# lc700x/desktop2stereo

Hardware: AMD Instinct MI355X
Metric: stereo frames/sec @1080p DepthAnything-v2-ViT-B (higher is better)
Workload: dtype bf16; 1 GPU; DepthAnything-v2-vitb bf16, 1920x1080 uint8 RGB noise frames, batch 1 per GPU, Depth Resolution 518 (model input 294x518), Full-SBS uint8 output 3840x1080, pred; parallelism=frame-sharded dp1, no data-path collective (each rank generates its own frames)

## Files before the change

### desktop2stereo_amd/_lib.py

```python
from __future__ import annotations

import ctypes as C
import os

HERE = os.path.dirname(os.path.abspath(__file__))
LIB_PATH = os.environ.get("D2S_LIB") or os.path.join(HERE, "libd2s_hip.so")

OK = 0
MODE = {"Half-SBS": 0, "Full-SBS": 1, "Half-TAB": 2, "Full-TAB": 3}
FMT_U8_HWC, FMT_F32_CHW, FMT_F32_HWC, FMT_U8_CHW = 0, 1, 2, 3
PREC_FP32, PREC_BF16, PREC_FP8, PREC_BF16X3, PREC_FP8_MLP = 0, 1, 2, 3, 4


class ModelDesc(C.Structure):
    _fields_ = [("hidden", C.c_int32), ("heads", C.c_int32), ("layers", C.c_int32),
                ("out_indices", C.c_int32 * 4), ("neck", C.c_int32 * 4), ("fusion", C.c_int32),
                ("head_hidden", C.c_int32), ("mlp", C.c_int32), ("patch", C.c_int32),
                ("pos_grid", C.c_int32), ("ln_eps", C.c_float), ("precision", C.c_int32), ("temporal", C.c_int32),
                ("max_depth", C.c_float)]


class PostParams(C.Structure):
    _fields_ = [("percentile", C.c_float), ("subsample_cap", C.c_int32), ("gamma", C.c_float),
                ("foreground_scale", C.c_float), ("aa_strength", C.c_float), ("ema_alpha", C.c_float),
                ("metric", C.c_int32)]


RESAMPLE = {"bilinear": 0, "bicubic_aa": 1}


class PreParams(C.Structure):
    _fields_ = [("mean", C.c_float * 3), ("std", C.c_float * 3), ("resample", C.c_int32), ("square", C.c_int32)]


class SbsParams(C.Structure):
    _fields_ = [("ipd_uv", C.c_double), ("depth_ratio", C.c_float), ("convergence", C.c_float),
                ("display_mode", C.c_int32), ("fill_16_9", C.c_int32)]


class DibrParams(C.Structure):
    _fields_ = [("ipd_uv", C.c_double), ("depth_strength", C.c_float), ("convergence", C.c_float), ("roll", C.c_float),
                ("search_radius", C.c_float), ("depth_tolerance", C.c_float), ("blur_radius", C.c_float),
                ("res_w", C.c_float), ("res_h", C.c_float), ("display_mode", C.c_int32),
                ("feather_enabled", C.c_int32), ("feather_width", C.c_float), ("corner_radius", C.c_float),
                ("viewport", C.c_float * 4), ("alpha_mode", C.c_int32), ("struct_size", C.c_uint32)]


class XrScreen(C.Structure):
    _fields_ = [("struct_size", C.c_uint32), ("curve", C.c_int32), ("width", C.c_double), ("height", C.c_double),
                ("distance", C.c_double), ("pan_x", C.c_double), ("pan_y", C.c_double), ("yaw", C.c_double), ("pitch", C.c_double),
                ("roll", C.c_double), ("normal_offset", C.c_double), ("clear", C.c_float * 4)]


class XrEye(C.Structure):
    _fields_ = [("vp", C.c_double * 16), ("width", C.c_int32), ("height", C.c_int32), ("eye", C.c_int32), ("struct_size", C.c_uint32)]


class XrGlow(C.Structure):
    _fields_ = [("struct_size", C.c_uint32), ("mode", C.c_int32), ("range_m", C.c_double), ("inner_edge_fraction", C.c_double)]


class XrFrost(C.Structure):
    _fields_ = [("struct_size", C.c_uint32), ("mode", C.c_int32), ("head", C.c_double * 3), ("intensity", C.c_double), ("alpha", C.c_double),
                ("edge_inset", C.c_double), ("beam_softness", C.c_double), ("beam_thickness", C.c_double), ("lod", C.c_double),
                ("threshold", C.c_double), ("noise_scale", C.c_double), ("blend", C.c_double), ("diffuse", C.c_double), ("time", C.c_double)]


class XrPanorama(C.Structure):
    _fields_ = [("struct_size", C.c_uint32), ("flip_y", C.c_int32), ("height", C.c_int32), ("width", C.c_int32),
                ("yaw_offset", C.c_double), ("exposure", C.c_double), ("ray", (C.c_double * 9) * 2)]


XR_GLOW = {"off": 0, "glow": 1, "glow2": 2}
XR_FROST = {"off": 0, "veil": 1, "frosted": 2}
XR_CURVE = {"flat": 0, "horizontal": 1, "vertical": 2}
DIBR_ALPHA = {"window": 0, "premultiplied": 1, "rgba": 2}
COMPOSITE = {"Anaglyph": 0, "Interleaved": 1, "Interleaved-V": 2, "Depth Map": 3}


class Conv3ProbeParams(C.Structure):
    _fields_ = [("struct_size", C.c_uint32), ("precision", C.c_int32), ("tile", C.c_int32),
                ("batch", C.c_int32), ("C", C.c_int32), ("N", C.c_int32), ("Hs", C.c_int32), ("Ws", C.c_int32),
                ("Hi", C.c_int32), ("Wi", C.c_int32), ("stride", C.c_int32), ("relu_in", C.c_int32), ("act", C.c_int32),
                ("out_f32", C.c_int32), ("map_head", C.c_int32), ("b3", C.c_float), ("max_depth", C.c_float),
                ("reserved", C.c_int32), ("splitk_elems", C.c_int64),
                ("x", C.c_void_p), ("w", C.c_void_p), ("bias", C.c_void_p), ("res", C.c_void_p), ("w3", C.c_void_p),
                ("out", C.c_void_p), ("kernel", C.c_char * 128)]


class RcuProbeParams(C.Structure):
    _fields_ = [("struct_size", C.c_uint32), ("batch", C.c_int32), ("H", C.c_int32), ("W", C.c_int32), ("C", C.c_int32),
                ("reserved", C.c_int32), ("x", C.c_void_p), ("w1", C.c_void_p), ("b1", C.c_void_p), ("w2", C.c_void_p),
                ("b2", C.c_void_p), ("wp", C.c_void_p), ("bp", C.c_void_p), ("out", C.c_void_p), ("kernel", C.c_char * 128)]


class AttentionProbeParams(C.Structure):
    _fields_ = [("struct_size", C.c_uint32), ("precision", C.c_int32), ("B", C.c_int32), ("heads", C.c_int32), ("N", C.c_int32),
                ("out_e4m3", C.c_int32), ("oscale", C.c_float), ("reserved", C.c_int32),
                ("q", C.c_void_p), ("k", C.c_void_p), ("v", C.c_void_p), ("out", C.c_void_p), ("kernel", C.c_char * 128)]


class LinearProbeParams(C.Structure):
    _fields_ = [("struct_size", C.c_uint32), ("site", C.c_int32), ("precision", C.c_int32), ("ln_fold", C.c_int32),
                ("M", C.c_int32), ("N", C.c_int32), ("K", C.c_int32), ("ntok", C.c_int32), ("heads", C.c_int32), ("npad", C.c_int32),
                ("gh", C.c_int32), ("gw", C.c_int32), ("ks", C.c_int32), ("pK", C.c_int32), ("ln_eps", C.c_float),
                ("s_act", C.c_float), ("s_out", C.c_float), ("s_res", C.c_float), ("s_pact", C.c_float), ("tile", C.c_int32),
                ("splitk_elems", C.c_int64),
                ("a", C.c_void_p), ("w", C.c_void_p), ("bias", C.c_void_p), ("scale", C.c_void_p), ("res", C.c_void_p), ("res2", C.c_void_p),
                ("ln_g", C.c_void_p), ("ln_b", C.c_void_p), ("pa", C.c_void_p), ("pw", C.c_void_p), ("pbias", C.c_void_p),
                ("pscale", C.c_void_p), ("x", C.c_void_p), ("out", C.c_void_p), ("out2", C.c_void_p), ("vt", C.c_void_p),
                ("stats", C.c_void_p), ("stats_slots", C.c_int32), ("reserved", C.c_int32),
                ("kernel", C.c_char * 128), ("kernel2", C.c_char * 128)]


class TemporalProbeParams(C.Structure):
    _fields_ = [("struct_size", C.c_uint32), ("op", C.c_int32), ("precision", C.c_int32), ("rows", C.c_int32), ("sites", C.c_int32),
                ("C", C.c_int32), ("groups", C.c_int32), ("slots", C.c_int32), ("eps", C.c_float), ("qscale", C.c_float),
                ("bx3_out", C.c_int32), ("rows_per_img", C.c_int32), ("img_rows", C.c_int32), ("row_off", C.c_int32), ("n", C.c_int64),
                ("x", C.c_void_p), ("out", C.c_void_p), ("gamma", C.c_void_p), ("beta", C.c_void_p), ("ptab", C.c_void_p),
                ("x_elems", C.c_uint64), ("out_elems", C.c_uint64), ("gamma_elems", C.c_uint64), ("beta_elems", C.c_uint64),
                ("ptab_elems", C.c_uint64), ("ring", C.c_void_p * 32), ("ring_elems", C.c_uint64 * 32),
                ("head", C.c_int32 * 32), ("Tw", C.c_int32 * 32), ("store_slot", C.c_int32 * 32),
                ("slot0", C.c_int32 * 32), ("nslots", C.c_int32 * 32), ("kernel", C.c_char * 128)]


class WarpPlanResult(C.Structure):
    _fields_ = [("struct_size", C.c_uint32), ("gather", C.c_int32), ("direct", C.c_int32), ("nc", C.c_int32), ("ntx", C.c_int32),
                ("wpc", C.c_int32), ("rpw", C.c_int32), ("out_h", C.c_int32), ("out_w", C.c_int32), ("grid", C.c_uint32),
                ("waves", C.c_int64), ("kernel", C.c_char * 64)]


class PostPlanResult(C.Structure):
    _fields_ = [("struct_size", C.c_uint32), ("form", C.c_int32), ("launches", C.c_int32), ("k", C.c_int32), ("r", C.c_int32),
                ("step", C.c_int32), ("m", C.c_int32), ("tail", C.c_int32), ("lds_bytes", C.c_uint32 * 3), ("kernel", (C.c_char * 32) * 3)]


POST_FORM = {0: "fused", 1: "tile", 2: "rows"}


class XrPlanResult(C.Structure):
    _fields_ = [("struct_size", C.c_uint32), ("kind", C.c_int32), ("rows_per_eye", C.c_int32), ("setup_launches", C.c_int32),
                ("grid", C.c_uint32 * 3), ("lds_dynamic_bytes", C.c_uint32), ("lds_static_bytes", C.c_uint32), ("reserved", C.c_uint32),
                ("workspace_bytes", C.c_uint64), ("out_elems", C.c_uint64), ("offsets", C.c_uint64 * 2)]


XR_ENTRY = {"eyes": 0, "glow": 1, "glow_curved": 2}
XR_KIND = {0: "plain", 1: "glow", 2: "glow_curved", 3: "frost", 4: "frost_curved"}


class ForwardPlanResult(C.Structure):
    _fields_ = [("struct_size", C.c_uint32), ("f8", C.c_int32), ("f8a", C.c_int32), ("x3", C.c_int32), ("lnf", C.c_int32),
                ("pp_fold", C.c_int32), ("tap_fold", C.c_int32), ("use_side", C.c_int32), ("ln_slots", C.c_int32 * 2),
                ("site", C.c_int32 * 11), ("tap_side", C.c_int32 * 4), ("head1_ups", C.c_int32), ("head2_fused", C.c_int32),
                ("head2_ups", C.c_int32), ("bn", C.c_int32), ("tm_fold", C.c_int32), ("tm_cache_store", C.c_int32),
                ("tm_slots", (C.c_int32 * 3) * 4), ("tm_folded", (C.c_int32 * 3) * 4), ("gh", C.c_int32), ("gw", C.c_int32),
                ("P", C.c_int32), ("N", C.c_int32), ("Npad", C.c_int32), ("fH", C.c_int32 * 4), ("fW", C.c_int32 * 4),
                ("tm_C", C.c_int32 * 4), ("tm_sites", C.c_int32 * 4), ("ln_launches", C.c_int32), ("rcu_fused", C.c_int32),
                ("splitk_elems", C.c_uint64), ("scr_elems", C.c_uint64)]


PLAN_FLAGS = {"calibrating": 1, "profiling": 2, "window_filled": 4, "calibrated": 8}
PLAN_SITES = ("patch", "qkv0", "qkv", "proj", "fc1", "fc2", "fc2_last", "neck0", "neck1", "neck2", "neck3")


class PrepatchProbeParams(C.Structure):
    _fields_ = [("struct_size", C.c_uint32), ("precision", C.c_int32), ("fmt", C.c_int32), ("batch", C.c_int32), ("H", C.c_int32),
                ("W", C.c_int32), ("decim_stride", C.c_int32), ("h", C.c_int32), ("w", C.c_int32), ("p", C.c_int32), ("Kp", C.c_int32),
                ("N", C.c_int32), ("D", C.c_int32), ("reserved", C.c_int32), ("pre", C.POINTER(PreParams)), ("frames", C.c_void_p),
                ("A", C.c_void_p), ("cls", C.c_void_p), ("pos", C.c_void_p), ("resid", C.c_void_p),
                ("frames_elems", C.c_uint64), ("A_elems", C.c_uint64), ("cls_elems", C.c_uint64), ("pos_elems", C.c_uint64),
                ("resid_elems", C.c_uint64), ("kernel", C.c_char * 64)]


TEMPORAL_OPS = {"groupnorm": 0, "temporal_attn": 1, "cache_store": 2, "geglu": 3, "cast_f32": 4, "layernorm": 5}

LINEAR_SITES = {"patch": 0, "qkv": 1, "proj": 2, "fc1": 3, "fc2": 4, "neck_proj": 5, "neck_resize": 6, "tm_proj_in": 7,
# ... 165 lines not shown
```

### desktop2stereo_amd/csrc/conv3.hip

```cpp
#include "conv3_tile.h"
#include <algorithm>

namespace d2s {

static_assert(sizeof(GemmA) + sizeof(GemmEpi) + 8 >= KERNARG_WARM_BYTES, "KERNARG_WARM reads past the kernarg segment");


template <int N_> __device__ __forceinline__ void c3_wait_vm() { asm volatile("s_waitcnt vmcnt(%0) lgkmcnt(0)" ::"n"(N_) : "memory"); }

template <int PST> __device__ __forceinline__ int c3_lane_pixel(int fr) {
    if constexpr ((PST & 1) == 0) return fr;
    else return fr < 4 ? 2 * fr : (fr < 12 ? 2 * (fr - 4) + 1 : 2 * (fr - 8));
}
template <int PST> __device__ __forceinline__ int c3_chunk_slot(int c) {
    if constexpr ((PST & 1) == 0) return c;
    else return (c & ~3) | ((c & 1) << 1) | ((c >> 1) & 1);
}

template <int CPP, int PST, int BN, int WM, int WN, int NS, int HG = 3 >
__global__ void __launch_bounds__(64 * WM * WN)
conv3_halo2_kernel(GemmA a, const bf16_t* __restrict__ W, int M, int N, int Kpad, GemmEpi e, int xn) {
    KERNARG_WARM(kaw_)
    KERNARG_WARM_END(kaw_)
    constexpr int TW = 16, TH = 8, HWD = TW + 2, HPX = (TH + 2) * HWD;
// ... 849 lines not shown
            for (int i = 0; i < FM; ++i)
#pragma unroll
                for (int jn = 0; jn < FN; ++jn) mma_chunk(acc[i][jn], fb[kt & 1][jn], fa[kt & 1][i], bf16_t());
            __builtin_amdgcn_sched_barrier(0);
            __builtin_amdgcn_s_barrier();
            if constexpr (kt < NKT - 1) {
                issue_w((gb + kt + PD) & (NS - 1), (kt + PD) % NKT);
                if constexpr (kt == HKT) load_halo(tl);
                read_frags(std::integral_constant<int, kt + 1>{}, fa[(kt + 1) & 1], fb[(kt + 1) & 1]);
                if constexpr (kt + 2 < NKT) {
                    if constexpr (kt >= HKT && kt <= HKT + PD - 2) asm volatile("s_waitcnt vmcnt(%0)" ::"n"(NLD + PD - 2) : "memory");
                    else asm volatile("s_waitcnt vmcnt(%0)" ::"n"(PD - 2) : "memory");
                }
            }
            __builtin_amdgcn_sched_barrier(0);
            __builtin_amdgcn_s_barrier();
#ifdef D2S_C3_TIMING
            if constexpr (kt == 0) { C3_ACC(4, wall_clock64() - t_a) }
#endif
        });
        if (!grp) __builtin_amdgcn_s_barrier();
        C3_T(t_b)
        C3_ACC(0, t_b - t_a)
        int b, ty0, tx0;
        tiles.org(t, b, ty0, tx0);
        bool ok[FM];
        long mo[FM];
        uint2 rr[FM][FN];
#pragma unroll
        for (int i = 0; i < FM; ++i) {
            const int y = ty0 + frow[i], x = tx0 + fcol[i];
            ok[i] = y < a.Ho && x < a.Wo;
            mo[i] = ok[i] ? ((long)(b * a.Ho + y) * a.Wo + x) * e.ldc + wave_n * 64 + fg * 4 : (long)(wave_n * 64 + fg * 4);
        }
        auto load_res = [&]() {
            const bf16_t* rp = (const bf16_t*)e.res1;
#pragma unroll
            for (int i = 0; i < FM; ++i)
#pragma unroll
                for (int jn = 0; jn < FN; ++jn) rr[i][jn] = *(const uint2*)(rp + mo[i] + jn * 16);
        };
        float cb[FN][4];
#pragma unroll
        for (int jn = 0; jn < FN; ++jn) {
            if (e.bias) load4(e.bias + wave_n * 64 + jn * 16 + fg * 4, cb[jn]);
            else cb[jn][0] = cb[jn][1] = cb[jn][2] = cb[jn][3] = 0.f;
        }
        if (e.res1) load_res();
        C3_T(t_c)
        C3_ACC(1, t_c - t_b)
        __builtin_amdgcn_s_waitcnt(0xc07f);
        __builtin_amdgcn_s_barrier();
        if (tn >= 0) store_halo();
        C3_T(t_d)
        C3_ACC(2, t_d - t_c)
#pragma unroll
        for (int i = 0; i < FM; ++i)
#pragma unroll
            for (int jn = 0; jn < FN; ++jn) {
                float v[4] = {acc[i][jn][0] + cb[jn][0], acc[i][jn][1] + cb[jn][1], acc[i][jn][2] + cb[jn][2], acc[i][jn][3] + cb[jn][3]};
                if (e.act == ACT_RELU) { v[0] = fmaxf(v[0], 0.f); v[1] = fmaxf(v[1], 0.f); v[2] = fmaxf(v[2], 0.f); v[3] = fmaxf(v[3], 0.f); }
                if (e.res1) {
                    const uint2 r = rr[i][jn];
                    v[0] += __uint_as_float(r.x << 16); v[1] += __uint_as_float(r.x & 0xffff0000u);
                    v[2] += __uint_as_float(r.y << 16); v[3] += __uint_as_float(r.y & 0xffff0000u);
                }
                if (ok[i]) *(uint2*)((bf16_t*)e.out + mo[i] + jn * 16) = make_uint2(pk_bf16(v[0], v[1]), pk_bf16(v[2], v[3]));
            }
        C3_ACC(6, wall_clock64() - t_d)
        C3_ACC(3, 1)
        gb = (gb + NKT) & (NS - 1); t = tn;
    }
    c3_wait_vm<0>();
    C3_ACC(5, wall_clock64() - t_begin)
}


struct RcuArgs {
    const bf16_t* x;
    bf16_t* out;
    const bf16_t *w1, *w2, *wp;
    const float *b1, *b2, *bp;
    int H, W, nimg, Kpad, KpadP;
};
constexpr int RCU_TH = 4, RCU_TW = 8;
typedef short s16x4 __attribute__((ext_vector_type(4)));
__device__ __forceinline__ uint2 rcu_pack4(const float v[4], bool relu) {
    uint2 t = make_uint2(pk_bf16(v[0], v[1]), pk_bf16(v[2], v[3]));
    if (relu) t = __builtin_bit_cast(uint2, __builtin_elementwise_max(__builtin_bit_cast(s16x4, t), (s16x4){0, 0, 0, 0}));
    return t;
}
typedef unsigned int u32x2 __attribute__((ext_vector_type(2)));
__device__ __forceinline__ void rcu_lds_write_b64(const u32x4* chunk, int half, uint2 v) {
    const unsigned addr = (unsigned)(unsigned long)((__attribute__((address_space(3))) const char*)chunk) + (unsigned)half * 8u;
    const u32x2 d = {v.x, v.y};
    asm volatile("ds_write_b64 %0, %1" ::"v"(addr), "v"(d) : "memory");
}
template <int PROJ>
__global__ void __launch_bounds__(512)
conv3_rcu_kernel(RcuArgs r) {
    constexpr int TH = RCU_TH, TW = RCU_TW, CPP = 16, PST = 17, NW = 8;
    constexpr int W0 = TW + 4, P0 = (TH + 4) * W0;
    constexpr int W1 = TW + 2, P1 = (TH + 2) * W1;
    constexpr int NKT = 18, NG = 2 * NKT + (PROJ ? 2 : 0);
    constexpr int WST = 128 * 8;
    constexpr int NS = 7, PD = NS - 1, BI = 128 / (8 * NW);
    static_assert(P1 <= 64 && TH * TW == 32 && BI == 2 && NG > PD, "fragment counts below are for a 4 x 8 tile");
    __shared__ __attribute__((aligned(16))) u32x4 lds[NS * WST + P0 * PST + P1 * PST];
    D2S_POISON_LDS(lds, NS * WST + P0 * PST + P1 * PST)
    u32x4* const h0 = lds + NS * WST;
    u32x4* const h1 = h0 + P0 * PST;
    u32x4* const h2 = h0;

    const int tid = threadIdx.x, lane = tid & 63;
    const int wid = __builtin_amdgcn_readfirstlane(tid >> 6);
    const int fr = lane & 15, fg = lane >> 4;
    GemmA a = {};
    a.ptr = r.x; a.Hi = a.Ho = r.H; a.Wi = a.Wo = r.W; a.C = 128; a.relu = 1;
    const C3Tiles<TH, TW> tiles(a);
    int b, ty0, tx0;
    tiles.org(blockIdx.x, b, ty0, tx0);

    const int n0 = wid * 16 + fg * 4;
    float c1[4], c2[4], cp[4] = {0.f, 0.f, 0.f, 0.f};
    load4(r.b1 + n0, c1); load4(r.b2 + n0, c2);
    if constexpr (PROJ) load4(r.bp + n0, cp);

    const unsigned wbytes = 256u * (unsigned)r.Kpad * 2u, pbytes = 256u * (unsigned)r.KpadP * 2u;
    const __amdgpu_buffer_rsrc_t rs1 = __builtin_amdgcn_make_buffer_rsrc(uniform_ptr(r.w1), 0, wbytes, 0x00020000);
    const __amdgpu_buffer_rsrc_t rs2 = __builtin_amdgcn_make_buffer_rsrc(uniform_ptr(r.w2), 0, wbytes, 0x00020000);
    const __amdgpu_buffer_rsrc_t rsP = __builtin_amdgcn_make_buffer_rsrc(uniform_ptr(PROJ ? r.wp : r.w2), 0, PROJ ? pbytes : wbytes, 0x00020000);
    unsigned voW[BI], voP[BI];
#pragma unroll
    for (int i = 0; i < BI; ++i) {
        const int row = (i * NW + wid) * 8 + (lane >> 3);
        const unsigned ch = (unsigned)(((lane & 7) ^ ((row >> 1) & 7)) * 16);
        voW[i] = (unsigned)(row * r.Kpad * 2) + ch;
        voP[i] = (unsigned)(row * r.KpadP * 2) + ch;
    }
    auto issue = [&](int g, int slot) {
        u32x4* st_ = lds + slot * WST;
        if (g < NKT) {
#pragma unroll
            for (int i = 0; i < BI; ++i) lds_dma16(rs1, st_ + (i * NW + wid) * 64, voW[i], g * 128);
        } else if (!PROJ || g < 2 * NKT) {
#pragma unroll
            for (int i = 0; i < BI; ++i) lds_dma16(rs2, st_ + (i * NW + wid) * 64, voW[i], (g - NKT) * 128);
        } else {
#pragma unroll
            for (int i = 0; i < BI; ++i) lds_dma16(rsP, st_ + (i * NW + wid) * 64, voP[i], (g - 2 * NKT) * 128);
        }
    };
#pragma unroll
    for (int t = 0; t < PD; ++t) issue(t, t);

    conv_halo_fill<bf16_t, 64 * NW, 3>(a, b, ty0 - 1, tx0 - 1, W0, P0, CPP, tid, h0,
        [&](int p, int c) { return p * PST + c; },
        [&](u32x4 v) { return relu_frag(v, relu_floor_bf16(a), bf16_t()); });
#pragma unroll
    for (int q = 0; q < 4; ++q) asm volatile("" : "+v"(c1[q]), "+v"(c2[q]), "+v"(cp[q]));

    int g = 0, slot = 0, islot = PD;
    auto ring_step = [&]() -> const u32x4* {
        const int rem = NG - 1 - g;
        if (rem >= PD - 1) c3_wait_vm<(PD - 1) * BI>();
        else if (rem == 4) c3_wait_vm<4 * BI>();
        else if (rem == 3) c3_wait_vm<3 * BI>();
        else if (rem == 2) c3_wait_vm<2 * BI>();
        else if (rem == 1) c3_wait_vm<1 * BI>();
        else c3_wait_vm<0>();
        __builtin_amdgcn_s_barrier();
        if (g + PD < NG) issue(g + PD, islot);
        const u32x4* B_l = lds + slot * WST;
        ++g;
        slot = slot + 1 == NS ? 0 : slot + 1;
        islot = islot + 1 == NS ? 0 : islot + 1;
        return B_l;
    };
    static_assert(PD == 6, "ring_step spells out the waits of the last PD - 1 tiles");
    int wo[2];
    {
        const int row = wid * 16 + fr;
#pragma unroll
        for (int ks = 0; ks < 2; ++ks) wo[ks] = row * 8 + ((ks * 4 + fg) ^ ((row >> 1) & 7));
    }

    {
        const u32x4* hb[4];
#pragma unroll
        for (int f = 0; f < 4; ++f) {
            const int p = f * 16 + fr < P1 ? f * 16 + fr : P1 - 1;
            hb[f] = h0 + ((p / W1) * W0 + p % W1) * PST + fg;
        }
        f32x4 acc[4];
#pragma unroll
        for (int f = 0; f < 4; ++f) acc[f] = (f32x4){0.f, 0.f, 0.f, 0.f};
#pragma unroll 1
        for (int kt = 0; kt < NKT; ++kt) {
            const int tap = kt >> 1, ky = (tap * 11) >> 5, kx = tap - 3 * ky;
            const int toff = (ky * W0 + kx) * PST + (kt & 1) * 8;
            const u32x4* B_l = ring_step();
            u32x4 fb[2], fa[2][4];
#pragma unroll
            for (int ks = 0; ks < 2; ++ks) {
                fb[ks] = B_l[wo[ks]];
#pragma unroll
                for (int f = 0; f < 4; ++f) fa[ks][f] = hb[f][toff + ks * 4];
            }
            __builtin_amdgcn_sched_barrier(0);
#pragma unroll
            for (int ks = 0; ks < 2; ++ks)
#pragma unroll
                for (int f = 0; f < 4; ++f) mma_chunk(acc[f], fb[ks], fa[ks][f], bf16_t());
        }
#pragma unroll
        for (int f = 0; f < 4; ++f) {
            const int p = f * 16 + fr;
            const int py = p / W1, px = p - py * W1;
            const int iy = ty0 - 1 + py, ix = tx0 - 1 + px;
            const float v[4] = {acc[f][0] + c1[0], acc[f][1] + c1[1], acc[f][2] + c1[2], acc[f][3] + c1[3]};
            uint2 t = rcu_pack4(v, true);
            if (!(iy >= 0 && iy < r.H && ix >= 0 && ix < r.W)) t = make_uint2(0u, 0u);
            if (p < P1) rcu_lds_write_b64(h1 + p * PST + 2 * wid + (fg >> 1), fg & 1, t);
        }
    }

    const int oy0 = fr >> 3, ox = fr & 7;
    uint2 rcu[2];
    {
        const u32x4* hb[2];
#pragma unroll
        for (int f = 0; f < 2; ++f) hb[f] = h1 + ((2 * f + oy0) * W1 + ox) * PST + fg;
        f32x4 acc[2];
#pragma unroll
        for (int f = 0; f < 2; ++f) acc[f] = (f32x4){0.f, 0.f, 0.f, 0.f};
#pragma unroll 1
        for (int kt = 0; kt < NKT; ++kt) {
            const int tap = kt >> 1, ky = (tap * 11) >> 5, kx = tap - 3 * ky;
            const int toff = (ky * W1 + kx) * PST + (kt & 1) * 8;
            const u32x4* B_l = ring_step();
            u32x4 fb[2], fa[2][2];
#pragma unroll
            for (int ks = 0; ks < 2; ++ks) {
                fb[ks] = B_l[wo[ks]];
#pragma unroll
                for (int f = 0; f < 2; ++f) fa[ks][f] = hb[f][toff + ks * 4];
            }
            __builtin_amdgcn_sched_barrier(0);
#pragma unroll
            for (int ks = 0; ks < 2; ++ks)
#pragma unroll
                for (int f = 0; f < 2; ++f) mma_chunk(acc[f], fb[ks], fa[ks][f], bf16_t());
        }
        float xr[2][4];
#pragma unroll
        for (int f = 0; f < 2; ++f) {
            const int y = ty0 + 2 * f + oy0, x = tx0 + ox;
            const bool ok = y < r.H && x < r.W;
            load4(r.x + ((long)(b * r.H + (ok ? y : 0)) * r.W + (ok ? x : 0)) * 128 + n0, xr[f]);
        }
#pragma unroll
        for (int f = 0; f < 2; ++f) {
            float v[4] = {acc[f][0] + c2[0], acc[f][1] + c2[1], acc[f][2] + c2[2], acc[f][3] + c2[3]};
            v[0] += xr[f][0]; v[1] += xr[f][1]; v[2] += xr[f][2]; v[3] += xr[f][3];
            rcu[f] = rcu_pack4(v, false);
        }
    }
    if constexpr (!PROJ) {
#pragma unroll
        for (int f = 0; f < 2; ++f) {
            const int y = ty0 + 2 * f + oy0, x = tx0 + ox;
            if (y < r.H && x < r.W) *(uint2*)(r.out + ((long)(b * r.H + y) * r.W + x) * 128 + n0) = rcu[f];
        }
    } else {
#pragma unroll
        for (int f = 0; f < 2; ++f) rcu_lds_write_b64(h2 + (f * 16 + fr) * PST + 2 * wid + (fg >> 1), fg & 1, rcu[f]);
        f32x4 acc[2];
#pragma unroll
        for (int f = 0; f < 2; ++f) acc[f] = (f32x4){0.f, 0.f, 0.f, 0.f};
#pragma unroll 1
        for (int kt = 0; kt < 2; ++kt) {
            const u32x4* B_l = ring_step();
#pragma unroll
            for (int ks = 0; ks < 2; ++ks) {
                const u32x4 fb = B_l[wo[ks]];
#pragma unroll
                for (int f = 0; f < 2; ++f) mma_chunk(acc[f], fb, h2[(f * 16 + fr) * PST + fg + kt * 8 + ks * 4], bf16_t());
            }
        }
#pragma unroll
        for (int f = 0; f < 2; ++f) {
            const int y = ty0 + 2 * f + oy0, x = tx0 + ox;
            const float v[4] = {acc[f][0] + cp[0], acc[f][1] + cp[1], acc[f][2] + cp[2], acc[f][3] + cp[3]};
            if (y < r.H && x < r.W) *(uint2*)(r.out + ((long)(b * r.H + y) * r.W + x) * 128 + n0) = rcu_pack4(v, false);
        }
    }
}

#define C3_INSTANCES(P, H, R)                                                                                                    \
    R(C3_RCU, conv3_rcu_kernel<0>)                                                                                               \
    R(C3_RCU_PROJ, conv3_rcu_kernel<1>)                                                                                          \
    P(C3_HEAD_UPS, conv3_head_ups_kernel)                                                                                        \
    P(C3_HEAD_1, conv3_head_kernel<1>)                                                                                           \
    P(C3_HEAD_0, conv3_head_kernel<0>)                                                                                           \
    P(C3_C128_UPS, conv3_c128_ups_kernel)                                                                                        \
    P(C3_WIDE_8_32, conv3_wide_kernel<8,32>)                                                                                     \
    P(C3_WIDE_16_16, conv3_wide_kernel<16,16>)                                                                                   \
    H(C3_H2_MID, 16,17,64,4,2,10,6)                                             \
    H(C3_H2_C128_N128, 16,17,128,2,4,2)                     \
    H(C3_H2_C128_N64, 16,17,64,4,2,3)                                                                                            \
    H(C3_H2_C128_N32, 16,17,32,4,1,3)                                                                                            \
    H(C3_H2_C64_N128, 8,10,128,2,4,3)                                                                                            \
    H(C3_H2_C64_N64, 8,10,64,4,2,3)                                                                                              \
    H(C3_H2_C64_N32, 8,10,32,4,1,3)
#define C3_ID(ID, ...) ID,
enum { C3_INSTANCES(C3_ID, C3_ID, C3_ID) };
#undef C3_ID
#define C3_BLOCK(CPP, PST, BN, WM, WN, ...) 64 * WM * WN
#define C3_P(ID, ...) {#__VA_ARGS__, 512},
#define C3_H(ID, ...) {"conv3_halo2_kernel<" #__VA_ARGS__ ">", C3_BLOCK(__VA_ARGS__)},
static const struct { const char* name; int block; } c3_inst[] = { C3_INSTANCES(C3_P, C3_H, C3_P) };
#undef C3_P
#undef C3_H
#undef C3_BLOCK
static void c3_plan(GemmPlan& p, int inst, unsigned grid, int xn, const GemmA& a) {
    p.family = GEMM_CONV3; p.inst = inst; p.name = c3_inst[inst].name; p.grid = grid; p.block = c3_inst[inst].block; p.xn = xn; p.ups = a.ups;
}


static bool c3_head_persistent_ok(const GemmA& a, int N, const GemmEpi& e, long t16) {
    static EnvInt headp_min{"D2S_HEADP_MIN", 2048};
    return e.map == MAP_HEAD && a.C == 64 && N <= 32 && t16 >= headp_min.get();
}
static bool c3_c128_ups_ok(const GemmA& a, int N, const GemmEpi& e, int nimg, long t8) {
    static EnvInt c128_min{"D2S_HEAD1P_MIN", 2048};
    return a.ups && a.C == 128 && N == 64 && e.map == MAP_ROWS && !a.relu && a.usy <= 0.5f && a.usx <= 0.5f && a.Hs >= 2 && a.Ws >= 2 &&
           (e.out_type == OUT_T || e.out_type == OUT_BF16) && !e.scale && !e.res1 && !e.res2 && e.act == ACT_NONE && !e.deq && !e.out2 && !(e.ldc & 7) &&
           c128_min.get() > 0 && t8 >= c128_min.get() && t8 < (1L << 30) && (long)nimg * a.Hs * a.Ws * a.C * 2 < (1L << 31);
}
static bool c3_wide_ok(const GemmA& a, int N, int Kpad, const GemmEpi& e, long t256, int ncu) {
    static EnvInt no_wide{"D2S_NO_WIDE", 0};
    return !no_wide.get() && !a.ups && e.map == MAP_ROWS && a.C == 128 && N == 128 && (long)gemm_npad(N) * Kpad * 2 < (1L << 31) &&
           (e.out_type == OUT_T || e.out_type == OUT_BF16) && !e.scale && !e.res2 && !e.res1_mod && (e.act == ACT_NONE || e.act == ACT_RELU) &&
           t256 >= 384 && t256 < (1L << 30) && (ncu & ~7) >= 8;
}
static bool c3_mid_ok(const GemmA& a, int N, int Kpad, const GemmEpi& e, long t8, int ncu) {
    return a.C == 128 && e.map == MAP_ROWS && N % 64 == 0 && (long)gemm_npad(N) * Kpad * 2 < (1L << 31) &&
           t8 * (N / 64) <= ncu && t8 * (N / 64) * 2 > ncu;
}

bool plan_conv3_halo2(const GemmA& a, int M, int N, int K, int Kpad, const GemmEpi& e, GemmPlan& p) {
    static EnvInt off{"D2S_NO_HALO2", 0};
    if (off.get()) return false;
    if (a.mode != A_CONV3 || a.stride != 1 || a.Hi != a.Ho || a.Wi != a.Wo || (a.C != 64 && a.C != 128) || K != 9 * a.C) return false;
    if (!(e.map == MAP_ROWS || e.map == MAP_HEAD) || e.rows_per_img || e.ln_stats || e.stats_out || e.deq || e.ksplit > 1) return false;
    if (e.map == MAP_HEAD && N > 32) return false;
    if (N != 32 && N != 64 && (N & 127)) return false;
    const int nimg = M / (a.Ho * a.Wo);
    if ((long)nimg * a.Ho * a.Wo != M) return false;
    const int ncu = device_cu_count();
    const long per16 = (long)cdiv(a.Ho, 16) * cdiv(a.Wo, 16), per8x32 = (long)cdiv(a.Ho, 8) * cdiv(a.Wo, 32);
    const long t16 = nimg * per16, t8 = (long)nimg * cdiv(a.Ho, 8) * cdiv(a.Wo, 16);
    const long t256 = nimg * std::min(per8x32, per16);
    if (c3_head_persistent_ok(a, N, e, t16)) {
        static EnvInt no_headups{"D2S_NO_HEADUPS", 0};
        if (a.ups && (no_headups.get() || a.usy > 0.6f || a.usx > 0.6f || a.relu)) return false;
        static EnvInt ups_v1{"D2S_HEADUPS_V1", 0};
        const bool ups_fits = (long)nimg * a.Hs * a.Ws * a.C * 2 < (1L << 31) && (long)a.Ws * a.C * 2 <= 65536;
        c3_plan(p, a.ups ? (!ups_v1.get() && ups_fits ? C3_HEAD_UPS : C3_HEAD_1) : C3_HEAD_0, std::min(ncu, (int)t16), (int)t16, a);
        return true;
    }
    if (c3_c128_ups_ok(a, N, e, nimg, t8)) {
        c3_plan(p, C3_C128_UPS, std::min(ncu & ~7, (int)t8), (int)t8, a);
        return true;
    }
    if (c3_wide_ok(a, N, Kpad, e, t256, ncu)) {
        c3_plan(p, per8x32 <= per16 ? C3_WIDE_8_32 : C3_WIDE_16_16, ncu & ~7, (int)t256, a);
        return true;
    }
    unsigned grid = 0;
    if (c3_mid_ok(a, N, Kpad, e, t8, ncu)) {
        const int xn = pick_xn((int)t8, N / 64, 64, Kpad, 2, grid);
        c3_plan(p, C3_H2_MID, grid, xn, a);
        return true;
    }
    const int bn = N <= 32 ? 32 : (N <= 64 ? 64 : 128);
    if (t8 * cdiv(N, bn) < 384) return false;
    if ((long)gemm_npad(N) * Kpad * 2 >= (1L << 31)) return false;
    const int xn = pick_xn((int)t8, cdiv(N, bn), bn, Kpad, 2, grid);
    if (a.C == 128) c3_plan(p, bn == 128 ? C3_H2_C128_N128 : (bn == 64 ? C3_H2_C128_N64 : C3_H2_C128_N32), grid, xn, a);
    else c3_plan(p, bn == 128 ? C3_H2_C64_N128 : (bn == 64 ? C3_H2_C64_N64 : C3_H2_C64_N32), grid, xn, a);
    return true;
}

void launch_conv3_halo2(const GemmPlan& p, const GemmA& a, const void* W, int M, int N, int Kpad, const GemmEpi& e, hipStream_t st) {
    const bf16_t* w = (const bf16_t*)W;
    const dim3 grid(p.grid), block(p.block);
    switch (p.inst) {
#define C3_P(ID, ...) case ID: hipLaunchKernelGGL((__VA_ARGS__), grid, block, 0, st, a, w, N, Kpad, e, p.xn); break;
#define C3_H(ID, ...) case ID: hipLaunchKernelGGL((conv3_halo2_kernel<__VA_ARGS__>), grid, block, 0, st, a, w, M, N, Kpad, e, p.xn); break;
#define C3_R(ID, ...) case ID: break;
        C3_INSTANCES(C3_P, C3_H, C3_R)
#undef C3_P
#undef C3_H
#undef C3_R
    }
}

bool c3_rcu_ok(bool plain_bf16, int C, int nimg, int H, int W) {
    return plain_bf16 && C == 128 && nimg > 0 && H > 0 && W > 0 && (long)nimg * H * W * 128 < (1L << 31) &&
           (long)nimg * cdiv(H, RCU_TH) * cdiv(W, RCU_TW) <= device_cu_count();
}
bool plan_conv3_rcu(bool plain_bf16, int C, int nimg, int H, int W, bool proj, GemmPlan& p) {
    if (!c3_rcu_ok(plain_bf16, C, nimg, H, W)) return false;
    p = GemmPlan{};
    const int inst = proj ? C3_RCU_PROJ : C3_RCU;
    p.family = GEMM_CONV3; p.inst = inst; p.name = c3_inst[inst].name; p.block = c3_inst[inst].block;
    p.grid = (unsigned)(nimg * cdiv(H, RCU_TH) * cdiv(W, RCU_TW)); p.ksplit = 1;
    return true;
}
void launch_conv3_rcu(const GemmPlan& p, const RcuOp& o, hipStream_t st) {
    const RcuArgs r = {(const bf16_t*)o.x, (bf16_t*)o.out, (const bf16_t*)o.w1, (const bf16_t*)o.w2, (const bf16_t*)o.wp, o.b1, o.b2, o.bp,
                       o.H, o.W, o.nimg, o.Kpad, o.KpadP};
    const dim3 grid(p.grid), block(p.block);
    switch (p.inst) {
#define C3_N(ID, ...)
#define C3_R(ID, ...) case ID: hipLaunchKernelGGL((__VA_ARGS__), grid, block, 0, st, r); break;
        C3_INSTANCES(C3_N, C3_N, C3_R)
#undef C3_N
#undef C3_R
    }
    kernel_note() = KernelNote{p.name, 0, 1, NOTE_TAIL_NONE};
}

}

#ifdef D2S_C3U_TIMING
extern "C" int d2s_c3u_timing(unsigned long long* out, int clear) {
    if (out) D2S_HIP(hipMemcpyFromSymbol(out, HIP_SYMBOL(d2s::c3u_timing), sizeof(unsigned long long) * 256 * 9));
    if (clear) { static unsigned long long z[256 * 9]; D2S_HIP(hipMemcpyToSymbol(HIP_SYMBOL(d2s::c3u_timing), z, sizeof(z))); }
    return D2S_OK;
}
#endif
#ifdef D2S_C3_TIMING
extern "C" int d2s_c3_timing(unsigned long long* out, int clear) {
    if (out) D2S_HIP(hipMemcpyFromSymbol(out, HIP_SYMBOL(d2s::c3_timing), sizeof(unsigned long long) * 256 * 8));
    if (clear) { static unsigned long long z[256 * 8]; D2S_HIP(hipMemcpyToSymbol(HIP_SYMBOL(d2s::c3_timing), z, sizeof(z))); }
    return D2S_OK;
}
#endif
```

### desktop2stereo_amd/csrc/core.cpp

```cpp
#include "common.h"

#include <atomic>
#include <cstdlib>

namespace d2s {

static thread_local std::string g_err;

void set_error(const std::string& msg) { g_err = msg; }

int hip_fail(hipError_t err, const char* what, const char* file, int line) {
    g_err = std::string("HIP error ") + hipGetErrorName(err) + " (" + hipGetErrorString(err) + ") in " + what +
            " at " + file + ":" + std::to_string(line);
    return D2S_E_HIP;
}

int env_int(const char* name, int dflt) {
    const char* v = getenv(name);
    return v ? atoi(v) : dflt;
}

static std::atomic<int> g_env_gen{1};
int env_generation() { return g_env_gen.load(std::memory_order_relaxed); }
int EnvInt::get() {
    const uint32_t g = (uint32_t)env_generation();
    const uint64_t c = cached.load(std::memory_order_relaxed);
    if ((uint32_t)(c >> 32) == g) return (int)(uint32_t)c;
    const int val = env_int(name, dflt);
    cached.store(((uint64_t)g << 32) | (uint32_t)val, std::memory_order_relaxed);
    return val;
}

int device_cu_count() {
    static const int n = [] { hipDeviceProp_t p; int d = 0; (void)hipGetDevice(&d); return hipGetDeviceProperties(&p, d) == hipSuccess ? p.multiProcessorCount : 256; }();
    return n;
}

}

extern "C" int d2s_debug_lds_poison(void) {
#ifdef D2S_LDS_POISON
    return 1;
#else
    return 0;
#endif
}
extern "C" int d2s_debug_reload_env(void) { return d2s::g_env_gen.fetch_add(1) + 1; }
extern "C" const char* d2s_last_error(void) { return d2s::g_err.c_str(); }
extern "C" int d2s_version(void) { return 127; }
```

### desktop2stereo_amd/csrc/engine.hip

```cpp
#include <map>
#include <string>
#include <vector>
#include <cmath>
#include <cstring>

#include "gemm.h"
#include "forward_plan.h"
#include "dibr_xr.h"
#include "vit_ops.h"

using namespace d2s;

namespace {

struct HostT { std::vector<float> data; std::vector<int64_t> shape; };

struct Layer {
    float *ln1g, *ln1b, *ln2g, *ln2b, *ls1, *ls2;
    LinearForms qkv, proj, fc1, fc2;
    LinearForms& lin(int i) { LinearForms* const a[4] = {&qkv, &proj, &fc1, &fc2}; return *a[i]; }
};

}

// ... 170 lines not shown
int pack_convT(d2s_engine* e, const std::string& wname, const std::string& bname, int C, int ks, DevLinear& out) {
    const std::string err = "weight " + wname + ": wrong shape";
    const float *p = host_f32(e, wname, (size_t)C * C * ks * ks, err), *bt = host_f32(e, bname, C, err);
    if (!p || !bt) return D2S_E_MISSING;
    int N = ks * ks * C;
    std::vector<float> bias(N);
    for (int n = 0; n < N; ++n) bias[n] = bt[n % C];
    return upload_linear(e, prepare_linear(e->wprec, N, C, [&](int n, int k) { return p[convT_weight_index(n, k, C, ks)]; }, bias.data()), out);
}

void cubic_coeffs(float t, float c[4]) {
    const float A = -0.75f;
    auto c1 = [&](float x) { return ((A + 2.f) * x - (A + 3.f)) * x * x + 1.f; };
    auto c2 = [&](float x) { return ((A * x - 5.f * A) * x + 8.f * A) * x - 4.f * A; };
    c[0] = c2(t + 1.f); c[1] = c1(t); c[2] = c1(1.f - t); c[3] = c2(2.f - t);
}

void interp_pos(const float* pos, int grid, int D, int gh, int gw, std::vector<float>& out, double offset = 0.0) {
    out.assign((size_t)(1 + gh * gw) * D, 0.f);
    std::memcpy(out.data(), pos, D * sizeof(float));
    if (gh == grid && gw == grid) { std::memcpy(out.data() + D, pos + D, (size_t)grid * grid * D * sizeof(float)); return; }
    float sy = (float)grid / (float)gh, sx = (float)grid / (float)gw;
    if (offset != 0.0) {
        sy = (float)(1.0 / (((double)gh + offset) / (double)grid)); sx = (float)(1.0 / (((double)gw + offset) / (double)grid));
    }
    for (int oy = 0; oy < gh; ++oy) {
        float fy = sy * ((float)oy + 0.5f) - 0.5f;
        float iyf = floorf(fy);
        float cy[4]; cubic_coeffs(fy - iyf, cy);
        int iy = (int)iyf;
        for (int ox = 0; ox < gw; ++ox) {
            float fx = sx * ((float)ox + 0.5f) - 0.5f;
            float ixf = floorf(fx);
            float cx[4]; cubic_coeffs(fx - ixf, cx);
            int ix = (int)ixf;
            float* o = out.data() + (size_t)(1 + oy * gw + ox) * D;
            for (int d = 0; d < D; ++d) {
                float acc = 0.f;
                for (int a = 0; a < 4; ++a) {
                    int yy = std::min(std::max(iy - 1 + a, 0), grid - 1);
                    float row = 0.f;
                    for (int b = 0; b < 4; ++b) {
                        int xx = std::min(std::max(ix - 1 + b, 0), grid - 1);
                        row += pos[(size_t)(1 + yy * grid + xx) * D + d] * cx[b];
                    }
                    acc += row * cy[a];
                }
                o[d] = acc;
            }
        }
    }
}

FrameState frame_state(const d2s_engine* e) {
    return FrameState{e->calib, e->fp8_ready, e->taps, e->prof_on, e->overlap && e->side != nullptr, e->no_lnfuse, e->tm_fold, e->tap_ln[0] != nullptr};
}

struct LnPair { void* buf; float* stats; };
LnPair tap_ln_pair(const d2s_engine* e, const ForwardPlan& pl, int i) {
    return i >= 0 && i < 4 && pl.tap_private[i] ? LnPair{e->tap_ln[i], e->tap_stats[i]} : LnPair{e->lnbuf, e->lnstats};
}

int slots_check(int got, int planned, const char* site) {
    if (got == planned) return D2S_OK;
    set_error(std::string("forward: ") + site + " left " + std::to_string(got) + " LayerNorm statistics slots, the frame's plan says " + std::to_string(planned));
    return D2S_E_STATE;
}

int linear(d2s_engine* e, const GemmA& a, const DevLinear& w, int M, const GemmEpi& ep, hipStream_t st, hipEvent_t stop = nullptr) {
    float* ws = (e->side && st == e->side) ? e->splitk_ws_side : e->splitk_ws;
    PROF(a.mode == A_CONV3 ? PC_CONV : PC_GEMM, 2.0 * M * w.N * w.K, 0, launch_linear(w, a, M, ep, ws, e->g.splitk_elems, 0, st, stop));
    return D2S_OK;
}

int conv3(d2s_engine* e, const void* in, int B, int Hi, int Wi, int C, int stride, int relu_in, const DevLinear& w,
          void* out, int act, const void* res1, const void* res2, hipStream_t st) {
    int Ho = (Hi + 2 - 3) / stride + 1, Wo = (Wi + 2 - 3) / stride + 1;
    GemmA a = convA(in, Hi, Wi, C, Ho, Wo, stride, relu_in);
    GemmEpi ep = rowsE(out, OUT_T, w.N, w.bias);
    ep.act = act; ep.res1 = res1; ep.res2 = res2;
    return linear(e, a, w, B * Ho * Wo, ep, st);
}

int rcu(d2s_engine* e, const void* x, int B, int H, int W, const DevLinear& c1, const DevLinear& c2, const DevLinear* proj, void* out, hipStream_t st) {
    GemmPlan p;
    if (!plan_conv3_rcu(true, e->d.fusion, B, H, W, proj != nullptr, p) || c1.Kpad != c2.Kpad || !c1.bias || !c2.bias || (proj && !proj->bias)) {
        set_error("forward: the frame's plan fuses a residual unit that conv3_rcu_kernel does not take");
        return D2S_E_STATE;
    }
    const RcuOp o = {x, out, B, H, W, c1.w, c2.w, proj ? proj->w : nullptr, c1.bias, c2.bias, proj ? proj->bias : nullptr, c1.Kpad, proj ? proj->Kpad : 0};
    const double macs = (double)c1.N * c1.K + (double)c2.N * c2.K + (proj ? (double)proj->N * proj->K : 0.0);
    PROF(PC_CONV, 2.0 * B * H * W * macs, 0, (launch_conv3_rcu(p, o, st), D2S_OK));
    return D2S_OK;
}

void window_rows(const d2s_engine::TSlot& sl, bool fold, void* ring, AttnRow& attn, CacheRow& store) {
    const bool in_attn = fold && sl.filled;
    attn = AttnRow{ring, (int16_t)sl.head, (int16_t)(sl.filled ? 32 : 1), in_attn ? sl.head : -1};
    store = CacheRow{ring, sl.filled ? sl.head : 0, sl.filled ? (in_attn ? 0 : 1) : 31};
}

int run_temporal(d2s_engine* e, const ForwardPlan& pl, int m, const void* x, void* out, int B, hipStream_t st, const void* add = nullptr) {
    d2s_engine::TMod& t = e->tm[m];
    const int C = t.C, S = B * t.sites, prec = e->prec;
    const int* ids = e->row_ids;
    const bool fold = pl.tm_fold;
    auto residual = [&](int j, const void* A, const DevLinear& W, const char* site) -> int {
        int slots = -1;
        const LinearOp o = op_tm_residual(e->tm_hs, C, A, W.bias, j > 0, e->tm_a, e->tm_stats, fold ? &slots : nullptr);
        RC(linear(e, o.a, W, S, o.ep, st));
        return fold ? slots_check(slots, pl.tm[m].slots[j], site) : D2S_OK;
    };
    auto consumer = [&](GemmEpi& ep, int j, const float* csum) { epi_ln_consumer(ep, e->tm_stats, pl.tm[m].slots[j], csum, 1e-5f, C); };
    void* gn_out = fold ? e->tm_out : e->tm_a;
    PROF(PC_ELT, 0, 0, launch_groupnorm(prec, x, t.gn_g, t.gn_b, gn_out, t.sites, C, 32, 1e-6f, st, B));
    RC(residual(0, gn_out, t.proj_in, "a temporal module's proj_in"));
    for (int a = 0; a < 2; ++a) {
        const bool folded = pl.tm[m].folded[a];
        if (!folded) PROF(PC_LN, 0, 0, launch_layernorm(prec, e->tm_hs, t.ln_g[a], t.ln_b[a], e->tm_a, S, C, 1e-5f, 0, 0, 0, st));
        {
            const DevLinear& W = t.kvq[a].form(false, folded);
            GemmEpi ep = rowsE(e->tm_kv, OUT_T, 3 * C, W.bias);
            if (folded) consumer(ep, a, W.csum);
            RC(linear(e, plainA(e->tm_a, C), W, S, ep, st));
        }
        AttnRows attn = {};
        CacheRows store = {};
        double win_rows = 0;
        bool store_due = false;
        for (int r = 0; r < B; ++r) {
            window_rows(e->tm_slot[ids[r]], fold, (char*)t.cache[a] + (size_t)ids[r] * t.ring_bytes, attn.r[r], store.r[r]);
            win_rows += attn.r[r].Tw;
            store_due |= store.r[r].nslots > 0;
        }
        PROF(PC_ATTN, 4.0 * t.sites * win_rows * C, 0, launch_temporal_attn(prec, e->tm_kv, t.ptab[a], e->tm_out, t.sites, C, 31, B, attn, st));
        RC(residual(a + 1, e->tm_out, t.to_out[a], "a temporal module's to_out"));
        if (store_due) PROF(PC_ELT, 0, 0, launch_cache_store(prec, e->tm_kv, t.sites, C, B, store, st));
    }
    {
        const bool folded = pl.tm[m].folded[2];
        if (!folded) PROF(PC_LN, 0, 0, launch_layernorm(prec, e->tm_hs, t.ffn_g, t.ffn_b, e->tm_a, S, C, 1e-5f, 0, 0, 0, st));
        const DevLinear& W = t.ff1.form(false, folded);
        GemmEpi ep = rowsE(folded ? e->tm_g : e->tm_u, OUT_T, (folded ? 4 : 8) * C, W.bias);
        if (folded) { ep.act = ACT_GEGLU; consumer(ep, 2, W.csum); }
        RC(linear(e, plainA(e->tm_a, C), W, S, ep, st));
        if (!folded) PROF(PC_ELT, 0, 0, launch_geglu(prec, e->tm_u, e->tm_g, S, 4 * C, st));
    }
    {
        GemmEpi ep = epi_residual(e->tm_hs, C, t.ff2.bias, nullptr);
        if (fold) epi_ln_producer(ep, e->tm_a, nullptr, nullptr);
        RC(linear(e, plainA(e->tm_g, 4 * C), t.ff2, S, ep, st));
    }
    const void* a_out = e->tm_a;
    if (!fold) {
        if (prec == D2S_PREC_BF16) PROF(PC_ELT, 0, 0, launch_cast_f32(prec, e->tm_hs, e->tm_a, (long)S * C, st));
        else a_out = e->tm_hs;
    }
    {
        GemmEpi ep = rowsE(out, OUT_T, C, t.proj_out.bias);
        ep.res1 = x; ep.res2 = add;
        RC(linear(e, plainA(a_out, C), t.proj_out, S, ep, st));
    }
    return D2S_OK;
}

int neck_proj(d2s_engine* e, const ForwardPlan& pl, int i, int B, hipStream_t st) {
    const d2s_model_desc& d = e->d;
    const int D = d.hidden, Mp = B * e->g.P, c = d.neck[i];
    const DevLinear& W = e->re[i].proj.form(false, pl.tap_folded);
    GemmEpi ep = rowsE(e->rproj[i], OUT_T, c, W.bias);
    if (!pl.tap_folded) return linear(e, plainA(e->tapbuf[i], D), W, Mp, ep, st);
    const LnPair ln = tap_ln_pair(e, pl, i);
    epi_ln_consumer(ep, ln.stats, pl.slots_fc2, W.csum, d.ln_eps, D);
    const int skip = epi_tap_fold_rows(ep, B, e->g.N, e->g.P);
    return linear(e, plainA((const bf16_t*)ln.buf + (size_t)skip * D, D), W, skip ? Mp : B * e->g.N, ep, st);
}

int neck_rest(d2s_engine* e, const ForwardPlan& pl, int i, int B, hipStream_t st) {
    const d2s_model_desc& d = e->d;
    const int F = d.fusion, gh = e->g.gh, gw = e->g.gw, Mp = B * e->g.P, c = d.neck[i];
    const void* src = e->rproj[i];
    int Hs = gh, Ws = gw;
    if (i < 2) {
        int ks = i == 0 ? 4 : 2;
        RC(linear(e, plainA(e->rproj[i], c), e->re[i].resize, Mp, epi_convT(e->rres[i], c, e->re[i].resize.bias, gh, gw, ks), st));
        src = e->rres[i]; Hs = gh * ks; Ws = gw * ks;
    } else if (i == 3) {
        RC(conv3(e, e->rproj[i], B, gh, gw, c, 2, 0, e->re[i].resize, e->rres[i], ACT_NONE, nullptr, nullptr, st));
        src = e->rres[i]; Hs = (gh - 1) / 2 + 1; Ws = (gw - 1) / 2 + 1;
    }
    if (d.temporal && i == 2) { RC(run_temporal(e, pl, 0, src, e->rres[2], B, st)); src = e->rres[2]; }
    if (d.temporal && i == 3) { RC(run_temporal(e, pl, 1, src, e->scr[0], B, st)); src = e->scr[0]; }
    RC(conv3(e, src, B, Hs, Ws, c, 1, 0, e->re[i].conv, e->feat[i], ACT_NONE, nullptr, nullptr, st));
    if (i < 3) {
        const int idx = 3 - i;
        if (pl.rcu1_fused[i]) RC(rcu(e, e->feat[i], B, Hs, Ws, e->fu[idx].r1c1, e->fu[idx].r1c2, nullptr, e->r1[i], st));
        else {
            RC(conv3(e, e->feat[i], B, Hs, Ws, F, 1, 1, e->fu[idx].r1c1, e->r1tmp, ACT_NONE, nullptr, nullptr, st));
            RC(conv3(e, e->r1tmp, B, Hs, Ws, F, 1, 1, e->fu[idx].r1c2, e->r1[i], ACT_NONE, e->feat[i], nullptr, st));
        }
    }
    return D2S_OK;
}

int forward(d2s_engine* e, const float* x, float* depth, int B, hipStream_t st) {
    const d2s_model_desc& d = e->d;
    const int D = d.hidden, N = e->g.N, P = e->g.P, M = B * N, Mp = B * P, prec = e->prec;
    const int F = d.fusion;
    ForwardPlan pl;
    RC(plan_forward(d, e->g, e->h, e->w, B, frame_state(e), pl));
    if (x) PROF(PC_ELT, 0, 0, launch_patchify(prec, x, e->patchA, B, e->h, e->w, d.patch, e->patch.Kpad, e->cls, e->pos, e->resid, N, D, st));
    {
        RC(linear(e, plainA(e->patchA, e->patch.Kpad), e->patch, Mp, epi_patch_embed(e->resid, D, e->patch.bias, e->pos, P, N), st));
    }
    if (e->taps) D2S_HIP(hipMemcpyAsync(e->tap_hidden, e->resid, (size_t)N * D * 4, hipMemcpyDeviceToDevice, st));
    int tap_i = 0;
    const bool f8 = pl.f8, f8a = pl.f8a, x3 = pl.x3;
    int pending_ln = -1;
    bool fork_in_launch = false;
    int ln_tap = -1;
    for (int l = 0; l < d.layers; ++l) {
        const Layer& ly = e->L[l];
        const float* sa = f8 ? &e->act_scale[(size_t)l * NSITE] : nullptr;
        float* am = e->calib ? e->amax + (size_t)l * NSITE : nullptr;
        const bool ln1_folded = pl.ln1_folded && l > 0;
        if (!ln1_folded) PROF(PC_LN, 0, 0, launch_layernorm(prec, e->resid, ly.ln1g, ly.ln1b, e->lnbuf, M, D, d.ln_eps, 0, 0, 0, st, f8a ? 1.0f / sa[0] : 0.f, x3));
        if (am) RC(launch_amax(prec, e->lnbuf, (long)M * D, am + 0, st));
        {
            const DevLinear& W = ly.qkv.form(f8a, ln1_folded);
            GemmEpi ep = epi_qkv(e->qkv, qkv_out_type(f8, x3), D, W.bias, e->vt, N, e->g.Npad, d.heads);
            const LnPair ln = tap_ln_pair(e, pl, ln1_folded ? ln_tap : -1);
            if (ln1_folded) epi_ln_consumer(ep, ln.stats, pl.slots_fc2, W.csum, d.ln_eps, D);
            RC(linear(e, splitA(ln.buf, D, x3), W, M, ep, st));
            ln_tap = -1;
        }
        PROF(PC_ATTN, 4.0 * B * d.heads * (double)N * N * 64, 0,
             launch_attention(x3 ? D2S_PREC_BF16X3 : prec, e->qkv, e->vt, e->attn, B, N, e->g.Npad, d.heads, st, f8a ? 1.0f / sa[1] : 0.f, e->attn_prescaled));
        if (am) RC(launch_amax(prec, e->attn, (long)M * D, am + 1, st));
        {
            if (pending_ln >= 0) { D2S_HIP(hipStreamWaitEvent(st, e->ev_ln[pending_ln], 0)); pending_ln = -1; }
            const DevLinear& W = ly.proj.form(f8a, false);
            int slots = -1;
            const LinearOp o = op_residual(e->resid, D, e->attn, D, x3, W.bias, ly.ls1, e->lnbuf, e->lnstats, pl.lnf ? &slots : nullptr, f8 ? 1.0f / sa[4] : 0.f);
            RC(linear(e, o.a, W, M, o.ep, st));
            if (pl.lnf) RC(slots_check(slots, pl.slots_proj, "proj"));
        }
        const bool ln2_folded = pl.ln2_folded;
        if (!ln2_folded) PROF(PC_LN, 0, 0, launch_layernorm(prec, e->resid, ly.ln2g, ly.ln2b, e->lnbuf, M, D, d.ln_eps, 0, 0, 0, st, f8 ? 1.0f / sa[2] : 0.f, x3));
        if (am) RC(launch_amax(D2S_PREC_FP32, e->resid, (long)M * D, am + 4, st));
        if (am) RC(launch_amax(prec, e->lnbuf, (long)M * D, am + 2, st));
        {
            const DevLinear& W = ly.fc1.form(f8, ln2_folded);
            GemmEpi ep = epi_fc1(e->mlp, fc1_out_type(x3), d.mlp, W.bias);
            if (ln2_folded) epi_ln_consumer(ep, e->lnstats, pl.slots_proj, W.csum, d.ln_eps, D);
            if (f8) ep.out_qscale = 1.0f / sa[3];
            RC(linear(e, splitA(e->lnbuf, D, x3), W, M, ep, st));
        }
        if (am) RC(launch_amax(prec, e->mlp, (long)M * d.mlp, am + 3, st));
        {
            const DevLinear& W = ly.fc2.form(f8, false);
            const bool stats = l + 1 < d.layers ? pl.fc2_stats : pl.fc2_stats_last;
            const bool tap_layer = tap_i < 4 && l + 1 == d.out_indices[tap_i];
            int slots = -1;
            const LnPair ln = tap_ln_pair(e, pl, tap_layer ? tap_i : -1);
            const LinearOp o = op_residual(e->resid, D, e->mlp, d.mlp, x3, W.bias, ly.ls2, ln.buf, ln.stats, stats ? &slots : nullptr, f8 ? 1.0f / sa[5] : 0.f);
            fork_in_launch = tap_layer && pl.tap_side[tap_i] && pl.tap_folded && e->side_sync;
            RC(linear(e, o.a, W, M, o.ep, st, fork_in_launch ? e->ev_tap[tap_i] : nullptr));
            if (tap_layer) ln_tap = tap_i;
            if (stats) RC(slots_check(slots, pl.slots_fc2, "FC2"));
        }
        if (am) RC(launch_amax(D2S_PREC_FP32, e->resid, (long)M * D, am + 5, st));
        if (e->taps) D2S_HIP(hipMemcpyAsync(e->tap_hidden + (size_t)(l + 1) * N * D, e->resid, (size_t)N * D * 4, hipMemcpyDeviceToDevice, st));
        if (tap_i < 4 && l + 1 == d.out_indices[tap_i]) {
            if (!pl.tap_folded) PROF(PC_LN, 0, 0, launch_layernorm(prec, e->resid, e->lnfg, e->lnfb, e->tapbuf[tap_i], Mp, D, d.ln_eps, P, N, 1, st));
            if (pl.tap_side[tap_i]) {
                if (!fork_in_launch) D2S_HIP(hipEventRecord(e->ev_tap[tap_i], st));
                D2S_HIP(hipStreamWaitEvent(e->side, e->ev_tap[tap_i], 0));
                RC(neck_proj(e, pl, tap_i, B, e->side));
                if (pl.tap_folded && !pl.tap_private[tap_i]) { D2S_HIP(hipEventRecord(e->ev_ln[tap_i], e->side)); pending_ln = tap_i; }
                RC(neck_rest(e, pl, tap_i, B, e->side));
            } else {
                RC(neck_proj(e, pl, tap_i, B, st));
            }
            ++tap_i;
        }
    }
    for (int i = 0; i < 4; ++i)
        if (!pl.tap_side[i]) RC(neck_rest(e, pl, i, B, st));
    if (pl.use_side) {
        D2S_HIP(hipEventRecord(e->ev_side, e->side));
        D2S_HIP(hipStreamWaitEvent(st, e->ev_side, 0));
    }
    void *X = e->scr[0], *Y = e->scr[1], *Z = e->scr[2];
    void* fused = nullptr;
    int Hc = 0, Wc = 0;
    for (int idx = 0; idx < 4; ++idx) {
        int mi = 3 - idx;
        void* m = e->feat[mi];
        Hc = e->g.fH[mi]; Wc = e->g.fW[mi];
        const void* hcur = idx == 0 ? m : fused;
        if (pl.rcu_fused[idx]) RC(rcu(e, hcur, B, Hc, Wc, e->fu[idx].r2c1, e->fu[idx].r2c2, &e->fu[idx].proj, X, st));
        else {
            RC(conv3(e, hcur, B, Hc, Wc, F, 1, 1, e->fu[idx].r2c1, X, ACT_NONE, nullptr, nullptr, st));
            RC(conv3(e, X, B, Hc, Wc, F, 1, 1, e->fu[idx].r2c2, Z, ACT_NONE, hcur, nullptr, st));
        }
        int Ho, Wo;
        if (idx < 3) { Ho = e->g.fH[mi - 1]; Wo = e->g.fW[mi - 1]; } else { Ho = Hc * 2; Wo = Wc * 2; }
        void* pout = e->scr[3 + (idx & 1)];
        const void* next_r1 = idx < 3 ? e->r1[2 - idx] : nullptr;
        if (!pl.rcu_fused[idx]) RC(linear(e, plainA(Z, F), e->fu[idx].proj, B * Hc * Wc, rowsE(X, OUT_T, F, e->fu[idx].proj.bias), st));
        if (d.temporal && idx < 2) {
            PROF(PC_ELT, 0, 0, launch_bilinear_nhwc(prec, X, pout, B, Hc, Wc, Ho, Wo, F, st));
            void* alt = e->scr[3 + ((idx + 1) & 1)];
            RC(run_temporal(e, pl, 2 + idx, pout, alt, B, st, next_r1));
            pout = alt;
        } else {
            if (!(idx == 3 && pl.head1_ups)) PROF(PC_ELT, 0, 0, launch_bilinear_nhwc(prec, X, pout, B, Hc, Wc, Ho, Wo, F, st, next_r1));
        }
        fused = pout; Hc = Ho; Wc = Wo;
    }
    void* c1out = X;
    void* up2 = Y;
    if (pl.head1_ups) {
        c1out = Y; up2 = X;
        const LinearOp o = op_head1_ups(X, e->g.fH[0], e->g.fW[0], F, c1out, e->head1.bias);
        PROF(PC_CONV, 2.0 * B * Hc * Wc * e->head1.N * e->head1.K, 0, launch_gemm(e->wprec, 0, o.a, e->head1.w, B * Hc * Wc, e->head1.N, e->head1.K, e->head1.Kpad, o.ep, st));
    } else {
        RC(conv3(e, fused, B, Hc, Wc, F, 1, 0, e->head1, c1out, ACT_NONE, nullptr, nullptr, st));
    }
    {
        const int Mh = B * e->h * e->w, Nh = d.head_hidden;
        if (!pl.head2_ups) PROF(PC_ELT, 0, 0, launch_bilinear_nhwc(prec, c1out, up2, B, Hc, Wc, e->h, e->w, F / 2, st));
        if (pl.head2_fused) {
            const LinearOp o = op_head_tail(pl.head2_ups ? c1out : up2, pl.head2_ups, Hc, Wc, e->h, e->w, F / 2, depth, e->head2.bias, e->w3, e->b3, d.max_depth);
            PROF(PC_CONV, 2.0 * Mh * Nh * e->head2.K, 0, launch_gemm(e->wprec, head_tile(pl.bn), o.a, e->head2.w, Mh, Nh, e->head2.K, e->head2.Kpad, o.ep, st));
        } else {
            RC(conv3(e, up2, B, e->h, e->w, F / 2, 1, 0, e->head2, Z, ACT_RELU, nullptr, nullptr, st));
            PROF(PC_ELT, 0, 0, launch_head_final(prec, Z, e->w3, e->b3, d.max_depth, depth, (long)B * e->h * e->w, d.head_hidden, st));
        }
    }
    if (d.temporal) {
        for (int r = 0; r < B; ++r) {
            d2s_engine::TSlot& sl = e->tm_slot[e->row_ids[r]];
            if (sl.filled) sl.head = (sl.head + 1) % 31;
            sl.filled = 1;
        }
    }
    e->last_batch = B;
    return D2S_OK;
}

int check_desc(const d2s_model_desc* desc) {
    D2S_REQUIRE(desc->hidden > 0 && desc->heads > 0 && desc->hidden == desc->heads * 64, "head_dim must be 64");
    D2S_REQUIRE(desc->layers > 0 && desc->patch > 0 && desc->pos_grid > 0 && desc->fusion % 8 == 0, "bad model desc");
    D2S_REQUIRE(desc->precision == D2S_PREC_FP32 || desc->precision == D2S_PREC_BF16 || desc->precision == D2S_PREC_FP8 ||
                desc->precision == D2S_PREC_BF16X3 || desc->precision == D2S_PREC_FP8_MLP, "bad precision");
    for (int i = 0; i < 4; ++i) D2S_REQUIRE(desc->neck[i] % 8 == 0 && desc->out_indices[i] >= 1 && desc->out_indices[i] <= desc->layers, "bad neck / out_indices");
    D2S_REQUIRE(desc->head_hidden % 4 == 0 && desc->mlp % 8 == 0, "bad head_hidden / mlp");
    D2S_REQUIRE(desc->max_depth >= 0.f && !(desc->temporal && desc->max_depth > 0.f),
                "max_depth must be >= 0, and 0 for a Video-Depth-Anything engine (its head ends in ReLU, dpt_temporal.py:136)");
    return D2S_OK;
}
int check_shape(const d2s_model_desc& d, int h, int w, int max_batch) {
    D2S_REQUIRE(h > 0 && w > 0 && h % d.patch == 0 && w % d.patch == 0 && max_batch >= 1, "h, w must be patch multiples");
    D2S_REQUIRE(!d.temporal || max_batch <= D2S_MAX_STREAMS, "a Video-Depth-Anything engine has at most D2S_MAX_STREAMS (32) stream slots: max_batch too large");
    for (int c : {d.neck[2], d.neck[3], d.fusion})
        D2S_REQUIRE(!d.temporal || (c % 32 == 0 && c <= 1024), "temporal module channels must be a multiple of 32 (GroupNorm) and <= 1024");
    return D2S_OK;
}

}

extern "C" int d2s_engine_create(const d2s_model_desc* desc, int device_id, d2s_engine** out) {
    D2S_REQUIRE(desc && out, "null pointer");
    RC(check_desc(desc));
    D2S_ON_DEVICE(device_id);
    d2s_engine* e = new d2s_engine();
    e->d = *desc; e->device = device_id;
    const PrecRules pr = prec_rules(desc->precision);
    e->fp8 = pr.e4m3;
    e->no_lnfuse = env_int("D2S_NO_LNFUSE", 0) != 0;
    e->lnf = pr.ln_folds(D2S_LIN_FC1) && !pr.e4m3 && !e->no_lnfuse;
    e->prec = pr.act;
    e->wprec = pr.w;
    e->attn_prescaled = e->prec == D2S_PREC_BF16;
    e->taps = env_int("D2S_TAPS", 0) != 0;
    *out = e;
    return D2S_OK;
}

extern "C" int d2s_engine_set_weight(d2s_engine* e, const char* name, const float* host, const int64_t* shape, int ndim) {
    D2S_REQUIRE(e && name && host && shape && ndim >= 1 && ndim <= 4, "bad argument");
    if (e->finalized) { set_error("d2s_engine_set_weight after finalize"); return D2S_E_STATE; }
    HostT t;
    size_t n = 1;
    for (int i = 0; i < ndim; ++i) { D2S_REQUIRE(shape[i] > 0, "bad shape"); n *= (size_t)shape[i]; t.shape.push_back(shape[i]); }
    t.data.assign(host, host + n);
    e->host[name] = std::move(t);
    return D2S_OK;
}

extern "C" int d2s_engine_finalize(d2s_engine* e, int h, int w, int max_batch) {
    D2S_REQUIRE(e, "null engine");
    if (e->finalized) { set_error("engine already finalized"); return D2S_E_STATE; }
    const d2s_model_desc& d = e->d;
    RC(check_shape(d, h, w, max_batch));
    D2S_ON_DEVICE(e->device);
    const int D = d.hidden, F = d.fusion;
// ... 198 lines not shown
    D2S_ON_DEVICE(e->device);
    if (e->side) (void)hipStreamSynchronize(e->side);
    for (int i = 0; i < 4; ++i) if (e->ev_tap[i]) (void)hipEventDestroy(e->ev_tap[i]);
    for (int i = 0; i < 4; ++i) if (e->ev_ln[i]) (void)hipEventDestroy(e->ev_ln[i]);
    if (e->ev_side) (void)hipEventDestroy(e->ev_side);
    if (e->side) (void)hipStreamDestroy(e->side);
    for (void* p : e->allocs) (void)hipFree(p);
    delete e;
    return D2S_OK;
}

extern "C" int d2s_engine_memory(const d2s_engine* e, uint64_t* bytes) {
    D2S_REQUIRE(e && bytes, "null pointer");
    *bytes = e->bytes;
    return D2S_OK;
}

namespace {
int resolve_streams(d2s_engine* e, int batch, const int* stream_ids) {
    if (!e->d.temporal) {
        D2S_REQUIRE(!stream_ids, "stream_ids on an engine that is not a Video-Depth-Anything engine: its batch rows are not streams");
        return D2S_OK;
    }
    uint32_t seen = 0;
    for (int r = 0; r < batch; ++r) {
        const int id = stream_ids ? stream_ids[r] : r;
        if (id < 0 || id >= e->maxB) { set_error("stream id " + std::to_string(id) + " out of range: the engine has " + std::to_string(e->maxB) + " stream slot(s)"); return D2S_E_INVALID; }
        if (seen >> id & 1u) { set_error("stream id " + std::to_string(id) + " named twice in one call"); return D2S_E_INVALID; }
        seen |= 1u << id;
    }
    for (int r = 0; r < batch; ++r) e->row_ids[r] = stream_ids ? stream_ids[r] : r;
    return D2S_OK;
}
}

extern "C" int d2s_model_forward_streams(d2s_engine* e, const float* x, float* depth, int batch, const int* stream_ids, void* stream) {
    D2S_REQUIRE(e && x && depth, "null pointer");
    if (!e->finalized) { set_error("d2s_model_forward before d2s_engine_finalize"); return D2S_E_STATE; }
    D2S_REQUIRE(batch >= 1 && batch <= e->maxB, "batch exceeds max_batch");
    RC(resolve_streams(e, batch, stream_ids));
    D2S_ON_DEVICE(e->device);
    return forward(e, x, depth, batch, (hipStream_t)stream);
}

extern "C" int d2s_model_forward(d2s_engine* e, const float* x, float* depth, int batch, void* stream) {
    return d2s_model_forward_streams(e, x, depth, batch, nullptr, stream);
}

extern "C" int d2s_forward_plan(const d2s_model_desc* desc, int h, int w, int batch, int flags, d2s_forward_plan_result* res) {
    D2S_REQUIRE(desc && res, "null pointer");
    D2S_REQUIRE(res->struct_size == sizeof(d2s_forward_plan_result), "d2s_forward_plan_result.struct_size must be sizeof(d2s_forward_plan_result)");
    RC(check_desc(desc));
    RC(check_shape(*desc, h, w, batch));
    const d2s_model_desc& d = *desc;
    const PrecRules pr = prec_rules(d.precision);
    FrameState s = {};
    s.calib = (flags & D2S_PLAN_CALIBRATING) != 0; s.fp8_ready = (flags & D2S_PLAN_CALIBRATED) != 0; s.prof = (flags & D2S_PLAN_PROFILING) != 0;
    s.taps = env_int("D2S_TAPS", 0) != 0; s.side = env_int("D2S_NO_OVERLAP", 0) == 0; s.no_lnfuse = env_int("D2S_NO_LNFUSE", 0) != 0;
    s.tm_fold = d.temporal && pr.ln_folds(D2S_LIN_TM_KVQ) && env_int("D2S_VDA_FUSE", 1) != 0;
    D2S_REQUIRE(!s.calib || (pr.e4m3 && !d.temporal), "D2S_PLAN_CALIBRATING: not a D2S_PREC_FP8 engine (or a Video-Depth-Anything engine)");
    const EngineGeom g = engine_geom(d, h, w, batch);
    ForwardPlan pl;
    RC(plan_forward(d, g, h, w, batch, s, pl));
    d2s_forward_plan_result r = {};
    r.struct_size = sizeof(r);
    r.f8 = pl.f8; r.f8a = pl.f8a; r.x3 = pl.x3; r.lnf = pl.lnf; r.pp_fold = pl.pp_fold; r.tap_fold = pl.tap_fold; r.use_side = pl.use_side;
    r.ln_slots[0] = pl.slots_proj; r.ln_slots[1] = pl.slots_fc2;
    const int e4a = pl.f8a ? D2S_PLAN_E4M3 : 0, e4 = pl.f8 ? D2S_PLAN_E4M3 : 0;
    r.site[D2S_PLAN_SITE_QKV0] = e4a;
    r.site[D2S_PLAN_SITE_QKV] = e4a | (pl.ln1_folded ? D2S_PLAN_FOLDED : 0);
    r.site[D2S_PLAN_SITE_PROJ] = e4a | (pl.lnf ? D2S_PLAN_STATS : 0);
    r.site[D2S_PLAN_SITE_FC1] = e4 | (pl.ln2_folded ? D2S_PLAN_FOLDED : 0);
    r.site[D2S_PLAN_SITE_FC2] = e4 | (pl.fc2_stats ? D2S_PLAN_STATS : 0);
    r.site[D2S_PLAN_SITE_FC2_LAST] = e4 | (pl.fc2_stats_last ? D2S_PLAN_STATS : 0);
    for (int i = 0; i < 4; ++i) { r.site[D2S_PLAN_SITE_NECK0 + i] = pl.tap_folded ? D2S_PLAN_FOLDED : 0; r.tap_side[i] = pl.tap_side[i]; }
    r.head1_ups = pl.head1_ups; r.head2_fused = pl.head2_fused; r.head2_ups = pl.head2_ups; r.bn = pl.bn;
    r.tm_fold = s.tm_fold;
    r.tm_cache_store = d.temporal && !(s.tm_fold && (flags & D2S_PLAN_WINDOW_FILLED));
    for (int m = 0; m < 4; ++m)
        for (int j = 0; j < 3; ++j) { r.tm_slots[m][j] = pl.tm[m].slots[j]; r.tm_folded[m][j] = pl.tm[m].folded[j]; }
    r.gh = g.gh; r.gw = g.gw; r.P = g.P; r.N = g.N; r.Npad = g.Npad;
    for (int i = 0; i < 4; ++i) { r.fH[i] = g.fH[i]; r.fW[i] = g.fW[i]; r.tm_C[i] = d.temporal ? g.tmC[i] : 0; r.tm_sites[i] = d.temporal ? g.tmS[i] : 0; }
    r.ln_launches = pl.ln_launches;
    for (int i = 0; i < 4; ++i) r.rcu_fused |= (pl.rcu_fused[i] ? 1 << i : 0) | (pl.rcu1_fused[i] ? 256 << i : 0);
    r.splitk_elems = g.splitk_elems; r.scr_elems = g.scr_elems;
    *res = r;
    return D2S_OK;
}

extern "C" int d2s_engine_calibrate(d2s_engine* e, const float* x, int batch, void* stream) {
    D2S_REQUIRE(e && x, "null pointer");
    if (!e->finalized) { set_error("d2s_engine_calibrate before d2s_engine_finalize"); return D2S_E_STATE; }
    D2S_REQUIRE(e->fp8, "d2s_engine_calibrate: not a D2S_PREC_FP8 engine");
    D2S_REQUIRE(batch >= 1 && batch <= e->maxB && !e->d.temporal, "bad batch (or a Video-Depth-Anything engine)");
    D2S_ON_DEVICE(e->device);
    hipStream_t st = (hipStream_t)stream;
    const int L = e->d.layers;
    D2S_HIP(hipMemsetAsync(e->amax, 0, (size_t)L * NSITE * sizeof(float), st));
    const bool prof = e->prof_on;
    e->prof_on = false;
    e->calib = true;
    int rc = forward(e, x, e->depth_small, batch, st);
    e->calib = false;
    e->prof_on = prof;
    if (rc != D2S_OK) return rc;
    static const float headroom = getenv("D2S_FP8_HEADROOM") ? std::max(1.0f, (float)atof(getenv("D2S_FP8_HEADROOM"))) : 1.0f;
    std::vector<float> am((size_t)L * NSITE);
    D2S_HIP(hipMemcpyAsync(am.data(), e->amax, am.size() * sizeof(float), hipMemcpyDeviceToHost, st));
    D2S_HIP(hipStreamSynchronize(st));
    for (int l = 0; l < L; ++l) {
        Layer& ly = e->L[l];
        for (int s = 0; s < NSITE; ++s) {
            float a = am[(size_t)l * NSITE + s];
            if (!(a > 0.f) || !std::isfinite(a)) { set_error("d2s_engine_calibrate: degenerate activation range"); return D2S_E_INVALID; }
            e->act_scale[(size_t)l * NSITE + s] = a * headroom / FP8_MAX;
        }
        for (int i = 0; i < 4; ++i)
            for (int folded = 0; folded < 2; ++folded) {
                const DevLinear& W = ly.lin(i).form(true, folded);
                const CalibSite cs = CALIB_SITE[i][folded];
                if (!W.w || l + cs.dlayer < 0) continue;
                const std::vector<float> dq = deq_scales(e->act_scale[(size_t)(l + cs.dlayer) * NSITE + cs.site], W.sw);
                D2S_HIP(hipMemcpy(W.deq, dq.data(), dq.size() * sizeof(float), hipMemcpyHostToDevice));
            }
    }
    e->fp8_ready = true;
    return D2S_OK;
}

extern "C" int d2s_engine_reset_stream(d2s_engine* e) {
    D2S_REQUIRE(e, "null engine");
    e->ema_init = 0;
    for (auto& sl : e->tm_slot) sl = d2s_engine::TSlot();
    for (auto& i : e->ema_slot_init) i = 0;
    return D2S_OK;
}

extern "C" int d2s_engine_reset_stream_at(d2s_engine* e, int stream_id) {
    D2S_REQUIRE(e, "null engine");
    const int slots = e->d.temporal ? (int)e->tm_slot.size() : 1;
    if (stream_id < 0 || stream_id >= slots) {
        set_error("d2s_engine_reset_stream_at: stream " + std::to_string(stream_id) + " does not exist (the engine has " + std::to_string(slots) + " slot(s))");
        return D2S_E_INVALID;
    }
    if (!e->d.temporal) { e->ema_init = 0; return D2S_OK; }
    e->tm_slot[stream_id] = d2s_engine::TSlot();
    e->ema_slot_init[stream_id] = 0;
    return D2S_OK;
}

extern "C" int d2s_pipeline(d2s_engine* e, const uint8_t* frames, int batch, int H, int W, int depth_resolution,
                            const d2s_pre_params* pre, const d2s_post_params* pp, const d2s_sbs_params* sp, int use_ema,
                            void* out, int out_fmt, float* depth_full, void* stream) {
    return d2s_pipeline_streams(e, frames, batch, nullptr, H, W, depth_resolution, pre, pp, sp, use_ema, out, out_fmt, depth_full, stream);
}

namespace d2s {
int dibr_warp_any(const uint8_t* rgb, const float* depth, int dh, int dw, int batch, int H, int W, const d2s_dibr_params* p,
                  void* out, int out_fmt, void* stream, bool check_only);
int dibr_composite_any(const uint8_t* rgb, const float* depth, int dh, int dw, int batch, int H, int W, const d2s_dibr_params* p,
                       int composite, void* out, int out_fmt, void* stream, bool check_only);
int dibr_warp_crop_any(const uint8_t* rgb, const float* depth, int dh, int dw, int batch, int H, int W, const d2s_dibr_params* p,
                       const double* crop, void* out, int out_fmt, void* stream, bool check_only);
}

namespace {
int pipeline_check(d2s_engine* e, int batch, const int* stream_ids, int H, int W, int depth_resolution, const d2s_pre_params* pre, int* stride_out) {
// ... 258 lines not shown
```

### desktop2stereo_amd/csrc/forward_plan.h

```cpp
#pragma once
#include <algorithm>
#include "linear_site.h"

namespace d2s {

struct EngineGeom {
    int gh, gw, P, N, Npad;
    int fH[4], fW[4];
    size_t splitk_elems;
    size_t scr_elems;
    int tmC[4], tmS[4];
};
static inline EngineGeom engine_geom(const d2s_model_desc& d, int h, int w, int max_batch) {
    EngineGeom g = {};
    const int F = d.fusion;
    g.gh = h / d.patch; g.gw = w / d.patch; g.P = g.gh * g.gw; g.N = g.P + 1; g.Npad = (g.N + 63) / 64 * 64;
    g.fH[0] = g.gh * 4; g.fW[0] = g.gw * 4; g.fH[1] = g.gh * 2; g.fW[1] = g.gw * 2; g.fH[2] = g.gh; g.fW[2] = g.gw;
    g.fH[3] = (g.gh - 1) / 2 + 1; g.fW[3] = (g.gw - 1) / 2 + 1;
    g.splitk_elems = (size_t)max_batch * 16 * g.fH[2] * g.fW[2] * std::max(F, d.neck[3]);
    g.scr_elems = std::max({(size_t)64 * g.gh * g.gw * F, (size_t)h * w * (F / 2), (size_t)h * w * d.head_hidden}) * max_batch;
    const int tC[4] = {d.neck[2], d.neck[3], F, F}, tM[4] = {2, 3, 2, 1};
    for (int m = 0; m < 4; ++m) { g.tmC[m] = tC[m]; g.tmS[m] = g.fH[tM[m]] * g.fW[tM[m]]; }
    return g;
}

static inline GemmA plainA(const void* p, long lda) { GemmA a = {}; a.ptr = p; a.mode = A_PLAIN; a.lda = lda; return a; }
static inline GemmA splitA(const void* p, long lda, bool split) { GemmA a = plainA(p, lda); a.bx3 = split ? 1 : 0; return a; }
static inline GemmA convA(const void* p, int Hi, int Wi, int C, int Ho, int Wo, int stride, int relu) {
    GemmA a = {}; a.ptr = p; a.mode = A_CONV3; a.Hi = Hi; a.Wi = Wi; a.C = C; a.Ho = Ho; a.Wo = Wo; a.stride = stride; a.relu = relu; return a;
}
struct LinearOp { GemmA a; GemmEpi ep; };

static inline LinearOp op_residual(float* resid, int D, const void* A, int K, bool x3, const float* bias, const float* ls, void* lnbuf,
                                   float* lnstats, int* slots, float out2_qscale) {
    LinearOp o = {splitA(A, K, x3), epi_residual(resid, D, bias, ls)};
    if (slots) epi_ln_producer(o.ep, lnbuf, lnstats, slots, x3, out2_qscale);
    return o;
}
static inline LinearOp op_tm_residual(float* hs, int C, const void* A, const float* bias, bool residual, void* copy, float* stats, int* slots) {
    LinearOp o = {plainA(A, C), residual ? epi_residual(hs, C, bias, nullptr) : rowsE(hs, OUT_F32, C, bias)};
    if (slots) epi_ln_producer(o.ep, copy, stats, slots);
    return o;
}
static inline GemmA upsA(const void* src, int Hs, int Ws, int C, int Ho, int Wo) {
    GemmA a = convA(src, Ho, Wo, C, Ho, Wo, 1, 0);
    a.ups = 1; a.Hs = Hs; a.Ws = Ws; a.usy = linear_scale(Hs, Ho, true); a.usx = linear_scale(Ws, Wo, true);
    return a;
}
static inline LinearOp op_head1_ups(const void* src, int Hs, int Ws, int F, void* out, const float* bias) {
    return {upsA(src, Hs, Ws, F, 2 * Hs, 2 * Ws), rowsE(out, OUT_T, F / 2, bias)};
}
static inline LinearOp op_head_tail(const void* in, bool ups, int Hs, int Ws, int h, int w, int C, float* depth, const float* bias, const float* w3,
                                    float b3, float max_depth) {
    LinearOp o = {ups ? upsA(in, Hs, Ws, C, h, w) : convA(in, h, w, C, h, w, 1, 0), rowsE(depth, OUT_F32, 1, bias)};
    o.ep.map = MAP_HEAD; o.ep.scale = w3; o.ep.head_b3 = b3; o.ep.head_max_depth = max_depth;
    return o;
}

static inline void* plan_addr() { static float word[4]; return word; }
static inline DevLinear linear_shape(int gprec, int N, int K) {
    DevLinear L;
    L.w = plan_addr(); L.bias = (const float*)plan_addr(); L.deq = gprec == D2S_PREC_FP8_OPERANDS ? (float*)plan_addr() : nullptr;
    L.N = N; L.K = K; L.Kpad = gemm_kpad(K, gprec); L.prec = gprec;
    return L;
}

struct FrameState {
    bool calib;
    bool fp8_ready;
    bool taps;
    bool prof;
    bool side;
    bool no_lnfuse;
    bool tm_fold;
    bool tap_private;
};
constexpr int LN_SLOTS_MAX = 16;
struct ForwardPlan {
    bool use_side;
    bool f8, f8a, x3;
    bool pp_fold, lnf, tap_fold;
    int slots_proj, slots_fc2;
    bool ln1_folded;
    bool ln2_folded;
    bool fc2_stats, fc2_stats_last;
    bool tap_folded;
    bool tap_side[4];
    bool tap_private[4];
    bool head1_ups;
    bool head2_fused, head2_ups;
    int bn;
    bool rcu_fused[4];
    bool rcu1_fused[4];
    bool tm_fold;
    struct { int slots[3]; bool folded[3]; } tm[4];
    int ln_launches;
};

static inline int plan_forward(const d2s_model_desc& d, const EngineGeom& g, int h, int w, int B, const FrameState& s, ForwardPlan& pl) {
    pl = ForwardPlan{};
    const PrecRules pr = prec_rules(d.precision);
    if (pr.e4m3 && !s.fp8_ready && !s.calib) {
        set_error("D2S_PREC_FP8 engine: activation scales are not set, call d2s_engine_calibrate first");
        return D2S_E_STATE;
    }
    const int D = d.hidden, F = d.fusion, M = B * g.N;
    float* const ws = (float*)plan_addr();
    pl.use_side = s.side && !s.prof;
    pl.f8 = pr.e4m3 && !s.calib;
    pl.f8a = pl.f8 && pr.e4m3_attn;
    pl.x3 = pr.w == D2S_PREC_BF16X3;
    static EnvInt lnf_pp{"D2S_LNF_PP", 1};
    const int pp_min = gemm_pp_min_tiles();
    const bool forms_lnf = pr.ln_folds(D2S_LIN_FC1) && !pr.e4m3 && !s.no_lnfuse;
    pl.pp_fold = lnf_pp.get() && forms_lnf && pr.w == D2S_PREC_BF16 && !s.calib && !s.taps && D % 256 == 0 && D <= 1024 && pp_min > 0 &&
                 (long)cdiv(M, 256) * (D / 256) >= pp_min;
    pl.lnf = (pr.ln_folds(D2S_LIN_FC1) && !s.no_lnfuse && !s.calib && B <= (pl.x3 ? 8 : 3)) || pl.pp_fold;
    pl.tap_fold = pl.lnf && pr.ln_folds(D2S_LIN_NECK_PROJ) && (B == 1 || pl.pp_fold);
    pl.fc2_stats = pl.lnf && pr.ln_folds(D2S_LIN_FC2);
    pl.fc2_stats_last = pl.fc2_stats && pl.tap_fold;
    GemmPlan gp;
    int slots = 0;
    const float qs = pl.f8 ? 1.f : 0.f;
    if (pl.lnf) {
        const LinearOp o = op_residual(ws, D, ws, D, pl.x3, ws, ws, ws, ws, &slots, qs);
        if (plan_linear(linear_shape(pl.f8a ? D2S_PREC_FP8_OPERANDS : pr.w, D, D), o.a, M, o.ep, ws, g.splitk_elems, gp)) { set_error(gp.error); return D2S_E_INVALID; }
        pl.slots_proj = gp.stats_slots;
    }
    if (pl.fc2_stats && (d.layers > 1 || pl.fc2_stats_last)) {
        const LinearOp o = op_residual(ws, D, ws, d.mlp, pl.x3, ws, ws, ws, ws, &slots, qs);
        if (plan_linear(linear_shape(pl.f8 ? D2S_PREC_FP8_OPERANDS : pr.w, D, d.mlp), o.a, M, o.ep, ws, g.splitk_elems, gp)) { set_error(gp.error); return D2S_E_INVALID; }
        pl.slots_fc2 = gp.stats_slots;
    }
    pl.ln2_folded = pl.lnf && pl.slots_proj <= LN_SLOTS_MAX;
    pl.ln1_folded = pl.fc2_stats && pr.ln_folds(D2S_LIN_QKV) && pl.slots_fc2 <= LN_SLOTS_MAX;
    pl.tap_folded = pl.tap_fold && pl.slots_fc2 <= LN_SLOTS_MAX;
    for (int i = 0; i < 4; ++i) pl.tap_side[i] = pl.use_side && (i < 3 || d.temporal);
    for (int i = 0; i < 4; ++i) pl.tap_private[i] = pl.tap_side[i] && pl.tap_folded && s.tap_private;
    pl.ln_launches = 1 + (d.layers - 1) * !pl.ln1_folded + d.layers * !pl.ln2_folded + 4 * !pl.tap_folded;
    {
        static EnvInt rcu_fuse{"D2S_RCU_FUSE", 1};
        const bool plain_bf16 = rcu_fuse.get() && pr.precision == D2S_PREC_BF16 && !s.calib;
        for (int i = 0; i < 4; ++i) {
            const bool ok = c3_rcu_ok(plain_bf16, F, B, g.fH[i], g.fW[i]);
            pl.rcu_fused[3 - i] = ok;
            pl.rcu1_fused[i] = ok && i < 3;
        }
    }
    pl.tm_fold = d.temporal && s.tm_fold;
    for (int m = 0; m < 4 && d.temporal; ++m) {
        const int C = g.tmC[m], S = B * g.tmS[m];
        for (int j = 0; j < 3; ++j) {
            if (pl.tm_fold) {
                const LinearOp o = op_tm_residual(ws, C, ws, ws, j > 0, ws, ws, &slots);
                if (plan_linear(linear_shape(pr.w, C, C), o.a, S, o.ep, ws, g.splitk_elems, gp)) { set_error(gp.error); return D2S_E_INVALID; }
                pl.tm[m].slots[j] = gp.stats_slots;
            }
            pl.tm[m].folded[j] = pl.tm_fold && pl.tm[m].slots[j] >= 1 && pl.tm[m].slots[j] <= LN_SLOTS_MAX;
            pl.ln_launches += !pl.tm[m].folded[j];
        }
    }
    {
        const DevLinear h1 = linear_shape(pr.w, F / 2, 9 * F);
        const LinearOp o = op_head1_ups(ws, g.fH[0], g.fW[0], F, ws, ws);
        pl.head1_ups = conv3_upsample_ok(pr.w, 0, o.a, B * 4 * g.fH[0] * g.fW[0], h1.N, h1.K, h1.Kpad, o.ep);
    }
    {
        const int Mh = B * h * w, Nh = d.head_hidden;
        pl.bn = Nh <= 32 ? 32 : 64;
        pl.head2_fused = Nh <= 64 && (long)cdiv(Mh, 256) * cdiv(Nh, pl.bn) >= 224;
        const DevLinear h2 = linear_shape(pr.w, Nh, 9 * (F / 2));
        const LinearOp o = op_head_tail(ws, true, 2 * g.fH[0], 2 * g.fW[0], h, w, F / 2, ws, ws, ws, 0.f, d.max_depth);
        pl.head2_ups = pl.head2_fused && conv3_upsample_ok(pr.w, head_tile(pl.bn), o.a, Mh, Nh, h2.K, h2.Kpad, o.ep);
    }
    return D2S_OK;
}

}
```

### desktop2stereo_amd/csrc/gemm.h

```cpp
#pragma once
#include "common.h"
#include <hip/hip_ext.h>
#include <cstring>

namespace d2s {

enum { A_PLAIN = 0, A_CONV3 = 1 };
enum { ACT_NONE = 0, ACT_GELU = 1, ACT_RELU = 2,
       ACT_GEGLU = 3 };
enum { MAP_ROWS = 0, MAP_SHUFFLE = 1, MAP_QKV = 2, MAP_HEAD = 3 };
enum { OUT_T = 0, OUT_F32 = 1, OUT_BF16 = 2, OUT_BX3 = 3 };

constexpr int D2S_PREC_FP8_OPERANDS = D2S_PREC_FP8;

struct GemmA {
    const void* ptr;
    int mode;
    long lda;
    int Hi, Wi, C;
    int Ho, Wo, stride;
    int relu;
    int buf;
    int bx3;
    int ups, Hs, Ws;
    float usy, usx;
};

constexpr int GEMM_PART_CTR_WORDS = 256;
struct GemmEpi {
    void* out;
    int out_type;
    long ldc;
    const float* bias;
    const float* scale;
    int act;
    const void* res1;
    const void* res2;
    int rows_per_img, img_rows, row_off;
    int res1_mod, res1_off;
    int map, gh, gw, ks, cout;
    void* vt; int ntok, npad, qk_cols, heads;
    float* part; size_t part_elems; int ksplit;
    float head_b3;
    float head_max_depth;
    const float* deq;
    float out_qscale;
    void* out2; float* stats_out; int* stats_slots;
    float out2_qscale;
    int out2_bx3;
    const float* ln_stats; int ln_slots; const float* ln_csum; float ln_eps; int ln_dim;
    int ln_M;
};

int launch_gemm(int precision, int tile, const GemmA& a, const void* W, int M, int N, int K, int Kpad,
                const GemmEpi& e, hipStream_t st, hipEvent_t stop = nullptr);
#define D2S_LAUNCH_STOP(stop, kernel, grid, block, st, ...)                                                            \
    do {                                                                                                               \
        if (stop) hipExtLaunchKernelGGL(kernel, grid, block, 0, st, nullptr, stop, 0, __VA_ARGS__);                    \
        else hipLaunchKernelGGL(kernel, grid, block, 0, st, __VA_ARGS__);                                              \
    } while (0)

bool conv3_upsample_ok(int precision, int tile, const GemmA& a, int M, int N, int K, int Kpad, const GemmEpi& e);

int gemm_pp_min_tiles();

enum { GEMM_GLDS = 0, GEMM_HALO = 1, GEMM_CONV3 = 2, GEMM_PP = 3, GEMM_SK = 4 };
enum { NOTE_TAIL_NONE = 0, NOTE_TAIL_INKERNEL = 1, NOTE_TAIL_TWO_LAUNCH = 2, NOTE_TAIL_ROWSPLIT = 3 };
struct GemmPlan {
    int family, inst;
    const char* name;
    int tile;
    unsigned grid, gridy;
    int block;
    unsigned grid2;
    int xn;
    int buf;
    int ksplit, tail;
    int stats_slots;
    int ups;
    int kps, tw, ink, lxn, skew_us;
    const char* error;
};
int plan_gemm(int precision, int tile, const GemmA& a, int M, int N, int K, int Kpad, const GemmEpi& e, GemmPlan& p);

bool plan_conv3_halo2(const GemmA& a, int M, int N, int K, int Kpad, const GemmEpi& e, GemmPlan& p);
void launch_conv3_halo2(const GemmPlan& p, const GemmA& a, const void* W, int M, int N, int Kpad, const GemmEpi& e, hipStream_t st);
struct RcuOp {
    const void* x; void* out;
    int nimg, H, W;
    const void *w1, *w2, *wp;
    const float *b1, *b2, *bp;
    int Kpad, KpadP;
};
bool c3_rcu_ok(bool plain_bf16, int C, int nimg, int H, int W);
bool plan_conv3_rcu(bool plain_bf16, int C, int nimg, int H, int W, bool proj, GemmPlan& p);
void launch_conv3_rcu(const GemmPlan& p, const RcuOp& o, hipStream_t st);
bool pp_supported(int precision, const GemmA& a, int M, int N, int K, int Kpad, const GemmEpi& e);
int plan_gemm_pp(int precision, const GemmA& a, int M, int N, int K, int Kpad, const GemmEpi& e, GemmPlan& p);
int launch_gemm_pp(const GemmPlan& p, int precision, const GemmA& a, const void* W, int M, int N, int K, int Kpad, const GemmEpi& e, hipStream_t st,
                   hipEvent_t stop = nullptr);
bool sk_supported(int precision, const GemmA& a, int M, int N, int K, int Kpad, const GemmEpi& e);
void plan_gemm_sk(const GemmA& a, int M, int N, int K, GemmPlan& p);
void launch_gemm_sk(const GemmPlan& p, const GemmA& a, const void* W, int M, int N, int Kpad, const GemmEpi& e, hipStream_t st);

struct KernelNote { const char* name; int tile; int ksplit; int tail; };
KernelNote& kernel_note();

static inline int head_tile(int bn) { return bn == 32 ? 912832 : 9256648; }

static inline size_t conv3_weight_index(int n, int k, int Ci) { const int tap = k / Ci, ci = k % Ci; return ((size_t)n * Ci + ci) * 9 + tap; }

static inline size_t elem_size(int precision) { return precision == D2S_PREC_BF16 ? 2 : (precision == D2S_PREC_FP8_OPERANDS ? 1 : 4); }
static inline void bx3_pack_elem(uint8_t* row, int k, float v) {
    const bf16_t hi = f2bf(v), lo = f2bf(v - bf2f(hi));
    uint8_t* u = row + (size_t)(k >> 3) * 32 + (k & 7) * 2;
    memcpy(u, &hi, 2); memcpy(u + 16, &lo, 2);
}
static inline int gemm_bk(int precision) { return 128 / (int)elem_size(precision); }
static inline int gemm_kpad(int K, int precision) { int bk = 2 * gemm_bk(precision); return (K + bk - 1) / bk * bk; }
static inline int gemm_npad(int N) { return (N + 255) / 256 * 256; }

}
```

### desktop2stereo_amd/csrc/gemm.hip

```cpp
#include "gemm_epi.h"
#include "linear_site.h"
#include <cstdio>
#include <deque>
#include <vector>

namespace d2s {

__device__ u32x4 d2s_zero_page[4];

#ifdef D2S_GLDS_TIMING
__device__ unsigned long long glds_timing[4096 * 8];
#define GL_STAMP(SLOT) { if (threadIdx.x == 0 && blockIdx.y == 0 && blockIdx.x < 4096) glds_timing[blockIdx.x * 8 + (SLOT)] = wall_clock64(); }
#else
#define GL_STAMP(SLOT) {}
#endif

__device__ __forceinline__ u32x4 relu_frag(u32x4 v, int, fp8_t) { return v; }
__device__ __forceinline__ u32x4 relu_frag(u32x4 v, int, bx3_t) { return v; }
__device__ __forceinline__ u32x4 relu_frag(u32x4 v, int floor_bits, float) {
    f32x4 x = __builtin_bit_cast(f32x4, v);
    float f = floor_bits == 0 ? 0.f : -3.0e38f;
    x = __builtin_elementwise_max(x, (f32x4){f, f, f, f});
    return __builtin_bit_cast(u32x4, x);
}

template <int N> __device__ __forceinline__ void wait_vmcnt() { asm volatile("s_waitcnt vmcnt(%0)" ::"n"(N) : "memory"); }

template <int CPR> __device__ __forceinline__ int swz_row(int r) { return CPR == 8 ? ((r >> 1) & 7) : (CPR == 4 ? ((r >> 1) & 3) : (r & 15)); }

static_assert(sizeof(GemmA) + sizeof(GemmEpi) + 8 >= KERNARG_WARM_BYTES, "KERNARG_WARM reads past the kernarg segment");
template <typename T, int BM, int BN, int WM, int WN, int NS, int CPR, int STG = 0>
__global__ void __launch_bounds__(64 * WM * WN)
gemm_glds_kernel(const T* __restrict__ W, const void* a_ptr, long a_lda, int M, int N, int K, int Kpad, int xn, GemmA a, GemmEpi e) {
    static_assert(STG == 0 || STG == 2 || (STG == 1 && NS == 2), "the register-staged variant uses two LDS stages");
    constexpr bool LEAN = STG == 2;
    constexpr bool BX3 = std::is_same<T, bx3_t>::value;
    static_assert(!BX3 || CPR == 8, "bf16x3 units are laid out for 128-byte K tiles");
    constexpr int CE = Prec<T>::CE;
    constexpr int BK = CPR * CE;
    constexpr int RPI = 64 / CPR;
    constexpr int NW = WM * WN;
    constexpr int AI = BM / (RPI * NW), BI = BN / (RPI * NW);
    constexpr int LPT = AI + BI;
    constexpr int FM = BM / WM / 16, FN = BN / WN / 16;
    constexpr int PD = NS - 1;
    constexpr int STAGE = (BM + BN) * CPR;
    __shared__ __attribute__((aligned(16))) u32x4 lds[NS * STAGE];
    KERNARG_WARM(kaw_)
    if constexpr (STG != 2) { KERNARG_WARM_END(kaw_) }
    D2S_POISON_LDS(lds, NS * STAGE)

    const int tid = threadIdx.x, lane = tid & 63;
    const int wid = __builtin_amdgcn_readfirstlane(tid >> 6);
    const int wave_m = wid / WN, wave_n = wid % WN;
    int tm_, tn_;
    GL_STAMP(0)
    if (!tile_of_block(blockIdx.x, (M + BM - 1) / BM, (N + BN - 1) / BN, xn, tm_, tn_)) return;
    const int bm0 = tm_ * BM, bn0 = tn_ * BN;
    static_assert((RPI * NW) % 16 == 0, "row swizzle must be invariant across a thread's instructions");
    static_assert(BM % (RPI * NW) == 0 && BN % (RPI * NW) == 0 && BM % (16 * WM) == 0 && BN % (16 * WN) == 0, "tile must split evenly over the waves");
    const int lrow = wid * RPI + lane / CPR;
    const int src_chunk = (lane % CPR) ^ swz_row<CPR>(lrow);
    const T* zero = (const T*)d2s_zero_page;

    const T* arow[AI];
    int aiy[AI], aix[AI];
    bool aok[AI];
    if constexpr (!LEAN)
#pragma unroll
    for (int i = 0; i < AI; ++i) {
        int m = bm0 + i * NW * RPI + lrow;
        aok[i] = m < M;
        int mm = aok[i] ? m : 0;
        if (a.mode == A_PLAIN) { arow[i] = (const T*)a.ptr + (long)mm * a.lda; aiy[i] = aix[i] = 0; }
        else {
            int ox = mm % a.Wo, oy = (mm / a.Wo) % a.Ho, b = mm / (a.Wo * a.Ho);
            aiy[i] = oy * a.stride - 1; aix[i] = ox * a.stride - 1;
            arow[i] = (const T*)a.ptr + (long)b * a.Hi * a.Wi * a.C;
        }
    }
    const T* wrow = W + (long)(bn0 + lrow) * Kpad + src_chunk * CE;
    const float inv_c = a.mode == A_CONV3 ? 1.0f / (float)a.C : 0.f;
    constexpr int ES = (int)sizeof(T);
    const __amdgpu_buffer_rsrc_t rsA = __builtin_amdgcn_make_buffer_rsrc(uniform_ptr(a_ptr), 0, (unsigned)((long)M * a_lda * ES), 0x00020000);
// ... 761 lines not shown
    e.out = Cout; e.out_type = OUT_F32; e.ldc = N; e.bias = bias;
    static EnvInt sk_force{"D2S_SPLITK_FORCE", 0};
    if (sk_force.get() > 1) {
        const size_t pe = (size_t)sk_force.get() * M * N;
        int rc = alloc_splitk_ws(dP, pe, st);
        if (rc != D2S_OK) return rc;
        e.part = (float*)dP.p; e.part_elems = pe;
    }
    int rc = D2S_OK;
    for (int i = 0; i < iters && rc == D2S_OK; ++i) rc = launch_gemm(precision, tile, a, dW.p, M, N, Kp, Kp, e, st);
    hipError_t err = hipStreamSynchronize(st);
    if (rc != D2S_OK) return rc;
    D2S_HIP(err);
    return D2S_OK;
}

extern "C" int d2s_conv3_probe(d2s_conv3_probe_params* p, void* stream) {
    D2S_REQUIRE(p && p->struct_size == sizeof(d2s_conv3_probe_params), "d2s_conv3_probe_params.struct_size must be sizeof(d2s_conv3_probe_params)");
    p->kernel[0] = 0;
    const int prec = p->precision, B = p->batch, C = p->C, N = p->N;
    D2S_REQUIRE(prec == D2S_PREC_BF16 || prec == D2S_PREC_FP32 || prec == D2S_PREC_BF16X3, "bad precision (bf16, fp32 or bf16x3)");
    D2S_REQUIRE(p->x && p->w && p->out && B > 0 && C > 0 && N > 0 && p->Hs > 0 && p->Ws > 0 && p->Hi > 0 && p->Wi > 0, "bad argument");
    D2S_REQUIRE(p->stride == 1 || p->stride == 2, "stride must be 1 or 2");
    const bool ups = p->Hs != p->Hi || p->Ws != p->Wi;
    D2S_REQUIRE(!ups || p->stride == 1, "a folded up-sample needs stride 1");
    D2S_REQUIRE(!p->map_head || (p->w3 && !p->res && p->act == 0 && p->stride == 1), "map_head: w3 needed; no residual, no act, stride 1");
    hipStream_t st = (hipStream_t)stream;
    const int Ho = (p->Hi + 2 - 3) / p->stride + 1, Wo = (p->Wi + 2 - 3) / p->stride + 1;
    const long M = (long)B * Ho * Wo, nsrc = (long)B * p->Hs * p->Ws;
    D2S_REQUIRE(M < (1L << 31) && nsrc * C < (1L << 31), "too large");
    const int K = 9 * C, Kp = gemm_kpad(K, prec);
    const bool bf = prec == D2S_PREC_BF16;
    const bool out_t = !p->out_f32 && !p->map_head;
    ProbeBuf dW, dX, dR, dP;
    {
        std::vector<float> w;
        int rc = fetch_f32(w, p->w, (size_t)N * C * 9);
        if (rc == D2S_OK) {
            const LinearImage im = prepare_linear(prec, N, K, [&](int n, int k) { return w[conv3_weight_index(n, k, C)]; }, nullptr);
            rc = upload(dW, im.w.data(), im.w.size());
        }
        if (rc != D2S_OK) return rc;
    }
    const void* x = p->x;
    if (bf) {
        D2S_HIP(hipMalloc(&dX.p, (size_t)nsrc * C * 2));
        hipLaunchKernelGGL(cast_pad_kernel, dim3(cdiv(nsrc * C, 256)), dim3(256), 0, st, p->x, dX.p, (int)nsrc, C, (int)nsrc, C, D2S_PREC_BF16);
        x = dX.p;
    }
    const void* res = p->res;
    if (res && bf && out_t) {
        D2S_HIP(hipMalloc(&dR.p, (size_t)M * N * 2));
        hipLaunchKernelGGL(cast_pad_kernel, dim3(cdiv(M * N, 256)), dim3(256), 0, st, p->res, dR.p, (int)M, N, (int)M, N, D2S_PREC_BF16);
        res = dR.p;
    }
    D2S_HIP(hipExtGetLastError());
    GemmA a = {};
    a.ptr = x; a.mode = A_CONV3; a.Hi = p->Hi; a.Wi = p->Wi; a.C = C; a.Ho = Ho; a.Wo = Wo; a.stride = p->stride; a.relu = p->relu_in;
    if (ups) { a.ups = 1; a.Hs = p->Hs; a.Ws = p->Ws; a.usy = linear_scale(p->Hs, p->Hi, true); a.usx = linear_scale(p->Ws, p->Wi, true); }
    GemmEpi e = {};
    e.out = p->out; e.out_type = out_t ? OUT_T : OUT_F32; e.ldc = N; e.bias = p->bias;
    e.act = p->act ? ACT_RELU : ACT_NONE; e.res1 = res;
    if (p->map_head) { e.ldc = 1; e.map = MAP_HEAD; e.scale = p->w3; e.head_b3 = p->b3; e.head_max_depth = p->max_depth; }
    const int tile = p->tile ? p->tile : (p->map_head ? head_tile(N <= 32 ? 32 : 64) : 0);
    if (p->splitk_elems > 0) {
        int rc = alloc_splitk_ws(dP, (size_t)p->splitk_elems, st);
        if (rc != D2S_OK) return rc;
        e.part = (float*)dP.p; e.part_elems = (size_t)p->splitk_elems;
    }
    if (ups && !conv3_upsample_ok(prec, tile, a, (int)M, N, K, Kp, e)) {
        set_error("d2s_conv3_probe: conv3_upsample_ok refuses to fold this up-sample");
        return D2S_E_UNSUPPORTED;
    }
    kernel_note() = KernelNote{nullptr, 0, 1};
    int rc = launch_gemm(prec, tile, a, dW.p, (int)M, N, K, Kp, e, st);
    hipError_t err = hipStreamSynchronize(st);
    if (rc != D2S_OK) return rc;
    D2S_HIP(err);
    snprintf(p->kernel, sizeof(p->kernel), "%s", noted_kernel().c_str());
    return D2S_OK;
}

extern "C" int d2s_rcu_probe(d2s_rcu_probe_params* p, void* stream) {
    D2S_REQUIRE(p && p->struct_size == sizeof(d2s_rcu_probe_params), "d2s_rcu_probe_params.struct_size must be sizeof(d2s_rcu_probe_params)");
    p->kernel[0] = 0;
    const int B = p->batch, H = p->H, W = p->W, C = p->C;
    D2S_REQUIRE(p->x && p->w1 && p->b1 && p->w2 && p->b2 && p->out && B > 0 && H > 0 && W > 0 && C > 0 && C % 8 == 0, "bad argument");
    D2S_REQUIRE(!p->wp == !p->bp, "the projection needs its weight and its bias");
    hipStream_t st = (hipStream_t)stream;
    const long npx = (long)B * H * W;
    D2S_REQUIRE(npx * C < (1L << 31), "too large");
    GemmPlan plan;
    if (!plan_conv3_rcu(true, C, B, H, W, p->wp != nullptr, plan)) {
        set_error("d2s_rcu_probe: c3_rcu_ok refuses this map (C = 128 and tiles x images <= CU count)");
        return D2S_E_UNSUPPORTED;
    }
    ProbeBuf dW[3], dX;
    int Kpad[3] = {0, 0, 0};
    for (int i = 0; i < 3; ++i) {
        const float* src = i == 0 ? p->w1 : (i == 1 ? p->w2 : p->wp);
        if (!src) continue;
        const int K = i < 2 ? 9 * C : C;
        std::vector<float> w;
        int rc = fetch_f32(w, src, (size_t)C * K);
        if (rc != D2S_OK) return rc;
        const LinearImage im = i < 2 ? prepare_linear(D2S_PREC_BF16, C, K, [&](int n, int k) { return w[conv3_weight_index(n, k, C)]; }, nullptr)
                                     : prepare_linear(D2S_PREC_BF16, C, K, [&](int n, int k) { return w[(size_t)n * K + k]; }, nullptr);
        rc = upload(dW[i], im.w.data(), im.w.size());
        if (rc != D2S_OK) return rc;
        Kpad[i] = im.Kpad;
    }
    D2S_HIP(hipMalloc(&dX.p, (size_t)npx * C * 2));
    hipLaunchKernelGGL(cast_pad_kernel, dim3(cdiv(npx * C, 256)), dim3(256), 0, st, p->x, dX.p, (int)npx, C, (int)npx, C, D2S_PREC_BF16);
    D2S_HIP(hipExtGetLastError());
    const RcuOp o = {dX.p, p->out, B, H, W, dW[0].p, dW[1].p, dW[2].p, p->b1, p->b2, p->bp, Kpad[0], Kpad[2]};
    kernel_note() = KernelNote{nullptr, 0, 1, NOTE_TAIL_NONE};
    launch_conv3_rcu(plan, o, st);
    D2S_HIP(hipStreamSynchronize(st));
    snprintf(p->kernel, sizeof(p->kernel), "%s", noted_kernel().c_str());
    return D2S_OK;
}

namespace d2s {
namespace {
enum { ACT_F32 = 0, ACT_BF16 = 1, ACT_BX3 = 2, ACT_E4M3 = 3 };
size_t act_bytes(int fmt) { return fmt == ACT_BF16 ? 2 : (fmt == ACT_E4M3 ? 1 : 4); }

int act_operand(ProbeBuf& buf, const float* x, int M, int K, int lda, int fmt, float qscale) {
    std::vector<float> h;
    int rc = fetch_f32(h, x, (size_t)M * K);
    if (rc != D2S_OK) return rc;
    std::vector<uint8_t> o((size_t)M * lda * act_bytes(fmt), 0);
    for (int m = 0; m < M; ++m)
        for (int k = 0; k < K; ++k) {
            const float v = h[(size_t)m * K + k];
            const size_t i = (size_t)m * lda + k;
            if (fmt == ACT_BF16) ((bf16_t*)o.data())[i] = f2bf(v);
            else if (fmt == ACT_E4M3) o[i] = f2e4m3(v * qscale);
            else if (fmt == ACT_BX3) bx3_pack_elem(o.data() + (size_t)m * lda * 4, k, v);
            else ((float*)o.data())[i] = v;
        }
    return upload(buf, o.data(), o.size());
}

}
}

extern "C" int d2s_linear_probe(d2s_linear_probe_params* p, void* stream) {
    D2S_REQUIRE(p && p->struct_size == sizeof(d2s_linear_probe_params), "d2s_linear_probe_params.struct_size must be sizeof(d2s_linear_probe_params)");
    p->kernel[0] = 0; p->kernel2[0] = 0; p->stats_slots = 0;
    const int prec = p->precision, site = p->site, M = p->M, N = p->N, K = p->K;
    D2S_REQUIRE(prec == D2S_PREC_FP32 || prec == D2S_PREC_BF16 || prec == D2S_PREC_BF16X3 || prec == D2S_PREC_FP8 || prec == D2S_PREC_FP8_MLP, "bad precision");
    D2S_REQUIRE(site >= D2S_LIN_PATCH && site <= D2S_LIN_TM_PROJ_OUT, "bad site");
    D2S_REQUIRE(M > 0 && N > 0 && K > 0 && p->w, "bad argument");
    hipStream_t st = (hipStream_t)stream;
    const PrecRules pr = prec_rules(prec);
    const int wprec = pr.w, aprec = pr.act;
    const bool x3 = wprec == D2S_PREC_BF16X3, f8 = pr.e4m3;
    const bool enc = site == D2S_LIN_QKV || site == D2S_LIN_PROJ || site == D2S_LIN_FC1 || site == D2S_LIN_FC2;
    const bool e8 = pr.e4m3_site(site);
    const bool fold = p->ln_fold != 0;
    const bool consumer = fold && (site == D2S_LIN_QKV || site == D2S_LIN_FC1 || site == D2S_LIN_NECK_PROJ || site == D2S_LIN_TM_KVQ || site == D2S_LIN_TM_FF1);
    const bool producer = fold && !consumer;
    D2S_REQUIRE(!producer || site == D2S_LIN_PROJ || site == D2S_LIN_FC2 || site == D2S_LIN_TM_PROJ_IN || site == D2S_LIN_TM_TO_OUT || site == D2S_LIN_TM_FF2,
                "ln_fold: not a LayerNorm consumer or producer site");
    D2S_REQUIRE(!fold || (pr.ln_folds(site) && (enc || !f8)), "ln_fold: the engine does not fold LayerNorm there in this precision");
    const bool per_frame = site == D2S_LIN_QKV || site == D2S_LIN_PATCH || site == D2S_LIN_NECK_PROJ;
    const int P = p->ntok - 1;
    D2S_REQUIRE(!per_frame || (p->ntok > 1 && M % (site == D2S_LIN_PATCH ? P : p->ntok) == 0), "M must be a multiple of the rows per frame");
    const int B = per_frame ? M / (site == D2S_LIN_PATCH ? P : p->ntok) : 1;
    D2S_REQUIRE(site != D2S_LIN_QKV || (p->vt && p->heads > 0 && N == 3 * K && K == 64 * p->heads && p->npad >= p->ntok), "QKV: N = 3 K, K = 64 heads, vt, npad >= ntok");
    D2S_REQUIRE(site != D2S_LIN_NECK_RESIZE || (p->ks > 0 && p->gh > 0 && p->gw > 0 && N == p->ks * p->ks * K && M % (p->gh * p->gw) == 0), "NECK_RESIZE: N = ks^2 K, M = B gh gw");
    D2S_REQUIRE(site != D2S_LIN_TM_FF1 || !consumer || N % 8 == 0, "GEGLU: N must be a multiple of 8");
    D2S_REQUIRE(!x3 || (site != D2S_LIN_QKV && site != D2S_LIN_FC1) || (N % 8 == 0 && K % 8 == 0), "bf16x3 unit-format outputs: whole units (N % 8 == 0)");
    D2S_REQUIRE(!consumer || (p->pa && p->pw && p->pK > 0 && p->ln_g && p->ln_b && p->x && p->out2 && p->stats), "ln_fold consumer: pa, pw, ln_g, ln_b, x, out2, stats");
    D2S_REQUIRE(!producer || (p->out2 && (site == D2S_LIN_TM_FF2 || p->stats)), "ln_fold producer: out2, stats");
    const bool x_out = site == D2S_LIN_PATCH || site == D2S_LIN_PROJ || site == D2S_LIN_FC2 || site == D2S_LIN_TM_PROJ_IN || site == D2S_LIN_TM_TO_OUT || site == D2S_LIN_TM_FF2;
    D2S_REQUIRE(x_out ? p->x != nullptr : p->out != nullptr, "x (residual-stream sites) / out needed");
    ProbeBuf ws;
    if (p->splitk_elems > 0) { int rc = alloc_splitk_ws(ws, (size_t)p->splitk_elems, st); if (rc != D2S_OK) return rc; }
    std::deque<ProbeBuf> mem;
    auto put = [&](LinearImage im, DevLinear& L, float s_a) {
        auto alloc = [&](void** d, const void* h, size_t bytes) { mem.emplace_back(); int rc = upload(mem.back(), h, bytes); *d = mem.back().p; return rc; };
        const bool folded = !im.csum.empty();
        return upload_linear(alloc, std::move(im), L, folded, nullptr, &s_a);
    };
    auto launch = [&](const GemmA& a, const DevLinear& L, int rows, const GemmEpi& ep, char* name) -> int {
        kernel_note() = KernelNote{nullptr, 0, 1, NOTE_TAIL_NONE};
        const int rc = launch_linear(L, a, rows, ep, (float*)ws.p, ws.p ? (size_t)p->splitk_elems : 0, p->tile, st);
        if (rc == D2S_OK) snprintf(name, 128, "%s", noted_kernel().c_str());
        return rc;
    };
    const int ofmt = x3 ? ACT_BX3 : ((consumer ? e8 : f8) ? ACT_E4M3 : ACT_BF16);
    const float o2q = ofmt == ACT_E4M3 ? 1.0f / p->s_res : 0.f;
    int slots = 0;
    ProbeBuf dPa;
    DevLinear Lp;
    if (consumer) {
// ... 99 lines not shown
```

### desktop2stereo_amd/csrc/gemm_epi.h

```cpp
#pragma once
#include "gemm.h"
#include <type_traits>

namespace d2s {

typedef __attribute__((ext_vector_type(8))) __bf16 bf16x8;
typedef __attribute__((ext_vector_type(4))) float f32x4;
typedef __attribute__((ext_vector_type(4))) unsigned int u32x4;

typedef __attribute__((ext_vector_type(4))) unsigned int u32x4_lds_;
__device__ __forceinline__ void lds_dma16(__amdgpu_buffer_rsrc_t rs, void* lds_dst, unsigned voffset, int soffset) {
    __builtin_amdgcn_raw_ptr_buffer_load_lds(rs, (__attribute__((address_space(3))) void*)lds_dst, 16, voffset, soffset, 0, 0);
}
__device__ __forceinline__ void* uniform_ptr(const void* p) {
    const unsigned long long a = (unsigned long long)p;
    const unsigned lo = __builtin_amdgcn_readfirstlane((unsigned)a), hi32 = __builtin_amdgcn_readfirstlane((unsigned)(a >> 32));
    return (void*)(((unsigned long long)hi32 << 32) | lo);
}

template <typename T> struct Prec;
template <> struct Prec<bx3_t>  { static constexpr int CE = 4; };
template <> struct Prec<bf16_t> { static constexpr int CE = 8; };
template <> struct Prec<float>  { static constexpr int CE = 4; };
template <> struct Prec<fp8_t>  { static constexpr int CE = 16; };

__device__ __forceinline__ void mma_chunk(f32x4& acc, const u32x4& w, const u32x4& a, bf16_t) {
    acc = __builtin_amdgcn_mfma_f32_16x16x32_bf16(*(const bf16x8*)&w, *(const bf16x8*)&a, acc, 0, 0, 0);
}
__device__ __forceinline__ void mma_chunk(f32x4& acc, const u32x4& w, const u32x4& a, float) {
    const float* wf = (const float*)&w;
    const float* af = (const float*)&a;
#pragma unroll
    for (int t = 0; t < 4; ++t) acc = __builtin_amdgcn_mfma_f32_16x16x4f32(wf[t], af[t], acc, 0, 0, 0);
}

#define BX3_UNIT(fg) ((0x2130 >> (4 * (fg))) & 3)
__device__ __forceinline__ void mma_bx3(f32x4& acc, const u32x4& w_hi, const u32x4& w_lo, const u32x4& a_hi, const u32x4& a_lo) {
    acc = __builtin_amdgcn_mfma_f32_16x16x32_bf16(*(const bf16x8*)&w_lo, *(const bf16x8*)&a_hi, acc, 0, 0, 0);
    acc = __builtin_amdgcn_mfma_f32_16x16x32_bf16(*(const bf16x8*)&w_hi, *(const bf16x8*)&a_lo, acc, 0, 0, 0);
    acc = __builtin_amdgcn_mfma_f32_16x16x32_bf16(*(const bf16x8*)&w_hi, *(const bf16x8*)&a_hi, acc, 0, 0, 0);
}

__device__ __forceinline__ void mma_chunk(f32x4& acc, const u32x4& w, const u32x4& a, fp8_t) {
    const long* wl = (const long*)&w;
    const long* al = (const long*)&a;
    acc = __builtin_amdgcn_mfma_f32_16x16x32_fp8_fp8(wl[0], al[0], acc, 0, 0, 0);
    acc = __builtin_amdgcn_mfma_f32_16x16x32_fp8_fp8(wl[1], al[1], acc, 0, 0, 0);
}

typedef float f32x2v __attribute__((ext_vector_type(2)));
__device__ __forceinline__ f32x2v gelu_erf2(f32x2v x) {
    const f32x2v ax = __builtin_elementwise_abs(x);
    const f32x2v den = ax * (0.3275911f * 0.70710678118654752f) + 1.0f;
    const f32x2v t = {__builtin_amdgcn_rcpf(den[0]), __builtin_amdgcn_rcpf(den[1])};
    const f32x2v hp = t * (t * (t * (t * (t * (0.5f * 1.061405429f) + (0.5f * -1.453152027f)) + (0.5f * 1.421413741f)) + (0.5f * -0.284496736f)) + (0.5f * 0.254829592f));
    const f32x2v arg = (ax * ax) * (-0.5f * 1.4426950408889634f);
    const f32x2v ex = {__builtin_amdgcn_exp2f(arg[0]), __builtin_amdgcn_exp2f(arg[1])};
    const f32x2v relu = {fmaxf(x[0], 0.f), fmaxf(x[1], 0.f)};
    return relu - (ax * hp) * ex;
}

__device__ __forceinline__ void load4(const float* p, float v[4]) { float4 t = *(const float4*)p; v[0] = t.x; v[1] = t.y; v[2] = t.z; v[3] = t.w; }
__device__ __forceinline__ void load4(const bf16_t* p, float v[4]) {
    uint2 t = *(const uint2*)p;
    v[0] = __uint_as_float(t.x << 16); v[1] = __uint_as_float(t.x & 0xffff0000u);
    v[2] = __uint_as_float(t.y << 16); v[3] = __uint_as_float(t.y & 0xffff0000u);
}
__device__ __forceinline__ void store4(float* p, const float v[4]) { *(float4*)p = make_float4(v[0], v[1], v[2], v[3]); }
typedef __bf16 bf16x2_t __attribute__((ext_vector_type(2)));
typedef float f32x2_t __attribute__((ext_vector_type(2)));
__device__ __forceinline__ uint32_t pk_bf16(float a, float b) {
    f32x2_t v = {a, b};
    return __builtin_bit_cast(uint32_t, __builtin_convertvector(v, bf16x2_t));
}
__device__ __forceinline__ uint32_t lerp_pair_bf16(uint32_t v00, uint32_t v01, uint32_t v10, uint32_t v11, float w0x_, float w1x_, float w0y_, float w1y_) {
    typedef float f2_ __attribute__((ext_vector_type(2)));
    const f2_ w0x = {w0x_, w0x_}, w1x = {w1x_, w1x_}, w0y = {w0y_, w0y_}, w1y = {w1y_, w1y_};
    const f2_ a00 = {__uint_as_float(v00 << 16), __uint_as_float(v00 & 0xffff0000u)}, a01 = {__uint_as_float(v01 << 16), __uint_as_float(v01 & 0xffff0000u)};
    const f2_ a10 = {__uint_as_float(v10 << 16), __uint_as_float(v10 & 0xffff0000u)}, a11 = {__uint_as_float(v11 << 16), __uint_as_float(v11 & 0xffff0000u)};
    const f2_ top = __builtin_elementwise_fma(w1x, a01, w0x * a00);
    const f2_ bot = __builtin_elementwise_fma(w1x, a11, w0x * a10);
    const f2_ o = __builtin_elementwise_fma(w1y, bot, w0y * top);
    return pk_bf16(o[0], o[1]);
}
__device__ __forceinline__ u32x4 lerp_chunk(const u32x4& v00, const u32x4& v01, const u32x4& v10, const u32x4& v11, const Tap& tx, const Tap& ty, bf16_t) {
    u32x4 r;
#pragma unroll
    for (int q = 0; q < 4; ++q) r[q] = lerp_pair_bf16(v00[q], v01[q], v10[q], v11[q], tx.w0, tx.w1, ty.w0, ty.w1);
    return r;
}
__device__ __forceinline__ u32x4 lerp_chunk(const u32x4& v00, const u32x4& v01, const u32x4& v10, const u32x4& v11, const Tap& tx, const Tap& ty, float) {
    u32x4 r;
#pragma unroll
    for (int q = 0; q < 4; ++q)
        r[q] = __float_as_uint(bilerp1(tx, ty, __uint_as_float(v00[q]), __uint_as_float(v01[q]), __uint_as_float(v10[q]), __uint_as_float(v11[q])));
    return r;
}
template <typename T>
__device__ __forceinline__ u32x4 ups_chunk(const T* src_img , const GemmA& a, int iy, int ix, int c_elem) {
    const Tap ty = linear_tap(iy, a.usy, a.Hs, true), tx = linear_tap(ix, a.usx, a.Ws, true);
    const T* r0 = src_img + (long)ty.i0 * a.Ws * a.C + c_elem;
    const T* r1 = src_img + (long)ty.i1 * a.Ws * a.C + c_elem;
    const u32x4 v00 = *(const u32x4*)(r0 + tx.i0 * a.C), v01 = *(const u32x4*)(r0 + tx.i1 * a.C);
    const u32x4 v10 = *(const u32x4*)(r1 + tx.i0 * a.C), v11 = *(const u32x4*)(r1 + tx.i1 * a.C);
    return lerp_chunk(v00, v01, v10, v11, tx, ty, T());
}

typedef short s16x8 __attribute__((ext_vector_type(8)));
__device__ __forceinline__ u32x4 relu_frag(u32x4 v, int floor_bits, bf16_t) {
    s16x8 x = __builtin_bit_cast(s16x8, v);
    short f = (short)floor_bits;
    x = __builtin_elementwise_max(x, (s16x8){f, f, f, f, f, f, f, f});
    return __builtin_bit_cast(u32x4, x);
}
__device__ __forceinline__ int relu_floor_bf16(const GemmA& a) { return a.relu ? 0 : (short)0x8000; }

template <typename T, int NT, int GRP, typename SlotF, typename FinF>
__device__ __forceinline__ void conv_halo_fill(const GemmA& a, int b, int ty0, int tx0, int hwd, int npx, int cpp, int tid, u32x4* halo, SlotF slot, FinF fin) {
    constexpr int CE = 16 / (int)sizeof(T);
    const T* img = (const T*)a.ptr + (long)b * (a.ups ? (long)a.Hs * a.Ws : (long)a.Hi * a.Wi) * a.C;
    const int total = npx * cpp;
    for (int base = tid; base < total; base += NT * GRP) {
        int pp[GRP], cc[GRP], iy[GRP], ix[GRP];
        bool in[GRP], st[GRP];
#pragma unroll
        for (int g = 0; g < GRP; ++g) {
            const int idx = base + g * NT;
            st[g] = idx < total;
            const int i2 = st[g] ? idx : 0;
            pp[g] = i2 / cpp; cc[g] = i2 - pp[g] * cpp;
            const int hy = pp[g] / hwd, hx = pp[g] - hy * hwd;
            iy[g] = ty0 + hy - 1; ix[g] = tx0 + hx - 1;
            in[g] = st[g] && iy[g] >= 0 && iy[g] < a.Hi && ix[g] >= 0 && ix[g] < a.Wi;
            if (!in[g]) { iy[g] = 0; ix[g] = 0; }
        }
        u32x4 r[GRP];
        if (a.ups) {
            Tap ty[GRP], tx[GRP];
            u32x4 v[GRP][4];
#pragma unroll
            for (int g = 0; g < GRP; ++g) {
                ty[g] = linear_tap(iy[g], a.usy, a.Hs, true); tx[g] = linear_tap(ix[g], a.usx, a.Ws, true);
                const T* r0 = img + (long)ty[g].i0 * a.Ws * a.C + cc[g] * CE;
                const T* r1 = img + (long)ty[g].i1 * a.Ws * a.C + cc[g] * CE;
                v[g][0] = *(const u32x4*)(r0 + tx[g].i0 * a.C); v[g][1] = *(const u32x4*)(r0 + tx[g].i1 * a.C);
                v[g][2] = *(const u32x4*)(r1 + tx[g].i0 * a.C); v[g][3] = *(const u32x4*)(r1 + tx[g].i1 * a.C);
            }
#pragma unroll
            for (int g = 0; g < GRP; ++g) r[g] = lerp_chunk(v[g][0], v[g][1], v[g][2], v[g][3], tx[g], ty[g], T());
        } else {
#pragma unroll
            for (int g = 0; g < GRP; ++g) r[g] = *(const u32x4*)(img + ((long)iy[g] * a.Wi + ix[g]) * a.C + cc[g] * CE);
        }
#pragma unroll
        for (int g = 0; g < GRP; ++g)
            if (st[g]) halo[slot(pp[g], cc[g])] = fin(in[g] ? r[g] : (u32x4){0u, 0u, 0u, 0u});
    }
}

__device__ __forceinline__ void store4(bf16_t* p, const float v[4]) {
    uint2 t;
    t.x = pk_bf16(v[0], v[1]);
    t.y = pk_bf16(v[2], v[3]);
    *(uint2*)p = t;
}
__device__ __forceinline__ void bx3_split4(const f32x4& x, uint2& hi, uint2& lo) {
    hi.x = pk_bf16(x[0], x[1]); hi.y = pk_bf16(x[2], x[3]);
    const float r0 = x[0] - __uint_as_float(hi.x << 16), r1 = x[1] - __uint_as_float(hi.x & 0xffff0000u);
    const float r2 = x[2] - __uint_as_float(hi.y << 16), r3 = x[3] - __uint_as_float(hi.y & 0xffff0000u);
    lo.x = pk_bf16(r0, r1); lo.y = pk_bf16(r2, r3);
}

__device__ __forceinline__ uint32_t pk_fp8x4(float a, float b, float c, float d) {
    a = fminf(fmaxf(a, -FP8_MAX), FP8_MAX); b = fminf(fmaxf(b, -FP8_MAX), FP8_MAX);
    c = fminf(fmaxf(c, -FP8_MAX), FP8_MAX); d = fminf(fmaxf(d, -FP8_MAX), FP8_MAX);
    int r = __builtin_amdgcn_cvt_pk_fp8_f32(a, b, 0, false);
    return (uint32_t)__builtin_amdgcn_cvt_pk_fp8_f32(c, d, r, true);
}
// ... 205 lines not shown
```

### desktop2stereo_amd/ops.py

```python
from __future__ import annotations

import ctypes as C
from typing import Dict, Optional, Sequence, Tuple

import numpy as np
import torch

from . import _lib
from ._lib import (FMT_F32_CHW, FMT_F32_HWC, FMT_U8_CHW, FMT_U8_HWC, MODE, PREC_BF16, PREC_FP32,
                   ModelDesc, PostParams, PreParams, SbsParams, check)
from .config import IMAGENET_MEAN, IMAGENET_STD, ModelConfig, PipelineParams, engine_shape


class _on:

    def __init__(self, device: torch.device):
        self.device = device
        self.guard = torch.cuda.device(device)

    def __enter__(self) -> C.c_void_p:
        self.guard.__enter__()
        return C.c_void_p(torch.cuda.current_stream(self.device).cuda_stream)

    def __exit__(self, *exc):
# ... 569 lines not shown
        f = frames.contiguous() if batched else frames.contiguous().unsqueeze(0)
        if f.shape[0] != B or (size is not None and tuple(f.shape[1:3]) != (H, W)):
            raise ValueError(f"dibr_composite: frames {tuple(f.shape)} do not match depth {tuple(d.shape)} / size {size}")
        H, W = f.shape[1:3]
        _same_device(f, d, "dibr_composite")
    elif mode != "Depth Map":
        raise ValueError(f"dibr_composite: {mode} needs the frames")
    lib = _lib.load()
    oh, ow = C.c_int(), C.c_int()
    check(lib.d2s_dibr_composite_shape(H, W, C.byref(dp), _lib.COMPOSITE[mode], C.byref(oh), C.byref(ow)), "d2s_dibr_composite_shape")
    shape, dtype, fmt = _dibr_out_spec(B, oh.value, ow.value, dp, out_u8)
    out = torch.empty(shape, dtype=dtype, device=d.device)
    with _on(d.device) as st:
        check(lib.d2s_dibr_composite_depth(_ptr(f) if f is not None else None, _ptr(d), dh, dw, B, H, W, C.byref(dp), _lib.COMPOSITE[mode],
                                           _ptr(out), fmt, st), "d2s_dibr_composite_depth")
    return out if batched else out[0]


_JPEG_WS: Dict[Tuple[int, int], torch.Tensor] = {}


def jpeg_bound(H: int, W: int) -> Tuple[int, int]:
    ob, wb = C.c_int64(), C.c_int64()
    check(_lib.load().d2s_jpeg_bound(H, W, C.byref(ob), C.byref(wb)), "d2s_jpeg_bound")
    return ob.value, wb.value


def jpeg_encode(frames: torch.Tensor, quality: int = 90, out_stride: Optional[int] = None,
                workspace: Optional[torch.Tensor] = None) -> Tuple[torch.Tensor, torch.Tensor]:
    _need_cuda(frames, "frames")
    if frames.shape[-1] != 3 or frames.dim() not in (3, 4) or frames.dtype not in (torch.uint8, torch.float32):
        raise ValueError("jpeg_encode: frames must be uint8/float32 [B,H,W,3] or [H,W,3]")
    f = (frames if frames.dim() == 4 else frames.unsqueeze(0)).contiguous()
    B, H, W, _ = f.shape
    safe, ws_frame = jpeg_bound(H, W)
    stride = int(out_stride) if out_stride else (safe // 2 + safe // 32 + 1024)
    if workspace is not None:
        if workspace.dtype != torch.uint8 or not workspace.is_cuda or workspace.numel() < ws_frame * B + 256:
            raise ValueError(f"jpeg_encode: workspace must be a uint8 device tensor of >= {ws_frame * B + 256} bytes")
        ws = workspace
    else:
        key = (f.device.index or 0, torch.cuda.current_stream(f.device).cuda_stream)
        ws = _JPEG_WS.get(key)
        if ws is None or ws.numel() < ws_frame * B + 256:
            ws = _JPEG_WS[key] = torch.empty(ws_frame * B + 256, dtype=torch.uint8, device=f.device)
    pad = (-ws.data_ptr()) % 256
    out = torch.empty((B, stride), dtype=torch.uint8, device=f.device)
    sizes = torch.empty((B,), dtype=torch.int32, device=f.device)
    _same_device(f, ws, "jpeg_encode workspace")
    with _on(f.device) as st:
        check(_lib.load().d2s_jpeg_encode(_ptr(f), FMT_U8_HWC if f.dtype == torch.uint8 else FMT_F32_HWC, B, H, W, int(quality),
                                          _ptr(out), stride, _ptr(sizes), C.c_void_p(ws.data_ptr() + pad), ws_frame * B, st),
              "d2s_jpeg_encode")
    return out, sizes


def model_desc(cfg: ModelConfig, precision: str = "bf16", temporal: bool = False, max_depth: float = 0.0) -> ModelDesc:
    if precision not in ("bf16", "fp32", "fp8", "bf16x3", "fp8_mlp"):
        raise ValueError("precision must be 'bf16', 'fp32', 'fp8', 'fp8_mlp' or 'bf16x3'")
    prec = {"bf16": PREC_BF16, "fp32": PREC_FP32, "fp8": _lib.PREC_FP8, "bf16x3": _lib.PREC_BF16X3, "fp8_mlp": _lib.PREC_FP8_MLP}[precision]
    return ModelDesc(cfg.hidden, cfg.heads, cfg.layers, (C.c_int32 * 4)(*cfg.out_indices), (C.c_int32 * 4)(*cfg.neck),
                     cfg.fusion, cfg.head_hidden, cfg.mlp, cfg.patch, cfg.pos_grid, cfg.ln_eps, prec, int(bool(temporal)), float(max_depth))


def forward_plan(cfg: ModelConfig, h: int, w: int, batch: int = 1, precision: str = "bf16", *, temporal: bool = False, max_depth: float = 0.0,
                 calibrating: bool = False, calibrated: bool = True, profiling: bool = False, window_filled: bool = False) -> dict:
    desc = model_desc(cfg, precision, temporal, max_depth)
    F = _lib.PLAN_FLAGS
    flags = (F["calibrating"] * bool(calibrating) | F["profiling"] * bool(profiling) | F["window_filled"] * bool(window_filled) |
             F["calibrated"] * bool(calibrated))
    r = _lib.ForwardPlanResult()
    r.struct_size = C.sizeof(_lib.ForwardPlanResult)
    check(_lib.load().d2s_forward_plan(C.byref(desc), int(h), int(w), int(batch), int(flags), C.byref(r)), "d2s_forward_plan")
    out = {k: bool(getattr(r, k)) for k in ("f8", "f8a", "x3", "lnf", "pp_fold", "tap_fold", "use_side", "head1_ups", "head2_fused",
                                            "head2_ups", "tm_fold", "tm_cache_store")}
    out.update({k: int(getattr(r, k)) for k in ("bn", "gh", "gw", "P", "N", "Npad", "ln_launches", "splitk_elems", "scr_elems")})
    out.update({k: list(getattr(r, k)) for k in ("ln_slots", "fH", "fW", "tm_C", "tm_sites")})
    out["sites"] = {n: {"folded": bool(v & 1), "stats": bool(v & 2), "e4m3": bool(v & 4)} for n, v in zip(_lib.PLAN_SITES, r.site)}
    out["tap_side"] = [bool(v) for v in r.tap_side]
    out["tm_slots"] = [list(m) for m in r.tm_slots]
    out["tm_folded"] = [[bool(v) for v in m] for m in r.tm_folded]
    out["rcu_fused"] = [bool(r.rcu_fused >> i & 1) for i in range(4)]
    out["rcu1_fused"] = [bool(r.rcu_fused >> (8 + i) & 1) for i in range(3)]
    return out


class Engine:

    def __init__(self, cfg: ModelConfig, weights: Dict[str, np.ndarray], h: int, w: int, max_batch: int = 1,
                 precision: str = "bf16", device: int = 0, temporal: bool = False, max_depth: float = 0.0):
        if not torch.cuda.is_available():
            raise _lib.D2SError("no ROCm device: the HIP engine cannot run (and there is no fallback)")
        self.lib = _lib.load()
        self.cfg, self.h, self.w, self.max_batch = cfg, h, w, max_batch
        self.precision = precision
        self.device = torch.device("cuda", device)
        desc = model_desc(cfg, precision, temporal, max_depth)
        self._h = C.c_void_p()
        with _on(self.device):
            check(self.lib.d2s_engine_create(C.byref(desc), device, C.byref(self._h)), "d2s_engine_create")
            for name, arr in weights.items():
                a = np.ascontiguousarray(arr, dtype=np.float32)
                shape = (C.c_int64 * a.ndim)(*a.shape)
                check(self.lib.d2s_engine_set_weight(self._h, name.encode(), a.ctypes.data_as(C.c_void_p), shape, a.ndim),
                      f"d2s_engine_set_weight({name})")
            check(self.lib.d2s_engine_finalize(self._h, h, w, max_batch), "d2s_engine_finalize")

    def _mine(self, t: torch.Tensor, what: str):
        _need_cuda(t, what)
        if t.device != self.device:
            raise _lib.D2SError(f"{what} is on {t.device}, the engine lives on {self.device}")

    def memory_bytes(self) -> int:
        b = C.c_uint64()
        check(self.lib.d2s_engine_memory(self._h, C.byref(b)))
        return b.value

    @staticmethod
    def _stream_ids(streams, B: int):
        if streams is None:
            return None
        ids = [int(s) for s in streams]
        if len(ids) != B:
            raise ValueError(f"streams names {len(ids)} slots for a batch of {B} frames")
        return (C.c_int * B)(*ids)

    def __call__(self, x: torch.Tensor, streams=None) -> torch.Tensor:
        self._mine(x, "pixel_values")
        x = x.to(torch.float32).contiguous()
        if x.dim() == 3:
            x = x.unsqueeze(0)
        B = x.shape[0]
        if tuple(x.shape[1:]) != (3, self.h, self.w):
            raise ValueError(f"engine was built for [B,3,{self.h},{self.w}], got {tuple(x.shape)}")
        out = torch.empty((B, self.h, self.w), dtype=torch.float32, device=x.device)
        with _on(self.device) as st:
            check(self.lib.d2s_model_forward_streams(self._h, _ptr(x), _ptr(out), B, self._stream_ids(streams, B), st), "d2s_model_forward")
        return out

    def calibrate(self, x: torch.Tensor):
        self._mine(x, "calibration inputs")
        x = x.to(torch.float32).contiguous()
        if x.dim() == 3:
            x = x.unsqueeze(0)
        if tuple(x.shape[1:]) != (3, self.h, self.w):
            raise ValueError(f"engine was built for [B,3,{self.h},{self.w}], got {tuple(x.shape)}")
        with _on(self.device) as st:
            check(self.lib.d2s_engine_calibrate(self._h, _ptr(x), x.shape[0], st), "d2s_engine_calibrate")

    def tap(self, name: str) -> torch.Tensor:
        rows, cols = C.c_int(), C.c_int()
        n = max(self.cfg.hidden * (self.h // 14 * (self.w // 14) + 1), 16 * (self.h // 14) * (self.w // 14) * self.cfg.fusion)
        buf = torch.empty(n, dtype=torch.float32, device=self.device)
        with _on(self.device) as st:
            check(self.lib.d2s_engine_tap(self._h, name.encode(), _ptr(buf), n, C.byref(rows), C.byref(cols), st), "d2s_engine_tap")
        return buf[: rows.value * cols.value].view(rows.value, cols.value)

    def profile(self, enable: bool):
        check(self.lib.d2s_engine_profile(self._h, int(enable)), "d2s_engine_profile")

    def profile_read(self) -> Dict[str, dict]:
        n = 16
        ms, fl, by = (C.c_double * n)(), (C.c_double * n)(), (C.c_double * n)()
        cnt = (C.c_int64 * n)()
        nc = C.c_int()
        check(self.lib.d2s_engine_profile_read(self._h, n, ms, fl, by, cnt, C.byref(nc)), "d2s_engine_profile_read")
# ... 120 lines not shown
            raise ValueError("view_pipeline_xr_glow_curved: glow must be an xr.XrGlow (mode \"off\" for none)")
        return self._view_pipeline_xr(frames, p, dp, screen, eyes, crop, use_ema, out_u8, want_depth, out, streams, glow, levels, "glow_curved")

    def view_pipeline_xr_frost(self, frames: torch.Tensor, p: PipelineParams, dp: "_lib.DibrParams", screen, eyes, frost, levels=None,
                               crop=None, use_ema: bool = False, out_u8: bool = True, want_depth: bool = False,
                               out: Optional[torch.Tensor] = None, streams=None):
        if frost is None:
            raise ValueError("view_pipeline_xr_frost: frost must be an xr.XrFrost (mode \"off\" for none)")
        return self._view_pipeline_xr(frames, p, dp, screen, eyes, crop, use_ema, out_u8, want_depth, out, streams, frost, levels, "frost")

    def view_pipeline_xr_frost_curved(self, frames: torch.Tensor, p: PipelineParams, dp: "_lib.DibrParams", screen, eyes, frost, levels=None,
                                      crop=None, use_ema: bool = False, out_u8: bool = True, want_depth: bool = False,
                                      out: Optional[torch.Tensor] = None, streams=None):
        if frost is None:
            raise ValueError("view_pipeline_xr_frost_curved: frost must be an xr.XrFrost (mode \"off\" for none)")
        return self._view_pipeline_xr(frames, p, dp, screen, eyes, crop, use_ema, out_u8, want_depth, out, streams, frost, levels,
                                      "frost_curved")

    def close(self):
        if getattr(self, "_h", None):
            self.lib.d2s_engine_destroy(self._h)
            self._h = None

    def __del__(self):
        try:
            self.close()
        except Exception:
            pass


def reload_env() -> int:
    return int(_lib.load().d2s_debug_reload_env())


def gemm_probe(A: torch.Tensor, Wt: torch.Tensor, bias: Optional[torch.Tensor], precision: str, tile: int = 0, iters: int = 1):
    M, K = A.shape
    N = Wt.shape[0]
    out = torch.empty((M, N), dtype=torch.float32, device=A.device)
    check(_lib.load().d2s_gemm_probe(_ptr(A.contiguous()), _ptr(Wt.contiguous()), _ptr(bias) if bias is not None else None,
                                     _ptr(out), M, N, K, {"bf16": PREC_BF16, "fp32": PREC_FP32, "fp8": _lib.PREC_FP8, "bf16x3": _lib.PREC_BF16X3}[precision], tile, iters,
                                     C.c_void_p(torch.cuda.current_stream(A.device).cuda_stream)),
          "d2s_gemm_probe")
    return out


def conv3_probe(x: torch.Tensor, w: torch.Tensor, bias: Optional[torch.Tensor] = None, precision: str = "bf16", *,
                up: Optional[tuple] = None, stride: int = 1, relu_in: bool = False, act: str = "none",
                res: Optional[torch.Tensor] = None, out_f32: bool = False, head: Optional[tuple] = None, tile: int = 0,
                splitk_elems: int = 0):
    _need_cuda(x, "x")
    B, Hs, Ws, Cin = x.shape
    N = w.shape[0]
    if tuple(w.shape) != (N, Cin, 3, 3):
        raise ValueError("conv3_probe: w must be [N, C, 3, 3]")
    Hi, Wi = up if up is not None else (Hs, Ws)
    Ho, Wo = (Hi - 1) // stride + 1, (Wi - 1) // stride + 1
    prec = {"bf16": PREC_BF16, "fp32": PREC_FP32, "bf16x3": _lib.PREC_BF16X3}[precision]
    keep = [x.float().contiguous(), w.float().contiguous()]
    p = _lib.Conv3ProbeParams()
    p.struct_size = C.sizeof(_lib.Conv3ProbeParams)
    p.precision, p.tile, p.batch, p.C, p.N = prec, int(tile), B, Cin, N
    p.Hs, p.Ws, p.Hi, p.Wi, p.stride = Hs, Ws, Hi, Wi, int(stride)
    p.relu_in, p.act, p.out_f32 = int(bool(relu_in)), {"none": 0, "relu": 1}[act], int(bool(out_f32))
    p.splitk_elems = int(splitk_elems)
    p.x, p.w = _ptr(keep[0]), _ptr(keep[1])
    if bias is not None:
        keep.append(bias.float().contiguous()); p.bias = _ptr(keep[-1])
    if res is not None:
        keep.append(res.float().contiguous()); p.res = _ptr(keep[-1])
    if head is not None:
        w3, b3, max_depth = head
        keep.append(w3.float().contiguous()); p.w3 = _ptr(keep[-1])
        p.map_head, p.b3, p.max_depth = 1, float(b3), float(max_depth)
        out = torch.empty((B, Ho, Wo), dtype=torch.float32, device=x.device)
    else:
        dt = torch.bfloat16 if precision == "bf16" and not out_f32 else torch.float32
        out = torch.empty((B, Ho, Wo, N), dtype=dt, device=x.device)
    p.out = _ptr(out)
    with _on(x.device) as st:
        check(_lib.load().d2s_conv3_probe(C.byref(p), st), "d2s_conv3_probe")
    return out, p.kernel.decode()


def rcu_probe(x: torch.Tensor, w1: torch.Tensor, b1: torch.Tensor, w2: torch.Tensor, b2: torch.Tensor,
              wp: Optional[torch.Tensor] = None, bp: Optional[torch.Tensor] = None):
    _need_cuda(x, "x")
    B, H, W, Cc = x.shape
    if tuple(w1.shape) != (Cc, Cc, 3, 3) or tuple(w2.shape) != (Cc, Cc, 3, 3) or (wp is not None and tuple(wp.shape) != (Cc, Cc)):
        raise ValueError("rcu_probe: w1, w2 must be [C, C, 3, 3], wp [C, C]")
    if (wp is None) != (bp is None):
        raise ValueError("rcu_probe: wp and bp go together")
    keep = [t.float().contiguous() for t in (x, w1, b1, w2, b2)] + ([wp.float().contiguous(), bp.float().contiguous()] if wp is not None else [])
    p = _lib.RcuProbeParams()
    p.struct_size = C.sizeof(_lib.RcuProbeParams)
    p.batch, p.H, p.W, p.C = B, H, W, Cc
    p.x, p.w1, p.b1, p.w2, p.b2 = (_ptr(t) for t in keep[:5])
    if wp is not None:
        p.wp, p.bp = _ptr(keep[5]), _ptr(keep[6])
    out = torch.empty((B, H, W, Cc), dtype=torch.bfloat16, device=x.device)
    p.out = _ptr(out)
    with _on(x.device) as st:
        check(_lib.load().d2s_rcu_probe(C.byref(p), st), "d2s_rcu_probe")
    return out, p.kernel.decode()


def linear_probe(site: str, precision: str, a: Optional[torch.Tensor], w: torch.Tensor, bias: Optional[torch.Tensor] = None, *,
                 scale: Optional[torch.Tensor] = None, x: Optional[torch.Tensor] = None, res: Optional[torch.Tensor] = None,
                 res2: Optional[torch.Tensor] = None, ln: Optional[tuple] = None, producer: Optional[tuple] = None, fold: bool = False,
                 ntok: int = 0, heads: int = 0, npad: int = 0, grid: Optional[tuple] = None, scales: tuple = (0.0, 0.0, 0.0, 0.0),
                 ln_eps: float = 1e-6, tile: int = 0, splitk_elems: int = 0) -> dict:
    _need_cuda(w, "w")
    dev = w.device
    prec = {"fp32": PREC_FP32, "bf16": PREC_BF16, "bf16x3": _lib.PREC_BF16X3, "fp8": _lib.PREC_FP8, "fp8_mlp": _lib.PREC_FP8_MLP}[precision]
    sid = _lib.LINEAR_SITES[site]
    N = w.shape[0] if site != "neck_resize" else w.shape[1] * w.shape[2] * w.shape[3]
    K = w.shape[1] if site != "neck_resize" else w.shape[0]
    consumer = fold and site in ("qkv", "fc1", "neck_proj", "tm_kvq", "tm_ff1")
    M = producer[0].shape[0] if consumer else (x.shape[0] if site in ("proj", "fc2", "tm_proj_in", "tm_to_out", "tm_ff2") else a.shape[0])
    if site == "neck_proj":
        M = (producer[0].shape[0] if consumer else a.shape[0] // (ntok - 1) * ntok)
    x3, f8, f8a = precision == "bf16x3", precision in ("fp8", "fp8_mlp"), precision == "fp8"
    e8 = f8 and (site in ("fc1", "fc2") or (f8a and site in ("qkv", "proj")))
    act16 = precision in ("bf16", "fp8", "fp8_mlp")
    t_out = torch.bfloat16 if act16 else torch.float32

    def alloc(rows, cols, dtype):
        buf = torch.empty((rows + 2, cols), dtype=dtype, device=dev)
        buf.view(torch.uint8).fill_(0x7f)
        return buf
    keep = []

    def fp(t):
        if t is None:
            return None
        keep.append(t.float().contiguous())
        return _ptr(keep[-1])
    p = _lib.LinearProbeParams()
    p.struct_size = C.sizeof(_lib.LinearProbeParams)
    p.site, p.precision, p.ln_fold, p.M, p.N, p.K = sid, prec, int(bool(fold)), M, N, K
    p.ntok, p.heads, p.npad = int(ntok), int(heads), int(npad)
    if grid is not None:
        p.gh, p.gw, p.ks = grid
    p.ln_eps, p.tile, p.splitk_elems = float(ln_eps), int(tile), int(splitk_elems)
    p.s_act, p.s_out, p.s_res, p.s_pact = (float(v) for v in scales)
    p.a, p.w, p.bias, p.scale, p.res, p.res2 = fp(a), fp(w), fp(bias), fp(scale), fp(res), fp(res2)
    if ln is not None:
        p.ln_g, p.ln_b = fp(ln[0]), fp(ln[1])
    if producer is not None:
        p.pK = producer[0].shape[1]
        p.pa, p.pw, p.pbias, p.pscale = fp(producer[0]), fp(producer[1]), fp(producer[2]), fp(producer[3])
    r = {"out": None, "out_guard": None, "vt": None, "out2": None, "x": None, "stats": None}
    if x is not None:
        r["x"] = x.float().clone().contiguous()
        p.x = _ptr(r["x"])
    if site == "qkv":
        odt = torch.bfloat16 if f8 else (torch.int32 if x3 else t_out)
        rows, cols = M, N
    elif site == "fc1":
        odt = torch.int32 if x3 else (torch.uint8 if e8 else t_out)
        rows, cols = M, N
    elif site == "neck_proj":
        odt, rows, cols = t_out, M // ntok * (ntok - 1), N
    elif site == "neck_resize":
        odt, rows, cols = t_out, M * grid[2] * grid[2], K
    elif site == "tm_ff1":
        odt, rows, cols = t_out, M, N // 2 if fold else N
    elif site in ("tm_kvq", "tm_proj_out"):
        odt, rows, cols = t_out, M, N
    else:
        odt = None
    if odt is not None:
        g = alloc(rows, cols, odt)
        r["out_guard"], r["out"] = g, g[1:rows + 1]
        p.out = _ptr(r["out"])
    if site == "qkv":
        B = M // ntok
        r["vt"] = torch.empty((B, heads, 64, npad), dtype=odt, device=dev)
        r["vt"].view(torch.uint8).fill_(0x7f)
        p.vt = _ptr(r["vt"])
    if fold:
        D = K if consumer else N
# ... 138 lines not shown
```

### include/d2s.h

```cpp
#ifndef D2S_H
#define D2S_H

#include <stdint.h>

#ifdef __cplusplus
extern "C" {
#endif

#define D2S_OK              0
#define D2S_E_INVALID       1
#define D2S_E_STATE         2
#define D2S_E_HIP           3
#define D2S_E_MISSING       4
#define D2S_E_UNSUPPORTED   5

#define D2S_MODE_HALF_SBS   0
#define D2S_MODE_FULL_SBS   1
#define D2S_MODE_HALF_TAB   2
#define D2S_MODE_FULL_TAB   3

#define D2S_FMT_U8_HWC      0
#define D2S_FMT_F32_CHW     1
#define D2S_FMT_F32_HWC     2
#define D2S_FMT_U8_CHW      3
// ... 350 lines not shown
                                       const d2s_xr_frost* frost, const uint8_t* levels, void* stream);
int d2s_view_pipeline_xr_frost_curved_streams(d2s_engine* e, const uint8_t* frames, int batch, const int* stream_ids, int H, int W,
                                              int depth_resolution, const d2s_pre_params* pre, const d2s_post_params* pp,
                                              const d2s_dibr_params* dp, const double* crop, const d2s_xr_screen* screen,
                                              const d2s_xr_eye* eyes, int n_eyes, int use_ema, void* out, int out_fmt, float* depth_full,
                                              void* workspace, uint64_t workspace_bytes, const d2s_xr_frost* frost, const uint8_t* levels,
                                              void* stream);
int d2s_view_pipeline_xr_panorama_streams(d2s_engine* e, const uint8_t* frames, int batch, const int* stream_ids, int H, int W,
                                          int depth_resolution, const d2s_pre_params* pre, const d2s_post_params* pp,
                                          const d2s_dibr_params* dp, const double* crop, const d2s_xr_screen* screen,
                                          const d2s_xr_eye* eyes, int n_eyes, int use_ema, void* out, int out_fmt, float* depth_full,
                                          void* workspace, uint64_t workspace_bytes, const d2s_xr_frost* frost, const uint8_t* levels,
                                          const d2s_xr_glow* glow, const d2s_xr_panorama* pano, const uint8_t* pano_rgb,
                                          const uint8_t* pano_levels, void* stream);
int d2s_engine_reset_stream(d2s_engine* e);

int d2s_engine_profile(d2s_engine* e, int enable);
int d2s_engine_profile_read(d2s_engine* e, int max_classes, double* ms, double* flops, double* bytes,
                            int64_t* launches, int* n_classes);
const char* d2s_profile_class_name(int cls);

int d2s_engine_tap(d2s_engine* e, const char* name, float* out, uint64_t out_elems,
                   int* rows, int* cols, void* stream);

int d2s_gemm_probe(const float* A, const float* Wt, const float* bias, float* C,
                   int M, int N, int K, int precision, int tile, int iters, void* stream);

int d2s_attention_probe(const float* q, const float* k, const float* v, float* out, int B, int heads, int N,
                        int precision, int iters, float* ms_per_iter, void* stream);

typedef struct d2s_attention_probe_params {
    uint32_t struct_size;
    int32_t precision;
    int32_t B, heads, N;
    int32_t out_e4m3;
    float   oscale;
    int32_t reserved;
    const float* q;
    const float* k;
    const float* v;
    void* out;
    char kernel[128];
} d2s_attention_probe_params;
int d2s_attention_probe_ex(d2s_attention_probe_params* p, void* stream);

typedef struct d2s_conv3_probe_params {
    uint32_t struct_size;
    int32_t precision;
    int32_t tile;
    int32_t batch, C, N;
    int32_t Hs, Ws;
    int32_t Hi, Wi;
    int32_t stride;
    int32_t relu_in;
    int32_t act;
    int32_t out_f32;
    int32_t map_head;
    float   b3, max_depth;
    int32_t reserved;
    int64_t splitk_elems;
    const float* x;
    const float* w;
    const float* bias;
    const float* res;
    const float* w3;
    void* out;
    char kernel[128];
} d2s_conv3_probe_params;
int d2s_conv3_probe(d2s_conv3_probe_params* p, void* stream);

typedef struct d2s_rcu_probe_params {
    uint32_t struct_size;
    int32_t batch, H, W, C;
    int32_t reserved;
    const float* x;
    const float* w1;
    const float* b1;
    const float* w2;
    const float* b2;
    const float* wp;
    const float* bp;
    void* out;
    char kernel[128];
} d2s_rcu_probe_params;
int d2s_rcu_probe(d2s_rcu_probe_params* p, void* stream);

enum {
    D2S_LIN_PATCH = 0,
    D2S_LIN_QKV = 1,
    D2S_LIN_PROJ = 2,
    D2S_LIN_FC1 = 3,
    D2S_LIN_FC2 = 4,
    D2S_LIN_NECK_PROJ = 5,
    D2S_LIN_NECK_RESIZE = 6,
    D2S_LIN_TM_PROJ_IN = 7,
    D2S_LIN_TM_KVQ = 8,
    D2S_LIN_TM_FF1 = 9,
    D2S_LIN_TM_TO_OUT = 10,
    D2S_LIN_TM_FF2 = 11,
    D2S_LIN_TM_PROJ_OUT = 12
};
typedef struct d2s_linear_probe_params {
    uint32_t struct_size;
    int32_t site;
    int32_t precision;
    int32_t ln_fold;
    int32_t M, N, K;
    int32_t ntok, heads, npad;
    int32_t gh, gw, ks;
    int32_t pK;
    float   ln_eps;
    float   s_act, s_out, s_res, s_pact;
    int32_t tile;
    int64_t splitk_elems;
    const float* a;
    const float* w;
    const float* bias;
    const float* scale;
    const float* res;
    const float* res2;
    const float* ln_g;
    const float* ln_b;
    const float* pa;
    const float* pw;
    const float* pbias;
    const float* pscale;
    float* x;
    void* out;
    void* out2;
    void* vt;
    float* stats;
    int32_t stats_slots;
    int32_t reserved;
    char kernel[128];
    char kernel2[128];
} d2s_linear_probe_params;
int d2s_linear_probe(d2s_linear_probe_params* p, void* stream);

enum {
    D2S_TP_GROUPNORM = 0,
    D2S_TP_TEMPORAL_ATTN = 1,
    D2S_TP_CACHE_STORE = 2,
    D2S_TP_GEGLU = 3,
    D2S_TP_CAST_F32 = 4,
    D2S_TP_LAYERNORM = 5
};
typedef struct d2s_temporal_probe_params {
    uint32_t struct_size;
    int32_t op;
    int32_t precision;
    int32_t rows, sites, C;
    int32_t groups, slots;
    float   eps;
    float   qscale;
    int32_t bx3_out;
    int32_t rows_per_img, img_rows, row_off;
    int64_t n;
    const void* x;
    void* out;
    const float* gamma;
    const float* beta;
    const float* ptab;
    uint64_t x_elems, out_elems, gamma_elems, beta_elems, ptab_elems;
    void* ring[D2S_MAX_STREAMS];
    uint64_t ring_elems[D2S_MAX_STREAMS];
    int32_t head[D2S_MAX_STREAMS], Tw[D2S_MAX_STREAMS], store_slot[D2S_MAX_STREAMS];
// ... 27 lines not shown
```

Baseline: 920.7 stereo frames/s.

## Add wide 8x8 RCU tile and fold bilinear upsample-add into RCU halo fill

Adds a taller 8x8-pixel variant of the fused RCU kernel, so maps too large for one 4x8 tile per CU can still use the fused path, with a shallower weight ring to fit LDS. It also adds an up-sample form where the halo fill computes the bilinear upsample of the coarser map plus the residual addend on the fly. This removes the separate upsample kernel and the round trip of its output through memory. In exchange it adds more gathered loads per halo pixel and higher register and LDS pressure, and the selection logic in the model pipeline is only partly visible.

Result: faster. 932.1 stereo frames/s (median of 6 runs) (+1.2%).

```diff
diff --git a/desktop2stereo_amd/_lib.py b/desktop2stereo_amd/_lib.py
--- a/desktop2stereo_amd/_lib.py
+++ b/desktop2stereo_amd/_lib.py
@@ -91,7 +91,8 @@
 class RcuProbeParams(C.Structure):
     _fields_ = [("struct_size", C.c_uint32), ("batch", C.c_int32), ("H", C.c_int32), ("W", C.c_int32), ("C", C.c_int32),
                 ("reserved", C.c_int32), ("x", C.c_void_p), ("w1", C.c_void_p), ("b1", C.c_void_p), ("w2", C.c_void_p),
-                ("b2", C.c_void_p), ("wp", C.c_void_p), ("bp", C.c_void_p), ("out", C.c_void_p), ("kernel", C.c_char * 128)]
+                ("b2", C.c_void_p), ("wp", C.c_void_p), ("bp", C.c_void_p), ("out", C.c_void_p), ("kernel", C.c_char * 128),
+                ("tile", C.c_int32), ("fold", C.c_int32), ("Hs", C.c_int32), ("Ws", C.c_int32), ("src", C.c_void_p)]
 
 
 class AttentionProbeParams(C.Structure):
diff --git a/desktop2stereo_amd/csrc/conv3.hip b/desktop2stereo_amd/csrc/conv3.hip
--- a/desktop2stereo_amd/csrc/conv3.hip
+++ b/desktop2stereo_amd/csrc/conv3.hip
@@ -955,30 +955,85 @@
     const bf16_t *w1, *w2, *wp;
     const float *b1, *b2, *bp;
     int H, W, nimg, Kpad, KpadP;
+    const bf16_t* src;
+    int Hs, Ws;
+    float usy, usx;
 };
-constexpr int RCU_TH = 4, RCU_TW = 8;
+constexpr int RCU_TH = 4, RCU_TW = 8, RCU_TH_WIDE = 8;
+typedef unsigned int u32x2 __attribute__((ext_vector_type(2)));
 typedef short s16x4 __attribute__((ext_vector_type(4)));
 __device__ __forceinline__ uint2 rcu_pack4(const float v[4], bool relu) {
     uint2 t = make_uint2(pk_bf16(v[0], v[1]), pk_bf16(v[2], v[3]));
     if (relu) t = __builtin_bit_cast(uint2, __builtin_elementwise_max(__builtin_bit_cast(s16x4, t), (s16x4){0, 0, 0, 0}));
     return t;
 }
-typedef unsigned int u32x2 __attribute__((ext_vector_type(2)));
 __device__ __forceinline__ void rcu_lds_write_b64(const u32x4* chunk, int half, uint2 v) {
     const unsigned addr = (unsigned)(unsigned long)((__attribute__((address_space(3))) const char*)chunk) + (unsigned)half * 8u;
     const u32x2 d = {v.x, v.y};
     asm volatile("ds_write_b64 %0, %1" ::"v"(addr), "v"(d) : "memory");
 }
-template <int PROJ>
+__device__ __forceinline__ void rcu_ups_request(const RcuArgs& r, int b, int y, int x, int c, u32x2 (&q)[5], float (&w)[4]) {
+    const Tap ty = linear_tap(y, r.usy, r.Hs, true), tx = linear_tap(x, r.usx, r.Ws, true);
+    const bf16_t* s = r.src + (long)b * r.Hs * r.Ws * 128 + c;
+    const bf16_t* r0 = s + (long)ty.i0 * r.Ws * 128;
+    const bf16_t* r1 = s + (long)ty.i1 * r.Ws * 128;
+    q[0] = *(const u32x2*)(r0 + tx.i0 * 128); q[1] = *(const u32x2*)(r0 + tx.i1 * 128);
+    q[2] = *(const u32x2*)(r1 + tx.i0 * 128); q[3] = *(const u32x2*)(r1 + tx.i1 * 128);
+    q[4] = *(const u32x2*)(r.x + ((long)(b * r.H + y) * r.W + x) * 128 + c);
+    w[0] = tx.w0; w[1] = tx.w1; w[2] = ty.w0; w[3] = ty.w1;
+}
+__device__ __forceinline__ uint2 rcu_ups_value(const u32x2 (&q)[5], const float (&w)[4]) {
+    return make_uint2(lerp_add_pair_bf16(q[0][0], q[1][0], q[2][0], q[3][0], q[4][0], w[0], w[1], w[2], w[3]),
+                      lerp_add_pair_bf16(q[0][1], q[1][1], q[2][1], q[3][1], q[4][1], w[0], w[1], w[2], w[3]));
+}
+template <int NT, int GRP, int W0, int P0, int PST>
+__device__ __forceinline__ void rcu_ups_fill(const RcuArgs& r, int b, int hy0, int hx0, int tid, u32x4* h0) {
+    const bf16_t* src = r.src + (long)b * r.Hs * r.Ws * 128;
+    const bf16_t* add = r.x + (long)b * r.H * r.W * 128;
+    constexpr int total = P0 * 16;
+    for (int base = tid; base < total; base += NT * GRP) {
+        int pp[GRP], cc[GRP];
+        bool in[GRP], st[GRP];
+        Tap ty[GRP], tx[GRP];
+        u32x4 v[GRP][5];
+#pragma unroll
+        for (int g = 0; g < GRP; ++g) {
+            const int idx = base + g * NT;
+            st[g] = idx < total;
+            const int i2 = st[g] ? idx : 0;
+            pp[g] = i2 >> 4; cc[g] = i2 & 15;
+            const int hy = pp[g] / W0, hx = pp[g] - hy * W0;
+            int iy = hy0 + hy, ix = hx0 + hx;
+            in[g] = st[g] && iy >= 0 && iy < r.H && ix >= 0 && ix < r.W;
+            if (!in[g]) { iy = 0; ix = 0; }
+            ty[g] = linear_tap(iy, r.usy, r.Hs, true); tx[g] = linear_tap(ix, r.usx, r.Ws, true);
+            const bf16_t* r0 = src + (long)ty[g].i0 * r.Ws * 128 + cc[g] * 8;
+            const bf16_t* r1 = src + (long)ty[g].i1 * r.Ws * 128 + cc[g] * 8;
+            v[g][0] = *(const u32x4*)(r0 + tx[g].i0 * 128); v[g][1] = *(const u32x4*)(r0 + tx[g].i1 * 128);
+            v[g][2] = *(const u32x4*)(r1 + tx[g].i0 * 128); v[g][3] = *(const u32x4*)(r1 + tx[g].i1 * 128);
+            v[g][4] = *(const u32x4*)(add + ((long)iy * r.W + ix) * 128 + cc[g] * 8);
+        }
+#pragma unroll
+        for (int g = 0; g < GRP; ++g) {
+            const u32x4 x = lerp_add_chunk(v[g][0], v[g][1], v[g][2], v[g][3], v[g][4], tx[g], ty[g]);
+            if (st[g]) h0[pp[g] * PST + cc[g]] = in[g] ? relu_frag(x, 0, bf16_t()) : (u32x4){0u, 0u, 0u, 0u};
+        }
+    }
+}
+template <int PROJ, int WIDE = 0, int UPS = 0>
 __global__ void __launch_bounds__(512)
 conv3_rcu_kernel(RcuArgs r) {
-    constexpr int TH = RCU_TH, TW = RCU_TW, CPP = 16, PST = 17, NW = 8;
+    constexpr int TH = WIDE ? RCU_TH_WIDE : RCU_TH, TW = RCU_TW, CPP = 16, PST = 17, NW = 8;
     constexpr int W0 = TW + 4, P0 = (TH + 4) * W0;
     constexpr int W1 = TW + 2, P1 = (TH + 2) * W1;
+    constexpr int NF1 = (P1 + 15) / 16, NF2 = TH * TW / 16;
     constexpr int NKT = 18, NG = 2 * NKT + (PROJ ? 2 : 0);
     constexpr int WST = 128 * 8;
-    constexpr int NS = 7, PD = NS - 1, BI = 128 / (8 * NW);
-    static_assert(P1 <= 64 && TH * TW == 32 && BI == 2 && NG > PD, "fragment counts below are for a 4 x 8 tile");
+    constexpr int NS = WIDE ? 5 : 7, PD = NS - 1, BI = 128 / (8 * NW);
+    constexpr int HG = WIDE ? 5 : 3;
+    static_assert(TW == 8 && (TH & 1) == 0 && BI == 2 && NG > PD && NF2 * 16 <= P0, "fragment slotting below is for 8-pixel-wide tiles, two rows per fragment");
+    static_assert(!UPS || PROJ, "the up-sample input form exists for the stages' units only");
+    static_assert((NS * WST + P0 * PST + P1 * PST) * 16 <= 160 * 1024, "LDS");
     __shared__ __attribute__((aligned(16))) u32x4 lds[NS * WST + P0 * PST + P1 * PST];
     D2S_POISON_LDS(lds, NS * WST + P0 * PST + P1 * PST)
     u32x4* const h0 = lds + NS * WST;
@@ -998,6 +1053,16 @@
     float c1[4], c2[4], cp[4] = {0.f, 0.f, 0.f, 0.f};
     load4(r.b1 + n0, c1); load4(r.b2 + n0, c2);
     if constexpr (PROJ) load4(r.bp + n0, cp);
+    [[maybe_unused]] u32x2 xq[UPS ? NF2 : 1][5];
+    [[maybe_unused]] float xw[UPS ? NF2 : 1][4];
+    if constexpr (UPS) {
+#pragma unroll
+        for (int f = 0; f < NF2; ++f) {
+            const int y = ty0 + 2 * f + (fr >> 3), x = tx0 + (fr & 7);
+            const bool ok = y < r.H && x < r.W;
+            rcu_ups_request(r, b, ok ? y : 0, ok ? x : 0, n0, xq[f], xw[f]);
+        }
+    }
 
     const unsigned wbytes = 256u * (unsigned)r.Kpad * 2u, pbytes = 256u * (unsigned)r.KpadP * 2u;
     const __amdgpu_buffer_rsrc_t rs1 = __builtin_amdgcn_make_buffer_rsrc(uniform_ptr(r.w1), 0, wbytes, 0x00020000);
@@ -1027,11 +1092,21 @@
 #pragma unroll
     for (int t = 0; t < PD; ++t) issue(t, t);
 
-    conv_halo_fill<bf16_t, 64 * NW, 3>(a, b, ty0 - 1, tx0 - 1, W0, P0, CPP, tid, h0,
-        [&](int p, int c) { return p * PST + c; },
-        [&](u32x4 v) { return relu_frag(v, relu_floor_bf16(a), bf16_t()); });
+    if constexpr (UPS) rcu_ups_fill<64 * NW, HG, W0, P0, PST>(r, b, ty0 - 2, tx0 - 2, tid, h0);
+    else
+        conv_halo_fill<bf16_t, 64 * NW, HG>(a, b, ty0 - 1, tx0 - 1, W0, P0, CPP, tid, h0,
+            [&](int p, int c) { return p * PST + c; },
+            [&](u32x4 v) { return relu_frag(v, relu_floor_bf16(a), bf16_t()); });
 #pragma unroll
     for (int q = 0; q < 4; ++q) asm volatile("" : "+v"(c1[q]), "+v"(c2[q]), "+v"(cp[q]));
+    [[maybe_unused]] uint2 xres[UPS ? NF2 : 1];
+    if constexpr (UPS) {
+#pragma unroll
+        for (int f = 0; f < NF2; ++f) {
+            asm volatile("" : "+v"(xq[f][0]), "+v"(xq[f][1]), "+v"(xq[f][2]), "+v"(xq[f][3]), "+v"(xq[f][4]));
+            xres[f] = rcu_ups_value(xq[f], xw[f]);
+        }
+    }
 
     int g = 0, slot = 0, islot = PD;
     auto ring_step = [&]() -> const u32x4* {
@@ -1050,7 +1125,7 @@
         islot = islot + 1 == NS ? 0 : islot + 1;
         return B_l;
     };
-    static_assert(PD == 6, "ring_step spells out the waits of the last PD - 1 tiles");
+    static_assert(PD <= 6, "ring_step spells out the waits of the last PD - 1 tiles");
     int wo[2];
     {
         const int row = wid * 16 + fr;
@@ -1059,35 +1134,35 @@
     }
 
     {
-        const u32x4* hb[4];
-#pragma unroll
-        for (int f = 0; f < 4; ++f) {
+        const u32x4* hb[NF1];
+#pragma unroll
+        for (int f = 0; f < NF1; ++f) {
             const int p = f * 16 + fr < P1 ? f * 16 + fr : P1 - 1;
             hb[f] = h0 + ((p / W1) * W0 + p % W1) * PST + fg;
         }
-        f32x4 acc[4];
-#pragma unroll
-        for (int f = 0; f < 4; ++f) acc[f] = (f32x4){0.f, 0.f, 0.f, 0.f};
+        f32x4 acc[NF1];
+#pragma unroll
+        for (int f = 0; f < NF1; ++f) acc[f] = (f32x4){0.f, 0.f, 0.f, 0.f};
 #pragma unroll 1
         for (int kt = 0; kt < NKT; ++kt) {
             const int tap = kt >> 1, ky = (tap * 11) >> 5, kx = tap - 3 * ky;
             const int toff = (ky * W0 + kx) * PST + (kt & 1) * 8;
             const u32x4* B_l = ring_step();
-            u32x4 fb[2], fa[2][4];
+            u32x4 fb[2], fa[2][NF1];
 #pragma unroll
             for (int ks = 0; ks < 2; ++ks) {
                 fb[ks] = B_l[wo[ks]];
 #pragma unroll
-                for (int f = 0; f < 4; ++f) fa[ks][f] = hb[f][toff + ks * 4];
+                for (int f = 0; f < NF1; ++f) fa[ks][f] = hb[f][toff + ks * 4];
             }
             __builtin_amdgcn_sched_barrier(0);
 #pragma unroll
             for (int ks = 0; ks < 2; ++ks)
 #pragma unroll
-                for (int f = 0; f < 4; ++f) mma_chunk(acc[f], fb[ks], fa[ks][f], bf16_t());
-        }
-#pragma unroll
-        for (int f = 0; f < 4; ++f) {
+                for (int f = 0; f < NF1; ++f) mma_chunk(acc[f], fb[ks], fa[ks][f], bf16_t());
+        }
+#pragma unroll
+        for (int f = 0; f < NF1; ++f) {
             const int p = f * 16 + fr;
             const int py = p / W1, px = p - py * W1;
             const int iy = ty0 - 1 + py, ix = tx0 - 1 + px;
@@ -1099,41 +1174,46 @@
     }
 
     const int oy0 = fr >> 3, ox = fr & 7;
-    uint2 rcu[2];
+    uint2 rcu[NF2];
     {
-        const u32x4* hb[2];
-#pragma unroll
-        for (int f = 0; f < 2; ++f) hb[f] = h1 + ((2 * f + oy0) * W1 + ox) * PST + fg;
-        f32x4 acc[2];
-#pragma unroll
-        for (int f = 0; f < 2; ++f) acc[f] = (f32x4){0.f, 0.f, 0.f, 0.f};
+        const u32x4* hb[NF2];
+#pragma unroll
+        for (int f = 0; f < NF2; ++f) hb[f] = h1 + ((2 * f + oy0) * W1 + ox) * PST + fg;
+        f32x4 acc[NF2];
+#pragma unroll
+        for (int f = 0; f < NF2; ++f) acc[f] = (f32x4){0.f, 0.f, 0.f, 0.f};
 #pragma unroll 1
         for (int kt = 0; kt < NKT; ++kt) {
             const int tap = kt >> 1, ky = (tap * 11) >> 5, kx = tap - 3 * ky;
             const int toff = (ky * W1 + kx) * PST + (kt & 1) * 8;
             const u32x4* B_l = ring_step();
-            u32x4 fb[2], fa[2][2];
+            u32x4 fb[2], fa[2][NF2];
 #pragma unroll
             for (int ks = 0; ks < 2; ++ks) {
                 fb[ks] = B_l[wo[ks]];
 #pragma unroll
-                for (int f = 0; f < 2; ++f) fa[ks][f] = hb[f][toff + ks * 4];
+                for (int f = 0; f < NF2; ++f) fa[ks][f] = hb[f][toff + ks * 4];
             }
             __builtin_amdgcn_sched_barrier(0);
 #pragma unroll
             for (int ks = 0; ks < 2; ++ks)
 #pragma unroll
-                for (int f = 0; f < 2; ++f) mma_chunk(acc[f], fb[ks], fa[ks][f], bf16_t());
-        }
-        float xr[2][4];
-#pragma unroll
-        for (int f = 0; f < 2; ++f) {
-            const int y = ty0 + 2 * f + oy0, x = tx0 + ox;
-            const bool ok = y < r.H && x < r.W;
-            load4(r.x + ((long)(b * r.H + (ok ? y : 0)) * r.W + (ok ? x : 0)) * 128 + n0, xr[f]);
-        }
-#pragma unroll
-        for (int f = 0; f < 2; ++f) {
+                for (int f = 0; f < NF2; ++f) mma_chunk(acc[f], fb[ks], fa[ks][f], bf16_t());
+        }
+        float xr[NF2][4];
+#pragma unroll
+        for (int f = 0; f < NF2; ++f) {
+            if constexpr (UPS) {
+                xr[f][0] = __uint_as_float(xres[f].x << 16); xr[f][1] = __uint_as_float(xres[f].x & 0xffff0000u);
+                xr[f][2] = __uint_as_float(xres[f].y << 16); xr[f][3] = __uint_as_float(xres[f].y & 0xffff0000u);
+            } else {
+                const int y = ty0 + 2 * f + oy0, x = tx0 + ox;
+                const bool ok = y < r.H && x < r.W;
+                load4(r.x + ((long)(b * r.H + (ok ? y : 0)) * r.W + (ok ? x : 0)) * 128 + n0, xr[f]);
+            }
+        }
+#pragma unroll
+        for (int f = 0; f < NF2; ++f) {
             float v[4] = {acc[f][0] + c2[0], acc[f][1] + c2[1], acc[f][2] + c2[2], acc[f][3] + c2[3]};
             v[0] += xr[f][0]; v[1] += xr[f][1]; v[2] += xr[f][2]; v[3] += xr[f][3];
             rcu[f] = rcu_pack4(v, false);
@@ -1141,16 +1221,16 @@
     }
     if constexpr (!PROJ) {
 #pragma unroll
-        for (int f = 0; f < 2; ++f) {
+        for (int f = 0; f < NF2; ++f) {
             const int y = ty0 + 2 * f + oy0, x = tx0 + ox;
             if (y < r.H && x < r.W) *(uint2*)(r.out + ((long)(b * r.H + y) * r.W + x) * 128 + n0) = rcu[f];
         }
     } else {
 #pragma unroll
-        for (int f = 0; f < 2; ++f) rcu_lds_write_b64(h2 + (f * 16 + fr) * PST + 2 * wid + (fg >> 1), fg & 1, rcu[f]);
-        f32x4 acc[2];
-#pragma unroll
-        for (int f = 0; f < 2; ++f) acc[f] = (f32x4){0.f, 0.f, 0.f, 0.f};
+        for (int f = 0; f < NF2; ++f) rcu_lds_write_b64(h2 + (f * 16 + fr) * PST + 2 * wid + (fg >> 1), fg & 1, rcu[f]);
+        f32x4 acc[NF2];
+#pragma unroll
+        for (int f = 0; f < NF2; ++f) acc[f] = (f32x4){0.f, 0.f, 0.f, 0.f};
 #pragma unroll 1
         for (int kt = 0; kt < 2; ++kt) {
             const u32x4* B_l = ring_step();
@@ -1158,11 +1238,11 @@
             for (int ks = 0; ks < 2; ++ks) {
                 const u32x4 fb = B_l[wo[ks]];
 #pragma unroll
-                for (int f = 0; f < 2; ++f) mma_chunk(acc[f], fb, h2[(f * 16 + fr) * PST + fg + kt * 8 + ks * 4], bf16_t());
-            }
-        }
-#pragma unroll
-        for (int f = 0; f < 2; ++f) {
+                for (int f = 0; f < NF2; ++f) mma_chunk(acc[f], fb, h2[(f * 16 + fr) * PST + fg + kt * 8 + ks * 4], bf16_t());
+            }
+        }
+#pragma unroll
+        for (int f = 0; f < NF2; ++f) {
             const int y = ty0 + 2 * f + oy0, x = tx0 + ox;
             const float v[4] = {acc[f][0] + cp[0], acc[f][1] + cp[1], acc[f][2] + cp[2], acc[f][3] + cp[3]};
             if (y < r.H && x < r.W) *(uint2*)(r.out + ((long)(b * r.H + y) * r.W + x) * 128 + n0) = rcu_pack4(v, false);
@@ -1173,6 +1253,10 @@
 #define C3_INSTANCES(P, H, R)                                                                                                    \
     R(C3_RCU, conv3_rcu_kernel<0>)                                                                                               \
     R(C3_RCU_PROJ, conv3_rcu_kernel<1>)                                                                                          \
+    R(C3_RCU_PROJ_UPS, conv3_rcu_kernel<1,0,1>)            \
+    R(C3_RCU_WIDE, conv3_rcu_kernel<0,1>)                                                                   \
+    R(C3_RCU_PROJ_WIDE, conv3_rcu_kernel<1,1>)                                                                                   \
+    R(C3_RCU_PROJ_WIDE_UPS, conv3_rcu_kernel<1,1,1>)                                                                             \
     P(C3_HEAD_UPS, conv3_head_ups_kernel)                                                                                        \
     P(C3_HEAD_1, conv3_head_kernel<1>)                                                                                           \
     P(C3_HEAD_0, conv3_head_kernel<0>)                                                                                           \
@@ -1284,17 +1368,25 @@
     return plain_bf16 && C == 128 && nimg > 0 && H > 0 && W > 0 && (long)nimg * H * W * 128 < (1L << 31) &&
            (long)nimg * cdiv(H, RCU_TH) * cdiv(W, RCU_TW) <= device_cu_count();
 }
-bool plan_conv3_rcu(bool plain_bf16, int C, int nimg, int H, int W, bool proj, GemmPlan& p) {
-    if (!c3_rcu_ok(plain_bf16, C, nimg, H, W)) return false;
+static bool c3_rcu_wide_fits(bool plain_bf16, int C, int nimg, int H, int W) {
+    return plain_bf16 && C == 128 && nimg > 0 && H > 0 && W > 0 && (long)nimg * H * W * 128 < (1L << 31) &&
+           (long)nimg * cdiv(H, RCU_TH_WIDE) * cdiv(W, RCU_TW) <= device_cu_count();
+}
+bool c3_rcu_wide_ok(bool plain_bf16, int C, int nimg, int H, int W) {
+    return !c3_rcu_ok(plain_bf16, C, nimg, H, W) && c3_rcu_wide_fits(plain_bf16, C, nimg, H, W);
+}
+bool plan_conv3_rcu(bool plain_bf16, int C, int nimg, int H, int W, bool proj, GemmPlan& p, bool wide, bool ups) {
+    if (!(wide ? c3_rcu_wide_fits(plain_bf16, C, nimg, H, W) : c3_rcu_ok(plain_bf16, C, nimg, H, W)) || (ups && !proj)) return false;
     p = GemmPlan{};
-    const int inst = proj ? C3_RCU_PROJ : C3_RCU;
-    p.family = GEMM_CONV3; p.inst = inst; p.name = c3_inst[inst].name; p.block = c3_inst[inst].block;
-    p.grid = (unsigned)(nimg * cdiv(H, RCU_TH) * cdiv(W, RCU_TW)); p.ksplit = 1;
+    const int inst = wide ? (ups ? C3_RCU_PROJ_WIDE_UPS : (proj ? C3_RCU_PROJ_WIDE : C3_RCU_WIDE)) : (ups ? C3_RCU_PROJ_UPS : (proj ? C3_RCU_PROJ : C3_RCU));
+    p.family = GEMM_CONV3; p.inst = inst; p.name = c3_inst[inst].name; p.block = c3_inst[inst].block; p.ups = ups;
+    p.grid = (unsigned)(nimg * cdiv(H, wide ? RCU_TH_WIDE : RCU_TH) * cdiv(W, RCU_TW)); p.ksplit = 1;
     return true;
 }
 void launch_conv3_rcu(const GemmPlan& p, const RcuOp& o, hipStream_t st) {
-    const RcuArgs r = {(const bf16_t*)o.x, (bf16_t*)o.out, (const bf16_t*)o.w1, (const bf16_t*)o.w2, (const bf16_t*)o.wp, o.b1, o.b2, o.bp,
-                       o.H, o.W, o.nimg, o.Kpad, o.KpadP};
+    RcuArgs r = {(const bf16_t*)o.x, (bf16_t*)o.out, (const bf16_t*)o.w1, (const bf16_t*)o.w2, (const bf16_t*)o.wp, o.b1, o.b2, o.bp,
+                 o.H, o.W, o.nimg, o.Kpad, o.KpadP, nullptr, 0, 0, 0.f, 0.f};
+    if (p.ups) { r.src = (const bf16_t*)o.src; r.Hs = o.Hs; r.Ws = o.Ws; r.usy = linear_scale(o.Hs, o.H, true); r.usx = linear_scale(o.Ws, o.W, true); }
     const dim3 grid(p.grid), block(p.block);
     switch (p.inst) {
 #define C3_N(ID, ...)
diff --git a/desktop2stereo_amd/csrc/core.cpp b/desktop2stereo_amd/csrc/core.cpp
--- a/desktop2stereo_amd/csrc/core.cpp
+++ b/desktop2stereo_amd/csrc/core.cpp
@@ -47,4 +47,4 @@
 }
 extern "C" int d2s_debug_reload_env(void) { return d2s::g_env_gen.fetch_add(1) + 1; }
 extern "C" const char* d2s_last_error(void) { return d2s::g_err.c_str(); }
-extern "C" int d2s_version(void) { return 127; }
+extern "C" int d2s_version(void) { return 128; }
diff --git a/desktop2stereo_amd/csrc/engine.hip b/desktop2stereo_amd/csrc/engine.hip
--- a/desktop2stereo_amd/csrc/engine.hip
+++ b/desktop2stereo_amd/csrc/engine.hip
@@ -276,13 +276,16 @@
     return linear(e, a, w, B * Ho * Wo, ep, st);
 }
 
-int rcu(d2s_engine* e, const void* x, int B, int H, int W, const DevLinear& c1, const DevLinear& c2, const DevLinear* proj, void* out, hipStream_t st) {
+int rcu(d2s_engine* e, const void* x, int B, int H, int W, const DevLinear& c1, const DevLinear& c2, const DevLinear* proj, void* out, hipStream_t st,
+        bool wide = false, const void* src = nullptr, int Hs = 0, int Ws = 0) {
     GemmPlan p;
-    if (!plan_conv3_rcu(true, e->d.fusion, B, H, W, proj != nullptr, p) || c1.Kpad != c2.Kpad || !c1.bias || !c2.bias || (proj && !proj->bias)) {
+    if (!plan_conv3_rcu(true, e->d.fusion, B, H, W, proj != nullptr, p, wide, src != nullptr) || c1.Kpad != c2.Kpad || !c1.bias || !c2.bias ||
+        (proj && !proj->bias) || (src && src == out)) {
         set_error("forward: the frame's plan fuses a residual unit that conv3_rcu_kernel does not take");
         return D2S_E_STATE;
     }
-    const RcuOp o = {x, out, B, H, W, c1.w, c2.w, proj ? proj->w : nullptr, c1.bias, c2.bias, proj ? proj->bias : nullptr, c1.Kpad, proj ? proj->Kpad : 0};
+    const RcuOp o = {x, out, B, H, W, c1.w, c2.w, proj ? proj->w : nullptr, c1.bias, c2.bias, proj ? proj->bias : nullptr, c1.Kpad, proj ? proj->Kpad : 0,
+                     src, Hs, Ws};
     const double macs = (double)c1.N * c1.K + (double)c2.N * c2.K + (proj ? (double)proj->N * proj->K : 0.0);
     PROF(PC_CONV, 2.0 * B * H * W * macs, 0, (launch_conv3_rcu(p, o, st), D2S_OK));
     return D2S_OK;
@@ -388,7 +391,7 @@
     RC(conv3(e, src, B, Hs, Ws, c, 1, 0, e->re[i].conv, e->feat[i], ACT_NONE, nullptr, nullptr, st));
     if (i < 3) {
         const int idx = 3 - i;
-        if (pl.rcu1_fused[i]) RC(rcu(e, e->feat[i], B, Hs, Ws, e->fu[idx].r1c1, e->fu[idx].r1c2, nullptr, e->r1[i], st));
+        if (pl.rcu1_fused[i] || pl.rcu1_wide[i]) RC(rcu(e, e->feat[i], B, Hs, Ws, e->fu[idx].r1c1, e->fu[idx].r1c2, nullptr, e->r1[i], st, pl.rcu1_wide[i]));
         else {
             RC(conv3(e, e->feat[i], B, Hs, Ws, F, 1, 1, e->fu[idx].r1c1, e->r1tmp, ACT_NONE, nullptr, nullptr, st));
             RC(conv3(e, e->r1tmp, B, Hs, Ws, F, 1, 1, e->fu[idx].r1c2, e->r1[i], ACT_NONE, e->feat[i], nullptr, st));
@@ -486,6 +489,7 @@
         D2S_HIP(hipStreamWaitEvent(st, e->ev_side, 0));
     }
     void *X = e->scr[0], *Y = e->scr[1], *Z = e->scr[2];
+    void* PX = X;
     void* fused = nullptr;
     int Hc = 0, Wc = 0;
     for (int idx = 0; idx < 4; ++idx) {
@@ -493,8 +497,16 @@
         void* m = e->feat[mi];
         Hc = e->g.fH[mi]; Wc = e->g.fW[mi];
         const void* hcur = idx == 0 ? m : fused;
-        if (pl.rcu_fused[idx]) RC(rcu(e, hcur, B, Hc, Wc, e->fu[idx].r2c1, e->fu[idx].r2c2, &e->fu[idx].proj, X, st));
-        else {
+        const bool one = pl.rcu_fused[idx] || pl.rcu_wide[idx];
+        if (one && pl.rcu_ups[idx]) {
+            void* prev = PX;
+            PX = prev == X ? Z : X;
+            RC(rcu(e, e->r1[3 - idx], B, Hc, Wc, e->fu[idx].r2c1, e->fu[idx].r2c2, &e->fu[idx].proj, PX, st, pl.rcu_wide[idx], prev, e->g.fH[mi + 1], e->g.fW[mi + 1]));
+        } else if (one) {
+            PX = X;
+            RC(rcu(e, hcur, B, Hc, Wc, e->fu[idx].r2c1, e->fu[idx].r2c2, &e->fu[idx].proj, PX, st, pl.rcu_wide[idx]));
+        } else {
+            PX = X;
             RC(conv3(e, hcur, B, Hc, Wc, F, 1, 1, e->fu[idx].r2c1, X, ACT_NONE, nullptr, nullptr, st));
             RC(conv3(e, X, B, Hc, Wc, F, 1, 1, e->fu[idx].r2c2, Z, ACT_NONE, hcur, nullptr, st));
         }
@@ -502,14 +514,15 @@
         if (idx < 3) { Ho = e->g.fH[mi - 1]; Wo = e->g.fW[mi - 1]; } else { Ho = Hc * 2; Wo = Wc * 2; }
         void* pout = e->scr[3 + (idx & 1)];
         const void* next_r1 = idx < 3 ? e->r1[2 - idx] : nullptr;
-        if (!pl.rcu_fused[idx]) RC(linear(e, plainA(Z, F), e->fu[idx].proj, B * Hc * Wc, rowsE(X, OUT_T, F, e->fu[idx].proj.bias), st));
+        if (!one) RC(linear(e, plainA(Z, F), e->fu[idx].proj, B * Hc * Wc, rowsE(X, OUT_T, F, e->fu[idx].proj.bias), st));
+        const bool next_forms = idx < 3 && pl.rcu_ups[idx + 1];
         if (d.temporal && idx < 2) {
-            PROF(PC_ELT, 0, 0, launch_bilinear_nhwc(prec, X, pout, B, Hc, Wc, Ho, Wo, F, st));
+            PROF(PC_ELT, 0, 0, launch_bilinear_nhwc(prec, PX, pout, B, Hc, Wc, Ho, Wo, F, st));
             void* alt = e->scr[3 + ((idx + 1) & 1)];
             RC(run_temporal(e, pl, 2 + idx, pout, alt, B, st, next_r1));
             pout = alt;
         } else {
-            if (!(idx == 3 && pl.head1_ups)) PROF(PC_ELT, 0, 0, launch_bilinear_nhwc(prec, X, pout, B, Hc, Wc, Ho, Wo, F, st, next_r1));
+            if (!(idx == 3 && pl.head1_ups) && !next_forms) PROF(PC_ELT, 0, 0, launch_bilinear_nhwc(prec, PX, pout, B, Hc, Wc, Ho, Wo, F, st, next_r1));
         }
         fused = pout; Hc = Ho; Wc = Wo;
     }
@@ -517,7 +530,7 @@
     void* up2 = Y;
     if (pl.head1_ups) {
         c1out = Y; up2 = X;
-        const LinearOp o = op_head1_ups(X, e->g.fH[0], e->g.fW[0], F, c1out, e->head1.bias);
+        const LinearOp o = op_head1_ups(PX, e->g.fH[0], e->g.fW[0], F, c1out, e->head1.bias);
         PROF(PC_CONV, 2.0 * B * Hc * Wc * e->head1.N * e->head1.K, 0, launch_gemm(e->wprec, 0, o.a, e->head1.w, B * Hc * Wc, e->head1.N, e->head1.K, e->head1.Kpad, o.ep, st));
     } else {
         RC(conv3(e, fused, B, Hc, Wc, F, 1, 0, e->head1, c1out, ACT_NONE, nullptr, nullptr, st));
@@ -882,7 +895,9 @@
     r.gh = g.gh; r.gw = g.gw; r.P = g.P; r.N = g.N; r.Npad = g.Npad;
     for (int i = 0; i < 4; ++i) { r.fH[i] = g.fH[i]; r.fW[i] = g.fW[i]; r.tm_C[i] = d.temporal ? g.tmC[i] : 0; r.tm_sites[i] = d.temporal ? g.tmS[i] : 0; }
     r.ln_launches = pl.ln_launches;
-    for (int i = 0; i < 4; ++i) r.rcu_fused |= (pl.rcu_fused[i] ? 1 << i : 0) | (pl.rcu1_fused[i] ? 256 << i : 0);
+    for (int i = 0; i < 4; ++i)
+        r.rcu_fused |= (pl.rcu_fused[i] ? 1 << i : 0) | (pl.rcu1_fused[i] ? 256 << i : 0) | (pl.rcu_wide[i] ? 16 << i : 0) | (pl.rcu1_wide[i] ? 4096 << i : 0) |
+                       (pl.rcu_ups[i] ? 65536 << i : 0);
     r.splitk_elems = g.splitk_elems; r.scr_elems = g.scr_elems;
     *res = r;
     return D2S_OK;
diff --git a/desktop2stereo_amd/csrc/forward_plan.h b/desktop2stereo_amd/csrc/forward_plan.h
--- a/desktop2stereo_amd/csrc/forward_plan.h
+++ b/desktop2stereo_amd/csrc/forward_plan.h
@@ -92,6 +92,8 @@
     int bn;
     bool rcu_fused[4];
     bool rcu1_fused[4];
+    bool rcu_wide[4], rcu1_wide[4];
+    bool rcu_ups[4];
     bool tm_fold;
     struct { int slots[3]; bool folded[3]; } tm[4];
     int ln_launches;
@@ -146,6 +148,14 @@
             pl.rcu_fused[3 - i] = ok;
             pl.rcu1_fused[i] = ok && i < 3;
         }
+        static EnvInt rcu_wide{"D2S_RCU_WIDE", 1}, rcu_ups{"D2S_RCU_UPS", 1};
+        for (int i = 0; i < 4; ++i) {
+            const bool wide = rcu_wide.get() && c3_rcu_wide_ok(plain_bf16, F, B, g.fH[i], g.fW[i]);
+            pl.rcu_wide[3 - i] = wide;
+            pl.rcu1_wide[i] = wide && i < 3;
+        }
+        for (int idx = 1; idx < 4; ++idx)
+            pl.rcu_ups[idx] = rcu_ups.get() && (pl.rcu_fused[idx] || pl.rcu_wide[idx]) && !(d.temporal && idx < 3);
     }
     pl.tm_fold = d.temporal && s.tm_fold;
     for (int m = 0; m < 4 && d.temporal; ++m) {
diff --git a/desktop2stereo_amd/csrc/gemm.h b/desktop2stereo_amd/csrc/gemm.h
--- a/desktop2stereo_amd/csrc/gemm.h
+++ b/desktop2stereo_amd/csrc/gemm.h
@@ -91,9 +91,11 @@
     const void *w1, *w2, *wp;
     const float *b1, *b2, *bp;
     int Kpad, KpadP;
+    const void* src; int Hs, Ws;
 };
 bool c3_rcu_ok(bool plain_bf16, int C, int nimg, int H, int W);
-bool plan_conv3_rcu(bool plain_bf16, int C, int nimg, int H, int W, bool proj, GemmPlan& p);
+bool c3_rcu_wide_ok(bool plain_bf16, int C, int nimg, int H, int W);
+bool plan_conv3_rcu(bool plain_bf16, int C, int nimg, int H, int W, bool proj, GemmPlan& p, bool wide = false, bool ups = false);
 void launch_conv3_rcu(const GemmPlan& p, const RcuOp& o, hipStream_t st);
 bool pp_supported(int precision, const GemmA& a, int M, int N, int K, int Kpad, const GemmEpi& e);
 int plan_gemm_pp(int precision, const GemmA& a, int M, int N, int K, int Kpad, const GemmEpi& e, GemmPlan& p);
diff --git a/desktop2stereo_amd/csrc/gemm.hip b/desktop2stereo_amd/csrc/gemm.hip
--- a/desktop2stereo_amd/csrc/gemm.hip
+++ b/desktop2stereo_amd/csrc/gemm.hip
@@ -1,5 +1,6 @@
 #include "gemm_epi.h"
 #include "linear_site.h"
+#include "vit_ops.h"
 #include <cstdio>
 #include <deque>
 #include <vector>
@@ -927,8 +928,13 @@
 }
 
 extern "C" int d2s_rcu_probe(d2s_rcu_probe_params* p, void* stream) {
-    D2S_REQUIRE(p && p->struct_size == sizeof(d2s_rcu_probe_params), "d2s_rcu_probe_params.struct_size must be sizeof(d2s_rcu_probe_params)");
+    D2S_REQUIRE(p && (p->struct_size == sizeof(d2s_rcu_probe_params) || p->struct_size == 216),
+                "d2s_rcu_probe_params.struct_size must be sizeof(d2s_rcu_probe_params)");
     p->kernel[0] = 0;
+    const bool grown = p->struct_size == sizeof(d2s_rcu_probe_params);
+    const bool wide = grown && p->tile == 1, ups = grown && p->src != nullptr, fold = ups && p->fold != 0;
+    D2S_REQUIRE(!grown || p->tile == 0 || p->tile == 1, "tile: 0 (4 x 8 pixels) or 1 (8 x 8)");
+    D2S_REQUIRE(!ups || (p->Hs > 0 && p->Ws > 0 && p->wp), "src: its size and the projection are needed");
     const int B = p->batch, H = p->H, W = p->W, C = p->C;
     D2S_REQUIRE(p->x && p->w1 && p->b1 && p->w2 && p->b2 && p->out && B > 0 && H > 0 && W > 0 && C > 0 && C % 8 == 0, "bad argument");
     D2S_REQUIRE(!p->wp == !p->bp, "the projection needs its weight and its bias");
@@ -936,11 +942,11 @@
     const long npx = (long)B * H * W;
     D2S_REQUIRE(npx * C < (1L << 31), "too large");
     GemmPlan plan;
-    if (!plan_conv3_rcu(true, C, B, H, W, p->wp != nullptr, plan)) {
+    if (!plan_conv3_rcu(true, C, B, H, W, p->wp != nullptr, plan, wide, fold)) {
         set_error("d2s_rcu_probe: c3_rcu_ok refuses this map (C = 128 and tiles x images <= CU count)");
         return D2S_E_UNSUPPORTED;
     }
-    ProbeBuf dW[3], dX;
+    ProbeBuf dW[3], dX, dS, dU;
     int Kpad[3] = {0, 0, 0};
     for (int i = 0; i < 3; ++i) {
         const float* src = i == 0 ? p->w1 : (i == 1 ? p->w2 : p->wp);
@@ -957,8 +963,21 @@
     }
     D2S_HIP(hipMalloc(&dX.p, (size_t)npx * C * 2));
     hipLaunchKernelGGL(cast_pad_kernel, dim3(cdiv(npx * C, 256)), dim3(256), 0, st, p->x, dX.p, (int)npx, C, (int)npx, C, D2S_PREC_BF16);
+    const void* xin = dX.p;
+    if (ups) {
+        const long nsrc = (long)B * p->Hs * p->Ws;
+        D2S_REQUIRE(nsrc * C < (1L << 31), "too large");
+        D2S_HIP(hipMalloc(&dS.p, (size_t)nsrc * C * 2));
+        hipLaunchKernelGGL(cast_pad_kernel, dim3(cdiv(nsrc * C, 256)), dim3(256), 0, st, p->src, dS.p, (int)nsrc, C, (int)nsrc, C, D2S_PREC_BF16);
+        if (!fold) {
+            D2S_HIP(hipMalloc(&dU.p, (size_t)npx * C * 2));
+            int rc = launch_bilinear_nhwc(D2S_PREC_BF16, dS.p, dU.p, B, p->Hs, p->Ws, H, W, C, st, dX.p);
+            if (rc != D2S_OK) return rc;
+            xin = dU.p;
+        }
+    }
     D2S_HIP(hipExtGetLastError());
-    const RcuOp o = {dX.p, p->out, B, H, W, dW[0].p, dW[1].p, dW[2].p, p->b1, p->b2, p->bp, Kpad[0], Kpad[2]};
+    const RcuOp o = {xin, p->out, B, H, W, dW[0].p, dW[1].p, dW[2].p, p->b1, p->b2, p->bp, Kpad[0], Kpad[2], fold ? dS.p : nullptr, p->Hs, p->Ws};
     kernel_note() = KernelNote{nullptr, 0, 1, NOTE_TAIL_NONE};
     launch_conv3_rcu(plan, o, st);
     D2S_HIP(hipStreamSynchronize(st));
diff --git a/desktop2stereo_amd/csrc/gemm_epi.h b/desktop2stereo_amd/csrc/gemm_epi.h
--- a/desktop2stereo_amd/csrc/gemm_epi.h
+++ b/desktop2stereo_amd/csrc/gemm_epi.h
@@ -94,6 +94,25 @@
 #pragma unroll
     for (int q = 0; q < 4; ++q)
         r[q] = __float_as_uint(bilerp1(tx, ty, __uint_as_float(v00[q]), __uint_as_float(v01[q]), __uint_as_float(v10[q]), __uint_as_float(v11[q])));
+    return r;
+}
+__device__ __forceinline__ uint32_t lerp_add_pair_bf16(uint32_t v00, uint32_t v01, uint32_t v10, uint32_t v11, uint32_t add, float w0x_, float w1x_,
+                                                       float w0y_, float w1y_) {
+    typedef float f2_ __attribute__((ext_vector_type(2)));
+    const f2_ w0x = {w0x_, w0x_}, w1x = {w1x_, w1x_}, w0y = {w0y_, w0y_}, w1y = {w1y_, w1y_};
+    const f2_ a00 = {__uint_as_float(v00 << 16), __uint_as_float(v00 & 0xffff0000u)}, a01 = {__uint_as_float(v01 << 16), __uint_as_float(v01 & 0xffff0000u)};
+    const f2_ a10 = {__uint_as_float(v10 << 16), __uint_as_float(v10 & 0xffff0000u)}, a11 = {__uint_as_float(v11 << 16), __uint_as_float(v11 & 0xffff0000u)};
+    const f2_ ad = {__uint_as_float(add << 16), __uint_as_float(add & 0xffff0000u)};
+    const f2_ top = __builtin_elementwise_fma(w1x, a01, w0x * a00);
+    const f2_ bot = __builtin_elementwise_fma(w1x, a11, w0x * a10);
+    const f2_ o = __builtin_elementwise_fma(w1y, bot, w0y * top) + ad;
+    return pk_bf16(o[0], o[1]);
+}
+__device__ __forceinline__ u32x4 lerp_add_chunk(const u32x4& v00, const u32x4& v01, const u32x4& v10, const u32x4& v11, const u32x4& add, const Tap& tx,
+                                                const Tap& ty) {
+    u32x4 r;
+#pragma unroll
+    for (int q = 0; q < 4; ++q) r[q] = lerp_add_pair_bf16(v00[q], v01[q], v10[q], v11[q], add[q], tx.w0, tx.w1, ty.w0, ty.w1);
     return r;
 }
 template <typename T>
diff --git a/desktop2stereo_amd/ops.py b/desktop2stereo_amd/ops.py
--- a/desktop2stereo_amd/ops.py
+++ b/desktop2stereo_amd/ops.py
@@ -675,6 +675,9 @@
     out["tm_folded"] = [[bool(v) for v in m] for m in r.tm_folded]
     out["rcu_fused"] = [bool(r.rcu_fused >> i & 1) for i in range(4)]
     out["rcu1_fused"] = [bool(r.rcu_fused >> (8 + i) & 1) for i in range(3)]
+    out["rcu_wide"] = [bool(r.rcu_fused >> (4 + i) & 1) for i in range(4)]
+    out["rcu1_wide"] = [bool(r.rcu_fused >> (12 + i) & 1) for i in range(3)]
+    out["rcu_ups"] = [bool(r.rcu_fused >> (16 + i) & 1) for i in range(4)]
     return out
 
 
@@ -961,8 +964,19 @@
     return out, p.kernel.decode()
 
 
-def rcu_probe(x: torch.Tensor, w1: torch.Tensor, b1: torch.Tensor, w2: torch.Tensor, b2: torch.Tensor,
-              wp: Optional[torch.Tensor] = None, bp: Optional[torch.Tensor] = None):
+def rcu_probe(x: Optional[torch.Tensor], w1: torch.Tensor, b1: torch.Tensor, w2: torch.Tensor, b2: torch.Tensor,
+              wp: Optional[torch.Tensor] = None, bp: Optional[torch.Tensor] = None, *, tile: str = "narrow",
+              up_from: Optional[tuple] = None, fold: bool = True):
+    if tile not in ("narrow", "wide"):
+        raise ValueError("rcu_probe: tile must be 'narrow' or 'wide'")
+    src = None
+    if up_from is not None:
+        if x is not None or wp is None:
+            raise ValueError("rcu_probe: up_from replaces x (pass None) and needs the projection")
+        src, x = up_from
+        _need_cuda(src, "src")
+        if src.dim() != 4 or x.dim() != 4 or src.shape[0] != x.shape[0] or src.shape[3] != x.shape[3]:
+            raise ValueError("rcu_probe: up_from = (src [B, Hs, Ws, C], addend [B, H, W, C])")
     _need_cuda(x, "x")
     B, H, W, Cc = x.shape
     if tuple(w1.shape) != (Cc, Cc, 3, 3) or tuple(w2.shape) != (Cc, Cc, 3, 3) or (wp is not None and tuple(wp.shape) != (Cc, Cc)):
@@ -976,6 +990,10 @@
     p.x, p.w1, p.b1, p.w2, p.b2 = (_ptr(t) for t in keep[:5])
     if wp is not None:
         p.wp, p.bp = _ptr(keep[5]), _ptr(keep[6])
+    p.tile = int(tile == "wide")
+    if src is not None:
+        keep.append(src.float().contiguous())
+        p.src, p.Hs, p.Ws, p.fold = _ptr(keep[-1]), src.shape[1], src.shape[2], int(bool(fold))
     out = torch.empty((B, H, W, Cc), dtype=torch.bfloat16, device=x.device)
     p.out = _ptr(out)
     with _on(x.device) as st:
diff --git a/include/d2s.h b/include/d2s.h
--- a/include/d2s.h
+++ b/include/d2s.h
@@ -456,6 +456,10 @@
     const float* bp;
     void* out;
     char kernel[128];
+    int32_t tile;
+    int32_t fold;
+    int32_t Hs, Ws;
+    const float* src;
 } d2s_rcu_probe_params;
 int d2s_rcu_probe(d2s_rcu_probe_params* p, void* stream);
 
```
